# facebookresearch/mbrl-lib

Measured on AMD Instinct MI355X. Metric: candidate-steps/sec (pop×particles×horizon / plan) per CEM iter; plans/sec, higher is better.
Workload: dtype f32

## Files before the change

__graft_entry__.py:

```python
import os
import subprocess
import sys

ROOT = os.path.dirname(os.path.abspath(__file__))
PKG = os.path.join(ROOT, "mbrl-lib_amd")
CSRC = os.path.join(PKG, "csrc")
LIB = os.path.join(PKG, "hipets", "libhipets.so")
BUILDINFO = os.path.join(PKG, "hipets", "libhipets.buildinfo.json")
OBJDIR = os.path.join(PKG, "build")
HIPCC = os.environ.get("HIPCC", "/opt/rocm/bin/hipcc")
HOST_UNITS = ["train.hip", "plan.hip", "rollout.hip", "model.hip", "comm.hip", "engine.hip"]
UNITS = ["rollout_r3.hip", "rollout_r4_gen.hip", "rollout_r4_gens.hip", "rollout_r3_gen.hip", "rollout_r3_gens.hip", "rollout_r2.hip", "rollout_r2_gen.hip",
         "rollout_r2_gens.hip", "rollout_r1_gen.hip", "rollout_r1_gens.hip", "rollout_r1.hip", "rollout_r4.hip", "rollout_r2_fast.hip", "rollout_r3_fast.hip",
         "rollout_r1_fast.hip", "planet.hip"] + HOST_UNITS + ["rollout_r4_fast.hip"]
FLAGS = ["--offload-arch=gfx950", "-O3", "-std=c++17", "-ffp-contract=off", "-fPIC", "-Wno-pass-failed"]


def _sources():
    return sorted(os.path.join(CSRC, f) for f in os.listdir(CSRC)) + [os.path.join(ROOT, "include", "hipets.h")]


def source_digest(extra_flags=()):
    import hashlib

    h = hashlib.sha256()
    h.update(" ".join(FLAGS + list(extra_flags)).encode())
    for path in _sources():
        h.update(os.path.basename(path).encode())
        with open(path, "rb") as f:
            h.update(f.read())
    return h.hexdigest()[:16]


def built_digest(lib=LIB):
    import json

    info = os.path.splitext(lib)[0] + ".buildinfo.json"
    if not (os.path.exists(lib) and os.path.exists(info)):
        return None
    try:
        return json.load(open(info)).get("source_digest")
    except Exception:
        return None


def scan_isa_hazards(asm_path):
    import re

    def regs(tok):
        tok = tok.strip().rstrip(",")
        m = re.fullmatch(r"([va])\[(\d+):(\d+)\]", tok)
        if m:
            return {(m.group(1), x) for x in range(int(m.group(2)), int(m.group(3)) + 1)}
        m = re.fullmatch(r"([va])(\d+)", tok)
        return {(m.group(1), int(m.group(2)))} if m else set()

    prog, labels, in_asm = [], {}, False
    for raw in open(asm_path, errors="replace"):
        line = raw.split(";")[0].strip() if not raw.lstrip().startswith(";;#") else raw.strip()
        if line.startswith(";;#ASMSTART"):
            in_asm = True
            continue
        if line.startswith(";;#ASMEND"):
            in_asm = False
            continue
        if not line or line.startswith("."):
            if line.startswith(".L") and line.endswith(":"):
                labels[line[:-1]] = len(prog)
                prog.append(("label", line[:-1], False))
            continue
        if line.endswith(":"):
            if line[0].isdigit():
                continue
            prog.append(("kernel", line[:-1], False))
            continue
        prog.append(("ins", line, in_asm))

    findings, seen = [], 0

    def step(kernel, line, asm, inflight, recent, count, via):
        nonlocal seen
        parts = line.replace(",", " ").split()
        op, ops = parts[0], parts[1:]
        touched = set()
        for o in ops:
            touched |= regs(o)
        if op.startswith("v_mfma"):
            if asm:
                if count:
                    seen += 1
                src = set()
                for o in ops[1:]:
                    src |= regs(o)
                ws = 0
                for nop, written, text, _ in reversed(recent[-3:]):
                    if ws >= 2:
                        break
                    if nop is not None:
                        ws += nop
                        continue
                    if written & src:
                        findings.append(f"{kernel}: '{text}' writes a source of '{line}' {ws} wait state(s) ahead{via}")
                    ws += 1
            inflight = [(r, c - 32) for r, c in inflight if c - 32 > 0]
            if asm:
                inflight.append((regs(ops[0]), 40))
            recent.append((None, set(), line, set()))
        else:
            cost, nop = 4, None
            if op == "s_nop":
                nop = int(ops[0]) + 1
                cost = 4 * nop
            elif op.startswith("s_waitcnt") or op.startswith("s_barrier"):
                cost = 64
            if any(r & touched for r, _ in inflight) and op.split("_")[0] in ("v", "ds", "global", "buffer", "scratch", "flat"):
                findings.append(f"{kernel}: '{line}' touches the destination of an MFMA still in flight{via}")
            inflight = [(r, c - cost) for r, c in inflight if c - cost > 0]
            writes = set()
            if ops and (op.startswith("v_") or op.startswith("ds_read") or (op.split("_")[0] in ("global", "buffer", "flat", "scratch") and "_load" in op)):
                writes = regs(ops[0])
            if writes:
                ws = 0
                for pnop, _, ptext, pstore in reversed(recent[-3:]):
                    if ws >= 2:
                        break
                    if pnop is not None:
                        ws += pnop
                        continue
                    if pstore & writes:
                        findings.append(f"{kernel}: '{line}' overwrites the data of '{ptext}' {ws} wait state(s) behind it{via}")
                    ws += 1
            store_data = set()
            if asm and op.split("_")[0] in ("global", "buffer", "flat", "scratch") and re.search(r"_store_dwordx[34]", op):
                store_data = regs(ops[1]) if op.startswith(("global", "flat", "scratch")) else regs(ops[0])
            recent.append((nop, regs(ops[0]) if (op.startswith("v_") and ops) else set(), line, store_data))
        if len(recent) > 8:
            del recent[0]
        return inflight

    def undrained(inflight, recent):
        ws = 0
        for nop, written, _, store in reversed(recent[-3:]):
            if ws >= 2:
                break
            if nop is not None:
                ws += nop
                continue
            if written or store:
                return True
            ws += 1
        return bool(inflight)

    edges = []
    kernel, inflight, recent = "?", [], []
    for kind, text, asm in prog:
        if kind == "kernel":
            kernel, inflight, recent = text, [], []
        elif kind == "ins":
            inflight = step(kernel, text, asm, inflight, recent, True, "")
            op = text.split()[0]
            if op.startswith("s_cbranch") or op == "s_branch":
                target = text.split()[-1]
                if target in labels and undrained(inflight, recent):
                    edges.append((kernel, target, list(inflight), list(recent)))
            if op in ("s_branch", "s_endpgm", "s_setpc_b64"):
                inflight, recent = [], []
    done = set()
# ... 247 lines not shown
```

include/hipets.h:

```cpp
#ifndef HIPETS_H
#define HIPETS_H

#include <stdint.h>

#ifdef __cplusplus
extern "C" {
#endif

#define HIPETS_ABI_VERSION 9
#define HIPETS_MAX_LAYERS 8
#define HIPETS_MAX_REWARD_TERMS 64
#define HIPETS_MAX_TERM_INTERVALS 64
#define HIPETS_MAX_OBS_COLUMNS 512

typedef struct hipets_engine hipets_engine;

enum { HIPETS_ACT_RELU = 0, HIPETS_ACT_SILU = 1, HIPETS_ACT_LEAKY_RELU = 2, HIPETS_ACT_TANH = 3, HIPETS_ACT_SIGMOID = 4 };
enum { HIPETS_PROP_RANDOM_MODEL = 0, HIPETS_PROP_FIXED_MODEL = 1, HIPETS_PROP_EXPECTATION = 2 };
enum { HIPETS_OBS_NONE = 0, HIPETS_OBS_HALFCHEETAH = 1, HIPETS_OBS_CARTPOLE_PETS = 2,
       HIPETS_OBS_COLUMNS = 3  };
enum { HIPETS_REW_LEARNED = 0, HIPETS_REW_CARTPOLE = 1, HIPETS_REW_CARTPOLE_PETS = 2, HIPETS_REW_INVERTED_PENDULUM = 3,
       HIPETS_REW_HALFCHEETAH = 4, HIPETS_REW_PUSHER = 5,
       HIPETS_REW_NONE = 6,
       HIPETS_REW_TERMS = 7  };
enum { HIPETS_TERM_NONE = 0, HIPETS_TERM_CARTPOLE = 1, HIPETS_TERM_INVERTED_PENDULUM = 2, HIPETS_TERM_HOPPER = 3,
       HIPETS_TERM_WALKER2D = 4, HIPETS_TERM_ANT = 5, HIPETS_TERM_HUMANOID = 6,
       HIPETS_TERM_BOX = 7  };
enum { HIPETS_NORM_NONE = 0, HIPETS_NORM_F32 = 1, HIPETS_NORM_F64 = 2 };
enum { HIPETS_ENSEMBLE_GAUSSIAN_MLP = 0, HIPETS_ENSEMBLE_BASIC = 1 };
enum { HIPETS_PREC_F32 = 0,
       HIPETS_PREC_BF16X3 = 1,
       HIPETS_PREC_BF16 = 2
                                };
enum { HIPETS_MODE_EXACT = 0,
       HIPETS_MODE_FAST = 1,
       HIPETS_MODE_DEVICE = 2
                                };

enum { HIPETS_TERM_FN_LINEAR = 0, HIPETS_TERM_FN_SQUARE = 1, HIPETS_TERM_FN_ABS = 2,
       HIPETS_TERM_FN_SIN = 3, HIPETS_TERM_FN_COS = 4, HIPETS_TERM_FN_EXP = 5, HIPETS_TERM_FN_SQRT = 6 };
enum { HIPETS_TERM_SRC_OBS = 0, HIPETS_TERM_SRC_ACT = 1, HIPETS_TERM_SRC_GROUP = 2, HIPETS_TERM_SRC_CONST = 3 };
enum { HIPETS_TERM_OP_ADD = 0, HIPETS_TERM_OP_MUL = 1, HIPETS_TERM_OP_DIV = 2 };
#define HIPETS_TERM_MAX_LEVEL 2
#define HIPETS_TERM_WORD(fn, op, level) ((int32_t)((fn) | ((op) << 8) | ((level) << 16)))
#define HIPETS_TERM_WORD_FN(word) ((int32_t)((word) & 0xff))
#define HIPETS_TERM_WORD_OP(word) ((int32_t)(((word) >> 8) & 0xff))
#define HIPETS_TERM_WORD_LEVEL(word) ((int32_t)(((uint32_t)(word)) >> 16))
enum { HIPETS_BOX_LO_OPEN = 1, HIPETS_BOX_HI_OPEN = 2 };
typedef struct {
    int32_t fn;
    int32_t source;
    int32_t i;
    int32_t j;
    float c;
    float w;
} hipets_reward_term;
typedef struct {
    int32_t dim;
    int32_t flags;
    float lo;
    float hi;
} hipets_term_interval;

enum { HIPETS_COL_ID = 0, HIPETS_COL_SIN = 1, HIPETS_COL_COS = 2 };
typedef struct {
    int32_t dim;
    int32_t fn;
} hipets_obs_column;

typedef struct {
    int32_t obs_dim;
    int32_t act_dim;
    int32_t in_dim;
    int32_t out_dim;
    int32_t hid;
    int32_t n_layers;
    int32_t ensemble_size;
    int32_t n_members;
    const int32_t* members;
    int32_t activation;
    float leaky_slope;
    int32_t propagation;
    int32_t deterministic;
    int32_t obs_process;
    int32_t reward_fn;
    int32_t termination_fn;
    int32_t target_is_delta;
    int32_t learned_rewards;
    int32_t n_no_delta;
    const int32_t* no_delta;
    int32_t normalizer;
    const double* norm_mean;
    const double* norm_std;
    const float* min_logvar;
    const float* max_logvar;
    const void* const* weights;
    const void* const* biases;
    int32_t ensemble_kind;
    int32_t precision;
    const hipets_reward_term* reward_terms;
    const hipets_term_interval* term_intervals;
    int32_t n_reward_terms;
    int32_t n_term_intervals;
    float reward_bias;
    float alive_bonus;
    int32_t term_require_finite;
} hipets_model_desc;

typedef struct {
    int32_t mode;
    const int64_t* perms;
    const float* eps;
    uint64_t seed;
    uint64_t stream_id;
    const int32_t* member_schedule;
    const float* fast_eps;
    float* trace_next_obs;
    float* trace_rewards;
    int32_t rows_per_group;
    int64_t* phase_cycles;
    int32_t no_sample;
    int32_t rows_per_member;
    int32_t n_env;
    int32_t generic_kernel;
    int32_t member_schedule_len;
    uint64_t perm_stream_id;
} hipets_rollout_opts;

int hipets_abi_version(void);
const char* hipets_last_error(void);
#define HIPETS_ERR_NONE 0
#define HIPETS_ERR_INVALID_ARGUMENT 1
#define HIPETS_ERR_RUNTIME 2
#define HIPETS_ERR_TIMEOUT 3
int hipets_last_error_kind(void);
int hipets_create(int device, hipets_engine** out);
void hipets_destroy(hipets_engine* e);

int hipets_set_model(hipets_engine* e, const hipets_model_desc* desc, void* stream);
int hipets_set_model_columns(hipets_engine* e, const hipets_model_desc* desc, const hipets_obs_column* cols, int32_t n_cols, void* stream);

int hipets_rollout(hipets_engine* e, const float* actions, const float* s0, int32_t pop, int32_t horizon,
                   int32_t num_particles, const hipets_rollout_opts* opts, float* returns, void* stream);
int hipets_step(hipets_engine* e, const float* obs, const float* actions, int32_t batch, const hipets_rollout_opts* opts,
                float* next_obs, float* rewards, uint8_t* dones, void* stream);

int hipets_fast_geometry(hipets_engine* e, int32_t pop, int32_t num_particles, int32_t horizon, int32_t rows_per_group,
                         int32_t* n_workgroups, int32_t* row_tiles);

enum { HIPETS_KERNEL_GENERIC = 0, HIPETS_KERNEL_HIDDEN_STATIC = 1, HIPETS_KERNEL_FUSED = 2, HIPETS_KERNEL_WIDE = 3,
       HIPETS_KERNEL_BF16 = 4  };
int hipets_kernel_class(hipets_engine* e, int32_t pop, int32_t num_particles, int32_t horizon, int32_t mode, int32_t rows_per_group,
                        int32_t* kernel_class, int32_t* row_tiles);

int hipets_fast_schedule(hipets_engine* e, int32_t horizon, int32_t n_workgroups, uint64_t seed, uint64_t stream_id,
                         int32_t* schedule, void* stream);
int hipets_fast_normals(hipets_engine* e, int32_t horizon, int32_t batch, uint64_t seed, uint64_t stream_id,
                        float* normals, void* stream);

int hipets_device_perms(hipets_engine* e, int32_t horizon, int32_t batch, uint64_t seed, uint64_t stream_id, int64_t* perms,
                        void* stream);

int hipets_set_persistent(hipets_engine* e, int32_t on);
int hipets_set_handover_timeout(hipets_engine* e, double seconds);
int hipets_check_async_error(hipets_engine* e, int32_t* timed_out);

typedef struct {
    int32_t population_size;
    int32_t horizon;
    int32_t act_dim;
    int32_t num_iterations;
    int32_t elite_num;
    double alpha;
    int32_t return_mean_elites;
    int32_t clipped_normal;
    int32_t unbiased_var;
} hipets_cem_params;

int hipets_cem_sample(hipets_engine* e, const hipets_cem_params* p, const float* mu, const float* dispersion,
                      const float* lower, const float* upper, const float* z, uint64_t seed, uint64_t stream_id,
                      float* population, void* stream);
int hipets_cem_refit(hipets_engine* e, const hipets_cem_params* p, float* values, const float* population,
                     float* mu, float* dispersion, float* best_value, float* best_solution, int32_t* elite_idx,
                     void* stream);

int hipets_cem_refit_elites(hipets_engine* e, const hipets_cem_params* p, float* values, const float* population,
                            const int32_t* elites, float* mu, float* dispersion, float* best_value, float* best_solution,
                            void* stream);

int hipets_gather_rows(hipets_engine* e, int32_t rows, int32_t dim, const float* src, const int32_t* index, float* dst,
                       void* stream);

int hipets_mppi_sample(hipets_engine* e, int32_t pop, int32_t horizon, int32_t act_dim, double beta, const float* mean,
                       const float* past_action, const float* lower, const float* upper, const float* z, uint64_t seed,
                       uint64_t stream_id, float* population, void* stream);
int hipets_mppi_update(hipets_engine* e, int32_t pop, int32_t horizon, int32_t act_dim, double gamma, float* values,
                       const float* population, float* mean, void* stream);

int hipets_icem_sample(hipets_engine* e, int32_t n, int32_t horizon, int32_t act_dim, double exponent, const float* mu,
                       const float* var, const float* lower, const float* upper, const float* normals, uint64_t seed,
                       uint64_t stream_id, float* population, void* stream);
int hipets_icem_shift(hipets_engine* e, int32_t keep, int32_t horizon, int32_t act_dim, const float* kept, const float* mu,
                      const float* var, const float* end_noise, uint64_t seed, uint64_t stream_id, float* out, void* stream);

int hipets_set_plan_mode(hipets_engine* e, int32_t mode);

typedef struct {
    float* populations;
    float* values;
    float* mus;
    float* dispersions;
    int32_t* elite_idx;
    int32_t max_rows;
} hipets_plan_trace;
int hipets_set_plan_trace(hipets_engine* e, const hipets_plan_trace* trace);

int hipets_plan_cem(hipets_engine* e, const hipets_cem_params* p, const float* x0, const float* lower,
                    const float* upper, const float* s0, int32_t num_particles, uint64_t seed, uint64_t plan_id,
                    float* out, void* stream);
int hipets_plan_cem_batched(hipets_engine* e, const hipets_cem_params* p, int32_t n_env, const float* x0, const float* lower,
                            const float* upper, const float* s0, int32_t num_particles, uint64_t seed, uint64_t plan_id,
                            float* out, void* stream);

int hipets_plan_mppi(hipets_engine* e, int32_t population_size, int32_t horizon, int32_t act_dim, int32_t num_iterations,
                     double gamma, double beta, float* mean, const float* lower, const float* upper, const float* s0,
                     int32_t num_particles, uint64_t seed, uint64_t plan_id, void* stream);

int hipets_plan_mppi_batched(hipets_engine* e, int32_t population_size, int32_t horizon, int32_t act_dim, int32_t num_iterations,
                             double gamma, double beta, int32_t n_env, float* mean, const float* lower, const float* upper,
                             const float* s0, int32_t num_particles, uint64_t seed, uint64_t plan_id, void* stream);

typedef struct {
    int32_t population_size;
    int32_t horizon;
    int32_t act_dim;
    int32_t num_iterations;
    int32_t elite_num;
    int32_t keep_elite_size;
    int32_t population_size_module;
    int32_t return_mean_elites;
    double alpha;
    double population_decay_factor;
    double colored_noise_exponent;
} hipets_icem_params;

int hipets_plan_icem(hipets_engine* e, const hipets_icem_params* p, const float* x0, const float* lower, const float* upper,
                     float* elite, int32_t has_elite, const int32_t* keep_idx, const float* s0, int32_t num_particles,
                     uint64_t seed, uint64_t plan_id, float* out, void* stream);

int hipets_plan_icem_batched(hipets_engine* e, const hipets_icem_params* p, int32_t n_env, const float* x0, const float* lower,
                             const float* upper, float* elite, int32_t has_elite, const int32_t* keep_idx, const float* s0,
                             int32_t num_particles, uint64_t seed, uint64_t plan_id, float* out, void* stream);

#define HIPETS_COMM_ID_BYTES 128
int hipets_comm_unique_id(void* id_out);
int hipets_comm_init(hipets_engine* e, const void* unique_id, int32_t rank, int32_t world_size);
int hipets_comm_destroy(hipets_engine* e);
int hipets_comm_info(hipets_engine* e, int32_t* rank, int32_t* world_size);
int hipets_plan_cem_sharded(hipets_engine* e, const hipets_cem_params* p, const float* x0, const float* lower, const float* upper,
                            const float* s0, int32_t num_particles, uint64_t seed, uint64_t plan_id, float* out, void* stream);

int hipets_plan_mppi_sharded(hipets_engine* e, int32_t population_size, int32_t horizon, int32_t act_dim, int32_t num_iterations,
                             double gamma, double beta, float* mean, const float* lower, const float* upper, const float* s0,
                             int32_t num_particles, uint64_t seed, uint64_t plan_id, void* stream);
int hipets_plan_icem_sharded(hipets_engine* e, const hipets_icem_params* p, const float* x0, const float* lower, const float* upper,
                             float* elite, int32_t has_elite, const int32_t* keep_idx, const float* s0, int32_t num_particles,
                             uint64_t seed, uint64_t plan_id, float* out, void* stream);

typedef struct {
    int32_t latent_size;
    int32_t action_size;
    int32_t belief_size;
    int32_t hidden_size;
    float min_std;
    const void* w_embed;
    const void* b_embed;
    const void* w_ih;
    const void* b_ih;
    const void* w_hh;
    const void* b_hh;
    const void* w_prior1;
    const void* b_prior1;
    const void* w_prior2;
    const void* b_prior2;
    const void* w_rew1;
    const void* b_rew1;
    const void* w_rew2;
    const void* b_rew2;
    const void* w_rew3;
    const void* b_rew3;
} hipets_planet_desc;
int hipets_planet_set_model(hipets_engine* e, const hipets_planet_desc* d, void* stream);

typedef struct {
    const float* eps;
    uint64_t seed;
    uint64_t stream_id;
    int32_t no_sample;
    float* trace_latent;
    float* trace_belief;
    float* trace_rewards;
    int64_t* phase_cycles;
    int32_t n_env;
} hipets_planet_opts;
int hipets_planet_rollout(hipets_engine* e, const float* actions, const float* latent0, const float* belief0, int32_t pop,
                          int32_t horizon, int32_t num_particles, const hipets_planet_opts* opts, float* returns, void* stream);

int hipets_plan_planet_cem(hipets_engine* e, const hipets_cem_params* p, const float* x0, const float* lower, const float* upper,
                           const float* latent0, const float* belief0, int32_t num_particles, uint64_t seed, uint64_t plan_id,
                           float* out, void* stream);

int hipets_plan_planet_cem_batched(hipets_engine* e, const hipets_cem_params* p, int32_t n_env, const float* x0, const float* lower,
                                   const float* upper, const float* latent0, const float* belief0, int32_t num_particles, uint64_t seed,
                                   uint64_t plan_id, float* out, void* stream);
int hipets_plan_planet_mppi_batched(hipets_engine* e, int32_t population_size, int32_t horizon, int32_t act_dim, int32_t num_iterations,
                                    double gamma, double beta, int32_t n_env, float* mean, const float* lower, const float* upper,
// ... 41 lines not shown
```

mbrl-lib_amd/csrc/engine.hip:

```cpp
#include <cstdarg>
#include <cstdio>
#include <cstring>

#include "engine.hpp"

namespace hipets {

thread_local std::string g_err;
thread_local int g_err_kind = HIPETS_ERR_NONE;

int fail(const char* fmt, ...) {
    char buf[1024];
    va_list ap;
    va_start(ap, fmt);
    vsnprintf(buf, sizeof(buf), fmt, ap);
    va_end(ap);
    g_err = buf;
    g_err_kind = HIPETS_ERR_INVALID_ARGUMENT;
    return 1;
}

int fail_kind(const int kind, const char* fmt, ...) {
    char buf[1024];
    va_list ap;
    va_start(ap, fmt);
    vsnprintf(buf, sizeof(buf), fmt, ap);
    va_end(ap);
    g_err = buf;
    g_err_kind = kind;
    return 1;
}

int stage_h2d(hipets_engine* e, void* dst, const void* src, size_t bytes, hipStream_t st) {
    hipets_engine::HostStage& sl = e->stage[e->stage_next];
    e->stage_next = (e->stage_next + 1) % 4;
    if (sl.used) HCHECK(hipEventSynchronize(sl.done));
    if (bytes > sl.cap) {
        if (sl.p) (void)hipHostFree(sl.p);
        sl.p = nullptr;
        sl.cap = 0;
        HCHECK(hipHostMalloc(&sl.p, bytes < 4096 ? 4096 : bytes, hipHostMallocDefault));
        sl.cap = bytes < 4096 ? 4096 : bytes;
    }
    if (!sl.done) HCHECK(hipEventCreateWithFlags(&sl.done, hipEventDisableTiming));
    std::memcpy(sl.p, src, bytes);
    HCHECK(hipMemcpyAsync(dst, sl.p, bytes, hipMemcpyHostToDevice, st));
    HCHECK(hipEventRecord(sl.done, st));
    sl.used = true;
    return 0;
}

int enter_stream(hipets_engine* e, hipStream_t st) {
    if (!e->last_done) HCHECK(hipEventCreateWithFlags(&e->last_done, hipEventDisableTiming));
    if (e->last_stream_set && e->last_stream != st) HCHECK(hipStreamWaitEvent(st, e->last_done, 0));
    e->last_stream = st;
    e->last_stream_set = true;
    return 0;
}

StreamScope::~StreamScope() {
    static const bool off = std::getenv("HIPETS_NO_STREAM_SCOPE") != nullptr;
    if (e && e->last_done && !off) (void)hipEventRecord(e->last_done, st);
}

}

using namespace hipets;

extern "C" {

int hipets_abi_version(void) { return HIPETS_ABI_VERSION; }

const char* hipets_last_error(void) { return g_err.c_str(); }

int hipets_last_error_kind(void) { return g_err_kind; }

int hipets_create(int device, hipets_engine** out) {
    if (!out) return fail("null out pointer");
    *out = nullptr;
    int n = 0;
    hipError_t err = hipGetDeviceCount(&n);
    if (err != hipSuccess || n <= 0)
        return fail("no HIP device visible (%s) -- libhipets has no CPU fallback", hipGetErrorString(err));
    if (device < 0 || device >= n) return fail("device %d out of range (%d visible)", device, n);
    HCHECK(hipSetDevice(device));
    hipDeviceProp_t prop;
    HCHECK(hipGetDeviceProperties(&prop, device));
    if (std::string(prop.gcnArchName).rfind("gfx950", 0) != 0)
        return fail("device %d is %s; libhipets is built for gfx950 (MI355X) only", device, prop.gcnArchName);
    auto* e = new hipets_engine();
    e->device = device;
    e->num_cu = prop.multiProcessorCount > 0 ? prop.multiProcessorCount : 256;
    e->lds_max = prop.sharedMemPerBlockOptin > 0 ? (size_t)prop.sharedMemPerBlockOptin : (size_t)prop.sharedMemPerBlock;
    if (e->lds_max > 160 * 1024) e->lds_max = 160 * 1024;
    if (hipHostMalloc(reinterpret_cast<void**>(&e->error_flag), sizeof(int), hipHostMallocMapped) != hipSuccess) e->error_flag = nullptr;
    if (e->error_flag) *e->error_flag = 0;
    const char* np = std::getenv("HIPETS_NO_PERSISTENT");
    e->persistent_ok = e->error_flag != nullptr && !(np && np[0] == '1');
    if (e->census.ensure(2 * sizeof(int))) e->persistent_ok = false;
    *out = e;
    return 0;
}

void hipets_destroy(hipets_engine* e) {
    if (!e) return;
    (void)hipSetDevice(e->device);
    comm_release(e);
    for (DevBuf* b : {&e->w3pack, &e->wpack, &e->bpack, &e->layer_meta, &e->norm_mean, &e->norm_std, &e->min_lv, &e->max_lv, &e->no_delta, &e->members,
                      &e->s0, &e->state, &e->totals, &e->term, &e->exchange, &e->step_keys, &e->plan_keys, &e->mu, &e->disp, &e->population, &e->values,
                      &e->best_value, &e->best_solution, &e->past_action, &e->kept, &e->elite_idx, &e->keep_idx, &e->planet_w, &e->planet_b, &e->planet_member, &e->planet_ops, &e->shard_values, &e->gathered, &e->census, &e->train_slab, &e->train_partial})
        b->release();
    for (auto& ev : e->events) { (void)hipEventDestroy(ev.first); (void)hipEventDestroy(ev.second); }
    for (auto& ev : e->event_pool) { (void)hipEventDestroy(ev.first); (void)hipEventDestroy(ev.second); }
    if (e->error_flag) (void)hipHostFree(e->error_flag);
    if (e->last_done) (void)hipEventDestroy(e->last_done);
    for (auto& sl : e->stage) {
        if (sl.p) (void)hipHostFree(sl.p);
        if (sl.done) (void)hipEventDestroy(sl.done);
    }
    delete e;
}

int hipets_set_plan_mode(hipets_engine* e, int32_t mode) {
    if (!e) return fail("null engine");
    if (mode != HIPETS_MODE_FAST && mode != HIPETS_MODE_DEVICE) return fail("plan mode must be HIPETS_MODE_FAST or HIPETS_MODE_DEVICE");
    e->plan_mode = mode;
    return 0;
}

int hipets_set_persistent(hipets_engine* e, int32_t on) {
    if (!e) return fail("null engine");
    if (on && !e->error_flag) return fail("persistent DEVICE-mode launches need the host-mapped timeout flag, which could not be allocated");
    e->persistent_ok = on != 0;
    return 0;
}

int hipets_set_handover_timeout(hipets_engine* e, double seconds) {
    if (!e) return fail("null engine");
    if (!(seconds >= 0.0) || seconds > 60.0) return fail("hand-over timeout %g s outside [0, 60]", seconds);
    e->poll_ticks = (long long)(seconds * 1.0e8);
    return 0;
}

int hipets_check_async_error(hipets_engine* e, int32_t* timed_out) {
    if (!e || !timed_out) return fail("null argument");
    *timed_out = 0;
    if (e->error_flag && *e->error_flag) {
        *e->error_flag = 0;
        e->persistent_ok = false;
        *timed_out = 1;
        g_err_kind = HIPETS_ERR_TIMEOUT;
        g_err = "a persistent DEVICE-mode rollout gave up waiting for rows of another workgroup (its workgroups were not all resident: "
                "another process or stream held CUs); everything computed from that launch on is invalid -- re-run the call.  "
                "Persistent launches are now disabled for this engine.";
    }
    return 0;
}

int hipets_set_plan_trace(hipets_engine* e, const hipets_plan_trace* t) {
    if (!e) return fail("null engine");
    e->has_trace = t != nullptr;
    if (t) e->trace = *t;
    return 0;
}

int hipets_timing_enable(hipets_engine* e, int32_t on) {
    if (!e) return fail("null engine");
    e->timing = on != 0;
    e->timing_stride = on > 1 ? on : 1;
    e->launch_counter = 0;
    return 0;
}

int hipets_timing_read(hipets_engine* e, int64_t* launches, double* total_ms, int32_t reset) {
    if (!e) return fail("null engine");
    HCHECK(hipSetDevice(e->device));
    double tot = 0.0;
    for (auto& ev : e->events) {
        HCHECK(hipEventSynchronize(ev.second));
        float ms = 0.f;
        HCHECK(hipEventElapsedTime(&ms, ev.first, ev.second));
        tot += ms;
    }
    if (launches) *launches = (int64_t)e->events.size();
    if (total_ms) *total_ms = tot;
    if (reset) {
        for (auto& ev : e->events) e->event_pool.push_back(ev);
        e->events.clear();
    }
    return 0;
}

}
```

mbrl-lib_amd/csrc/engine.hpp:

```cpp
#pragma once
#include <hip/hip_runtime.h>

#include <cstdlib>
#include <string>
#include <utility>
#include <vector>

#include "../../include/hipets.h"
#include "planet_types.hpp"
#include "rollout_types.hpp"

namespace hipets {

extern thread_local std::string g_err;
extern thread_local int g_err_kind;

}

#pragma GCC visibility push(hidden)

namespace hipets {

int fail(const char* fmt, ...);
int fail_kind(int kind, const char* fmt, ...);

#define HCHECK(expr)                                                                              \
    do {                                                                                          \
        hipError_t _e = (expr);                                                                   \
        if (_e != hipSuccess) return fail_kind(HIPETS_ERR_RUNTIME, "%s failed: %s (%s:%d)", #expr, hipGetErrorString(_e), __FILE__, __LINE__); \
    } while (0)

struct DevBuf {
    void* p = nullptr;
    size_t cap = 0;
    int ensure(size_t bytes) {
        if (bytes <= cap) return 0;
        if (p) (void)hipFree(p);
        p = nullptr;
        cap = 0;
        hipError_t e = hipMalloc(&p, bytes);
        if (e != hipSuccess) return fail_kind(HIPETS_ERR_RUNTIME, "hipMalloc(%zu) failed: %s", bytes, hipGetErrorString(e));
        cap = bytes;
        return 0;
    }
    void release() {
        if (p) (void)hipFree(p);
        p = nullptr;
        cap = 0;
    }
    template <typename T>
    T* as() const { return reinterpret_cast<T*>(p); }
};

}

#pragma GCC visibility pop

struct hipets_engine {
    using DevBuf = hipets::DevBuf;
    int device = 0;
    int num_cu = 256;
    size_t lds_max = 160 * 1024;
    bool has_model = false;
    hipets::ModelDev md{};
    int ensemble_size = 0;
    DevBuf w3pack;
    DevBuf wpack, bpack, layer_meta, norm_mean, norm_std, min_lv, max_lv, no_delta, members;
    DevBuf s0, state, totals, term;
    DevBuf exchange, step_keys, plan_keys;
    struct HostStage { void* p = nullptr; size_t cap = 0; hipEvent_t done = nullptr; bool used = false; };
    HostStage stage[4];
    int stage_next = 0;
    uint32_t tag_base = 0;
    uint64_t plan_keys_seed = 0, plan_keys_first = 0;
    int plan_keys_count = 0, plan_keys_H = 0;
    int* error_flag = nullptr;
    bool persistent_ok = true;
    long long poll_ticks = 20000000ll;
    DevBuf census;
    hipStream_t last_stream = nullptr;
    bool last_stream_set = false;
    hipEvent_t last_done = nullptr;
    DevBuf mu, disp, population, values, best_value, best_solution, past_action, kept, elite_idx, keep_idx;
    void* comm = nullptr;
    int comm_rank = 0, comm_world = 1;
    DevBuf shard_values, gathered;
    bool has_planet = false;
    bool planet_static = false;
    hipets::PlanetDev pd{};
    DevBuf planet_w, planet_b, planet_member, planet_ops;
    int plan_mode = HIPETS_MODE_FAST;
    bool has_trace = false;
    hipets_plan_trace trace{};
    bool timing = false;
    int timing_stride = 1;
    unsigned long long launch_counter = 0;
    std::vector<std::pair<hipEvent_t, hipEvent_t>> events;
    std::vector<std::pair<hipEvent_t, hipEvent_t>> event_pool;
    DevBuf train_slab, train_partial;
};

#pragma GCC visibility push(hidden)

namespace hipets {


int stage_h2d(hipets_engine* e, void* dst, const void* src, size_t bytes, hipStream_t st);

int enter_stream(hipets_engine* e, hipStream_t st);
struct StreamScope {
    hipets_engine* e;
    hipStream_t st;
    ~StreamScope();
};
#define ENTER_STREAM(e, st)                \
    if (enter_stream((e), (st))) return 1; \
    StreamScope stream_scope_ { (e), (st) }

struct LocalErr {
    std::string msg;
    int kind = HIPETS_ERR_NONE;
    bool ok() const { return kind == HIPETS_ERR_NONE; }
    void note(const int rc) {
        if (rc && ok()) { msg = g_err; kind = g_err_kind == HIPETS_ERR_NONE ? HIPETS_ERR_RUNTIME : g_err_kind; }
    }
    int report() const {
        if (ok()) return 0;
        g_err = msg;
        g_err_kind = kind;
        return 1;
    }
};


int rollout_impl(hipets_engine* e, const float* actions, const float* s0, int32_t pop, int32_t H, int32_t P, const hipets_rollout_opts* o,
                 float* returns, void* stream);
int planet_rollout_impl(hipets_engine* e, const float* actions, const float* latent0, const float* belief0, int32_t pop, int32_t H, int32_t P,
                        const hipets_planet_opts* o, float* returns, hipStream_t st);
int plan_step_keys(hipets_engine* e, int H, int iters, uint64_t seed, uint64_t first_stream, hipStream_t st);
int pack_weights(hipStream_t st, float* dst, const float* src, const int* members, int M, int K, int N, int Kp, int Np, long long member_stride,
                 long long layer_off, int permute_cols, int src_nk, int head_dim = 0);
int pack_weights_b3(hipStream_t st, uint4* dst, const float* src, const int* members, int M, int K, int N, int Kp32, int Np, long long member_stride,
                    long long layer_off, int src_nk, int pieces);
int pack_bias(hipStream_t st, float* dst, const float* src, const int* members, int M, int N, int Np, int member_stride, int layer_off,
              int permute_cols, int head_dim = 0);


int comm_all_gather(hipets_engine* e, size_t width, hipStream_t st);
int comm_unpad_shards(hipets_engine* e, int rows, int width, hipStream_t st);
void comm_release(hipets_engine* e);

}

#pragma GCC visibility pop
```

mbrl-lib_amd/csrc/kspec.hpp:

```cpp
#pragma once
#include "gemm_bf16.hpp"
#include "gemm_f32.hpp"
#include "rollout_types.hpp"

namespace hipets {

constexpr int kSplMaxTiles = 8;

constexpr int lean_ld(int hidc, int outc) {
    int m = (hidc > outc ? hidc : outc) * 16;
    while (m % 64 != 8) m += 4;
    return m;
}

template <int ACT_, int HIDC_ = -1, int OUTC_ = -1, int NORM_ = -1, int OBSP_ = -1, int REW_ = -1, int TERM_ = -1, int KMODE_ = -1, int PREC_ = 0,
          int FUSE_ = 0>
struct KSpec {
    static constexpr bool WIDE = FUSE_ != 0 && HIDC_ >= 0 && PREC_ == HIPETS_PREC_F32 && OUTC_ > kSplMaxTiles;
    static constexpr int LD = (HIDC_ >= 0 && PREC_ == HIPETS_PREC_F32) ? lean_ld(HIDC_, WIDE ? HIDC_ : OUTC_) : -1;
    static constexpr int ACT = ACT_, HIDC = HIDC_, OUTC = OUTC_, NORM = NORM_, OBSP = OBSP_, REW = REW_, TERM = TERM_, KMODE = KMODE_;
    static constexpr int PREC = PREC_;
    static constexpr int PIECES = PREC_ == HIPETS_PREC_BF16X3 ? 3 : (PREC_ == HIPETS_PREC_BF16 ? 1 : 0);
    static constexpr bool LEAN = HIDC_ >= 0 && OUTC_ >= 0;
    static constexpr bool HID_STATIC = HIDC_ >= 0 && OUTC_ < 0;
    static constexpr bool FUSE = FUSE_ != 0 && LEAN && PREC_ == HIPETS_PREC_F32 && (OUTC_ <= kSplMaxTiles || WIDE);
    static constexpr bool SPL_OUT = OUTC_ >= 0 && OUTC_ <= kSplMaxTiles;
    static constexpr bool KSPLIT = FUSE && !WIDE && kWaves == 4 && HIDC_ == 13;
    static_assert(!FUSE || ((REW_ == HIPETS_REW_HALFCHEETAH || REW_ == HIPETS_REW_CARTPOLE || REW_ == HIPETS_REW_CARTPOLE_PETS || REW_ == HIPETS_REW_LEARNED) &&
                            (TERM_ == HIPETS_TERM_NONE || TERM_ == HIPETS_TERM_CARTPOLE || TERM_ == HIPETS_TERM_HUMANOID || TERM_ == HIPETS_TERM_INVERTED_PENDULUM ||
                             TERM_ == HIPETS_TERM_HOPPER)),
                  "fused tail: the reward / termination lane sees dims 0..3 of its row");
    static_assert(!FUSE || TERM_ != HIPETS_TERM_HOPPER || (REW_ == HIPETS_REW_LEARNED && !WIDE),
                  "fused tail with an all-dims termination function: instances with a learned reward");
    static_assert(!FUSE || REW_ != HIPETS_REW_LEARNED || !WIDE, "fused tail with learned rewards: no WIDE instance");
    static_assert(!FUSE || (NORM_ == HIPETS_NORM_F64 && (OBSP_ == HIPETS_OBS_NONE || !WIDE)), "fused tail: f64 normaliser; WIDE instances: no obs preprocessing");
    static_assert(!FUSE || OBSP_ == HIPETS_OBS_NONE || OBSP_ == HIPETS_OBS_HALFCHEETAH || OBSP_ == HIPETS_OBS_CARTPOLE_PETS, "unknown obs preprocessing");
};

template <int R, class S>
__device__ __forceinline__ void mlp_layer_b3(const ModelDev& md, const LayerMeta* lmeta, const int l, const int member, const float* in, float* out,
                                             const int wave, const int lane) {
    const LayerMeta lm = lmeta[l];
    const uint4* W3 = md.w3 + (size_t)member * md.w3member + lm.woff3;
    const float* bias = md.b + (size_t)member * md.bmember + lm.boff;
    const char* inb = reinterpret_cast<const char*>(in);
    char* outb = reinterpret_cast<char*>(out);
    if (l < md.n_layers - 1) linear_op_b3<R, S::ACT, S::HIDC, S::PIECES>(W3, bias, lm.Kp32 / 32, md.ld * 4, false, inb, outb, wave, lane);
    else linear_op_b3<R, S::ACT, S::OUTC, S::PIECES>(W3, bias, lm.Kp32 / 32, md.ld * 4, true, inb, outb, wave, lane);
}

template <int R, class S>
__device__ __forceinline__ void mlp_layer(const ModelDev& md, const LayerMeta* lmeta, const int l, const int member,
                                          const float* in, float* out, const int wave, const int lane, Prof& prof, float* part = nullptr) {
    const LayerMeta lm = lmeta[l];
    const float* W = md.w + (size_t)member * md.wmember + lm.woff;
    const float* bias = md.b + (size_t)member * md.bmember + lm.boff;
    if constexpr (S::KSPLIT && R == 1) {
        float* const po = part + (l & 1) * (kWaves * 64 * 4);
        const float* const pi = part + ((l & 1) ^ 1) * (kWaves * 64 * 4);
        if (l == 0) linear_op<R, S::ACT, S::HIDC, NoTail, S::LD, false, -1, 2>(W, bias, lm, md.ld, true, md.activation, md.slope, in, out, wave, lane, prof, nullptr, 0, nullptr, po);
        else linear_op<R, S::ACT, S::HIDC, NoTail, S::LD, false, S::HIDC, 3>(W, bias, lm, md.ld, true, md.activation, md.slope, in, out, wave, lane, prof, nullptr, 0, pi, po);
    } else if constexpr (S::LEAN) {
        constexpr int kHidChunks = MinWavesOf<R>::value == 1 ? S::HIDC : -1;
        if (l == 0) linear_op<R, S::ACT, S::HIDC, NoTail, S::LD>(W, bias, lm, md.ld, true, md.activation, md.slope, in, out, wave, lane, prof, nullptr, S::WIDE ? md.ld_in : 0);
        else if (l < md.n_layers - 1) linear_op<R, S::ACT, S::HIDC, NoTail, S::LD, false, kHidChunks>(W, bias, lm, md.ld, true, md.activation, md.slope, in, out, wave, lane, prof);
        else linear_op<R, S::ACT, S::OUTC, NoTail, S::LD, (S::OUTC <= kSplMaxTiles), kHidChunks>(W, bias, lm, md.ld, false, md.activation, md.slope, in, out, wave, lane, prof);
    } else if constexpr (S::HID_STATIC) {
        constexpr int kHidChunks = (MinWavesOf<R>::value == 1 && ((S::HIDC + kWaves - 1) / kWaves) * R <= 13) ? S::HIDC : -1;
        if (l == 0) linear_op<R, S::ACT, S::HIDC, NoTail, S::LD>(W, bias, lm, md.ld, true, md.activation, md.slope, in, out, wave, lane, prof);
        else if (l < md.n_layers - 1) linear_op<R, S::ACT, S::HIDC, NoTail, S::LD, false, kHidChunks>(W, bias, lm, md.ld, true, md.activation, md.slope, in, out, wave, lane, prof);
        else if (lm.Np / kTile <= kSplMaxTiles)
            linear_op<R, S::ACT, -1, NoTail, -1, true>(W, bias, lm, md.ld, false, md.activation, md.slope, in, out, wave, lane, prof);
        else linear_op<R, S::ACT>(W, bias, lm, md.ld, false, md.activation, md.slope, in, out, wave, lane, prof);
    } else {
        if (l == md.n_layers - 1 && lm.Np / kTile <= kSplMaxTiles)
            linear_op<R, S::ACT, -1, NoTail, -1, true>(W, bias, lm, md.ld, false, md.activation, md.slope, in, out, wave, lane, prof);
        else linear_op<R, S::ACT>(W, bias, lm, md.ld, l < md.n_layers - 1, md.activation, md.slope, in, out, wave, lane, prof);
    }
}

template <int R, class S, class TL>
__device__ __forceinline__ void mlp_output_layer_fused(const ModelDev& md, const LayerMeta* lmeta, const int member, const float* in,
                                                       const int wave, const int lane, Prof& prof, const TL& tl, const float* part = nullptr) {
    const LayerMeta lm = lmeta[md.n_layers - 1];
    const float* W = md.w + (size_t)member * md.wmember + lm.woff_pairs;
    const float* bias = md.b + (size_t)member * md.bmember + lm.boff_pairs;
    if constexpr (S::KSPLIT && R == 1) {
        const float* const pi = part + ((md.n_layers - 2) & 1) * (kWaves * 64 * 4);
        linear_op<R, S::ACT, S::OUTC, TL, S::LD, S::SPL_OUT, S::HIDC, 1>(W, bias, lm, md.ld, false, md.activation, md.slope, in, nullptr, wave, lane, prof, &tl, 0, pi);
    } else {
        linear_op<R, S::ACT, S::OUTC, TL, S::LD, S::SPL_OUT, MinWavesOf<R>::value == 1 ? S::HIDC : -1>(W, bias, lm, md.ld, false, md.activation, md.slope, in, nullptr, wave, lane, prof, &tl);
    }
}

}
```

mbrl-lib_amd/csrc/residency.hpp:

```cpp
#pragma once
#include <hip/hip_ext.h>

#include <cstdio>
#include <cstdlib>
#include <iterator>
#include <map>
#include <mutex>
#include <utility>

#include "launch.hpp"
#include "residency_rule.hpp"

namespace hipets {

inline hipError_t enqueue_rollout(const KernelRec& k, int grid, unsigned lds, const ModelDev& md, const RolloutArgs& ra, hipStream_t st, hipEvent_t start, hipEvent_t stop) {
    void* args[2] = {const_cast<ModelDev*>(&md), const_cast<RolloutArgs*>(&ra)};
    if (start) (void)hipExtLaunchKernel(k.fn, dim3(grid), dim3(kThreads), args, lds, st, start, stop, 0);
    else (void)hipLaunchKernel(k.fn, dim3(grid), dim3(kThreads), args, lds, st);
    return hipGetLastError();
}

inline int max_workgroups() {
    static const int wg_cap = [] { const char* v = std::getenv("HIPETS_MAX_WORKGROUPS"); const int n = v ? std::atoi(v) : 0; return n > 0 ? n : 0; }();
    return wg_cap;
}

struct DeviceResidency {
    std::mutex mu;
    std::map<std::pair<const void*, unsigned>, Occ> table;
};
constexpr int kDevSlots = 64, kMaxEntries = 32;
inline DeviceResidency& device_residency(const int dev) {
    static DeviceResidency devices[kDevSlots];
    return devices[dev >= 0 && dev < kDevSlots ? dev : kDevSlots - 1];
}
template <class F>
hipError_t with_residency(const KernelRec& k, const unsigned lds, const int lds_max, F&& f) {
    int dev = 0;
    hipError_t e = hipGetDevice(&dev);
    if (e != hipSuccess) return e;
    DeviceResidency& d = device_residency(dev);
    std::lock_guard<std::mutex> lock(d.mu);
    auto& table = d.table;
    if (dev >= kDevSlots) table.clear();
    const auto first = table.lower_bound({k.fn, 0u}), last = table.upper_bound({k.fn, ~0u});
    if (std::distance(first, last) >= kMaxEntries && !table.count({k.fn, lds})) table.erase(first, last);
    Occ& oc = table[{k.fn, lds}];
    if (oc.blocks == 0) {
        int nb = 0;
        hipFuncAttributes fa{};
        if ((e = hipOccupancyMaxActiveBlocksPerMultiprocessor(&nb, k.fn, kThreads, lds)) != hipSuccess) return e;
        if ((e = hipDeviceGetAttribute(&oc.n_cu, hipDeviceAttributeMultiprocessorCount, dev)) != hipSuccess) return e;
        if ((e = hipFuncGetAttributes(&fa, k.fn)) != hipSuccess) return e;
        const int regs = std::max(fa.numRegs, 1);
        const int by_regs = 512 / (((regs + 7) / 8) * 8);
        const int by_lds = (int)((size_t)lds_max / ((size_t)lds + (size_t)fa.sharedSizeBytes + 2048));
        if (std::getenv("HIPETS_DEBUG_OCC")) std::fprintf(stderr, "[hipets] occupancy query %d, regs %d -> %d, lds %u -> %d\n", nb, regs, by_regs, lds, by_lds);
        oc.api = std::clamp(nb, 1, 2);
        oc.blocks = std::clamp(std::max(nb, std::min(by_regs, by_lds)), 1, 2);
        oc.validated = 0;
    }
    return f(oc);
}

inline hipError_t resident_capacity(KernelRec& k, const int want, const unsigned lds, const int lds_max, const ModelDev& md, const RolloutArgs& q, hipStream_t st, int* capacity) {
    const hipError_t e = full_lds_once(k.lds, k.fn, lds_max);
    if (e != hipSuccess) return e;
    auto census_ok = [&](const int g) {
        int seen[2] = {0, 0};
        if (!q.census || hipMemsetAsync(q.census, 0, sizeof(seen), st) != hipSuccess || enqueue_rollout(k, g, lds, md, q, st, nullptr, nullptr) != hipSuccess ||
            hipMemcpyAsync(seen, q.census, sizeof(seen), hipMemcpyDeviceToHost, st) != hipSuccess || hipStreamSynchronize(st) != hipSuccess)
            return false;
        if (std::getenv("HIPETS_DEBUG_OCC")) std::fprintf(stderr, "[hipets] co-residency self-test: grid %d, arrived %d, saw all %d\n", g, seen[0], seen[1]);
        return seen[1] == g;
    };
    return with_residency(k, lds, lds_max, [&](Occ& oc) { return *capacity = resident_capacity_rule(oc, want, max_workgroups(), census_ok), hipSuccess; });
}

inline hipError_t decide_launch_form(KernelRec& k, const int logical, const unsigned lds, const int lds_max, const int n_cu, const ModelDev& md, const RolloutArgs& ra,
                                     int* census, const long long poll_ticks, hipStream_t st, bool* persistent_ok, bool* persistent) {
    int capacity = 0;
    RolloutArgs q = ra;
    q.census = census;
    q.poll_ticks = std::max(poll_ticks, 20000000ll);
    const hipError_t e = resident_capacity(k, logical, lds, lds_max, md, q, st, &capacity);
    if (e == hipSuccess && capacity <= 0) *persistent_ok = false;
    *persistent = capacity > 0 && persistent_pays(logical, capacity, n_cu);
    return e;
}

inline hipError_t launch_rollout_kernel(KernelRec& k, int grid, const unsigned lds, const int lds_max, const ModelDev& md, const RolloutArgs& ra, hipStream_t st,
                                        hipEvent_t start, hipEvent_t stop) {
    const hipError_t e = full_lds_once(k.lds, k.fn, lds_max);
    if (e != hipSuccess) return e;
    if (!ra.exchange) return enqueue_rollout(k, grid, lds, md, ra, st, start, stop);
    return with_residency(k, lds, lds_max, [&](Occ& oc) {
        grid = std::min(grid, oc.blocks * oc.n_cu);
        if (max_workgroups()) grid = std::min(grid, max_workgroups());
        if (grid > oc.validated) return hipErrorLaunchFailure;
        return enqueue_rollout(k, grid, lds, md, ra, st, start, stop);
    });
}

}
```

mbrl-lib_amd/csrc/rollout.hip:

```cpp
#include <hip/hip_ext.h>

#include <algorithm>

#include "engine.hpp"
#include "launch.hpp"
#include "residency.hpp"
#include "rollout_helpers.hpp"
#include "rollout_smem.hpp"

using namespace hipets;

namespace {

KernelRec* rollout_instance(const hipets_engine* e, int R, const RolloutArgs& ra) {
    static constexpr decltype(&rollout_instance_r1) resolvers[kMaxR] = {rollout_instance_r1, rollout_instance_r2, rollout_instance_r3, rollout_instance_r4};
    if (R < 1 || R > kMaxR) return fail("unsupported rows_per_group %d (1..%d)", R, kMaxR), nullptr;
    hipError_t why = hipSuccess;
    KernelRec* k = resolvers[R - 1](e->md, ra, &why);
    const bool b3 = e->md.precision == HIPETS_PREC_BF16X3;
    if (!k && why == hipErrorNotSupported && (b3 || e->md.precision == HIPETS_PREC_BF16))
        fail("precision %s: no shape-specialised kernel instance for this model / call (SiLU, f64 normaliser, no obs preprocessing, in-kernel "
             "sampling, one of the %s layer shapes, R = %d); use precision f32", b3 ? "bf16x3" : "bf16", b3 ? "BASELINE" : "two bf16", R);
    else if (!k) fail_kind(HIPETS_ERR_RUNTIME, "rollout kernel launch failed: %s", hipGetErrorString(why));
    return k;
}

int launch_rollout(hipets_engine* e, int R, int grid, size_t lds, const RolloutArgs& ra, hipStream_t st) {
    RolloutArgs rl = ra;
    rl.lds_bytes = (unsigned)lds;
    KernelRec* k = rollout_instance(e, R, rl);
    if (!k) return 1;
    hipEvent_t a = nullptr, b = nullptr;
    const bool timed = e->timing && (e->launch_counter++ % (unsigned long long)e->timing_stride) == 0;
    if (timed) {
        if (!e->event_pool.empty()) {
            a = e->event_pool.back().first;
            b = e->event_pool.back().second;
            e->event_pool.pop_back();
        } else {
            HCHECK(hipEventCreate(&a));
            HCHECK(hipEventCreate(&b));
        }
    }
    const hipError_t err = launch_rollout_kernel(*k, grid, (unsigned)lds, (int)e->lds_max, e->md, rl, st, a, b);
    if (timed) e->events.emplace_back(a, b);
    if (err != hipSuccess) return fail_kind(HIPETS_ERR_RUNTIME, "rollout kernel launch failed: %s", hipGetErrorString(err));
    return 0;
}

int launch_form(hipets_engine* e, int R, int logical, size_t lds, RolloutArgs ra, hipStream_t st, bool* persistent) {
    ra.lds_bytes = (unsigned)lds;
    KernelRec* k = rollout_instance(e, R, ra);
    if (!k) return 1;
    HCHECK(decide_launch_form(*k, logical, (unsigned)lds, (int)e->lds_max, e->num_cu, e->md, ra, e->census.as<int>(), e->poll_ticks, st, &e->persistent_ok, persistent));
    return 0;
}

size_t lds_for(const hipets_engine* e, int R, int horizon, bool wide = false) {
    const ModelDev& md = e->md;
    if (wide)
        return rollout_smem_bytes(kTile * R, lean_ld(md.hidC, md.hidC), md.obs_dim, md.act_dim, md.in_dim, md.out_dim, md.out_total, horizon, false,
                                  md.lv_rows, md.ld_in);
    return rollout_smem_bytes(kTile * R, md.ld, md.obs_dim, md.act_dim, md.in_dim, md.out_dim, md.out_total, horizon,
                              md.propagation == HIPETS_PROP_EXPECTATION, md.lv_rows);
}


int wave_units(int C, int R) {
    const int full = C / kWaves, rem = C % kWaves, nu = rem * R;
    int simd[4] = {0, 0, 0, 0};
    for (int w = 0; w < kWaves; ++w) simd[w % 4] += full * R + (w < nu ? (nu - w + kWaves - 1) / kWaves : 0);
    return std::max(std::max(simd[0], simd[1]), std::max(simd[2], simd[3]));
}

int choose_R(const hipets_engine* e, long long tiles_total_per_slice, int slices, int forced, int horizon, bool wide, bool drift) {
    if (forced > 0) return forced;
    const int C = e->md.hidC;
    const double a = (wide ? (drift ? 6.45 : 2.67) : 1.77) * (double)C / 13.0;
    int best = 1;
    double best_cost = 1e300;
    bool b3_only = false;
    if (e->md.precision != HIPETS_PREC_F32)
        for (int R = 1; R <= kMaxR; ++R) b3_only = b3_only || b3_shape_exists(e->md, R);
    for (int R = 1; R <= kMaxR; ++R) {
        if (lds_for(e, R, horizon, wide) > e->lds_max) break;
        if (wide && R > 2) break;
        if (b3_only && !b3_shape_exists(e->md, R)) continue;
        const long long groups = (tiles_total_per_slice + R - 1) / R;
        const long long nwg = groups * slices;
        const long long n = (nwg + e->num_cu - 1) / e->num_cu;
        const int co = (R <= 2 && !wide) ? 2 : 1;
        const double u = wave_units(C, R);
        const double u_pair = (co == 2 && drift) ? (double)C * R / 4.0 : u;
        const long long full = n / co, rem = n % co;
        double cost = (double)full * (a + co * u_pair) + (rem ? a + (double)rem * u : 0.0);
        if (!lean_shape_exists(e->md, R)) cost *= 1.08;
        if (cost < best_cost - 1e-9) {
            best_cost = cost;
            best = R;
        }
    }
    return best;
}

enum class GeoCall { rollout, step, query };
struct Geometry {
    int domains;
    long long rpd;
    long long tiles;
    bool wide;
    bool whole_horizon;
    int R;
    int groups;
    size_t lds;
};

int rollout_geometry(const hipets_engine* e, int mode, long long B, int rows_per_member, int H, int rows_per_group, GeoCall call,
                     const RolloutArgs& probe, Geometry* g) {
    const ModelDev& md = e->md;
    const bool fast = mode == HIPETS_MODE_FAST;
    const bool expectation = md.propagation == HIPETS_PROP_EXPECTATION;
    g->domains = (fast || expectation) ? 1 : md.M;
    const bool slots = mode == HIPETS_MODE_EXACT && !expectation && rows_per_member > 0;
    g->rpd = slots ? rows_per_member : B / g->domains;
    g->tiles = (g->rpd + kTile - 1) / kTile;
    g->whole_horizon = fast && call != GeoCall::step;
    g->wide = call != GeoCall::step && rows_per_group <= 2 && wide_model(md) && lean_call(md, probe);
    if (g->whole_horizon && !g->wide && wide_model(md) && probe.schedule && rows_per_group == 0)
        return fail("this call runs the general kernel layout (injected eps / traces / generic_kernel) on a model whose default geometry is "
                    "the wide-output instance's: size member_schedule with hipets_fast_geometry(rows_per_group = -1) and pass its row-tile "
                    "count as opts->rows_per_group");
    const bool drift = g->whole_horizon && H > 1;
    g->R = choose_R(e, g->tiles, g->domains, rows_per_group, H, g->wide, drift);
    g->lds = lds_for(e, g->R, H, g->wide);
    if (g->lds > e->lds_max) return fail("rows_per_group %d does not fit LDS", g->R);
    g->groups = (int)((g->tiles + g->R - 1) / g->R);
    if (fast && call != GeoCall::query && g->groups > 8000)
        return fail("FAST mode supports at most 8000 workgroups per launch (got %d)%s", g->groups, call == GeoCall::rollout ? "; shard the population" : "");
    return 0;
}

int check_member_maps(const hipets_engine* e, const hipets_rollout_opts* o, long long B, bool one_step) {
    const ModelDev& md = e->md;
    const bool device = o->mode == HIPETS_MODE_DEVICE;
    const bool expectation = md.propagation == HIPETS_PROP_EXPECTATION;
    const bool slots = o->mode == HIPETS_MODE_EXACT && !expectation && o->rows_per_member > 0;
    const bool exempt = one_step ? o->mode == HIPETS_MODE_EXACT && o->rows_per_member > 0 : slots;
    if (!md.iid_members && !exempt && B % md.M != 0)
        return fail("GaussianMLP ensemble requires batch size to be a multiple of the number of models. "
                    "Current batch size is %lld for %d models.", B, md.M);
    if ((o->mode != HIPETS_MODE_EXACT && !device) || expectation) return 0;
    if (device && md.iid_members) return fail("DEVICE mode has no BasicEnsemble (iid member map) variant: use FAST, or EXACT with injected maps");
    if (!device && !o->perms) return fail("EXACT mode with random_model/fixed_model propagation needs opts.perms");
    if ((md.iid_members && !device && !slots) || (slots && o->rows_per_member > B))
        return fail("EXACT mode with per-row member maps needs opts.rows_per_member in [1, B] (padded member slots)");
    return 0;
}

int bind_mode(const hipets_engine* e, const hipets_rollout_opts* o, long long B, int H, GeoCall call, uint64_t perm_stream, uint32_t perm_step,
              RolloutArgs* ra, Geometry* g) {
    const bool expectation = e->md.propagation == HIPETS_PROP_EXPECTATION;
    const bool fast = o->mode == HIPETS_MODE_FAST;
    if (o->mode == HIPETS_MODE_DEVICE) {
        ra->use_philox = o->no_sample ? 0 : 1;
        if (!expectation) {
            ra->perm_n = (unsigned)B;
            perm_radices((uint32_t)B, &ra->perm_a, &ra->perm_b);
            ra->perm_keys = perm_round_keys(perm_key(o->seed, perm_stream, perm_step));
        }
    } else if (o->mode == HIPETS_MODE_EXACT) {
        ra->perm = expectation ? nullptr : reinterpret_cast<const long long*>(o->perms);
        ra->eps = o->eps;
    } else if (fast) {
        ra->eps = o->fast_eps;
        ra->use_philox = (o->fast_eps || o->no_sample) ? 0 : 1;
        ra->schedule = expectation ? nullptr : o->member_schedule;
        ra->fast_members = call == GeoCall::step ? 1 : 0;
    } else {
        return fail("unknown rollout mode %d", o->mode);
    }
    if (rollout_geometry(e, o->mode, B, o->rows_per_member, H, o->rows_per_group, call, *ra, g)) return 1;
    ra->whole_horizon = g->whole_horizon ? 1 : 0;
    ra->wide_lds = g->wide ? 1 : 0;
    ra->groups = g->groups;
    if (!g->whole_horizon) ra->rows_per_domain = (int)g->rpd;
    if (fast) perm_radices((uint32_t)g->groups, &ra->fm_a, &ra->fm_b);
    return 0;
}

}

namespace hipets {

int pack_weights(hipStream_t st, float* dst, const float* src, const int* members, int M, int K, int N, int Kp, int Np, long long member_stride,
                 long long layer_off, int permute_cols, int src_nk, int head_dim) {
    const long long n = (long long)Kp * Np * M;
    hipLaunchKernelGGL(pack_weights_kernel, dim3((unsigned)((n + 255) / 256)), dim3(256), 0, st, dst, src, members, M, K, N, Kp, Np, member_stride, layer_off,
                       permute_cols, src_nk, head_dim);
    HCHECK(hipGetLastError());
    return 0;
}

int pack_weights_b3(hipStream_t st, uint4* dst, const float* src, const int* members, int M, int K, int N, int Kp32, int Np, long long member_stride,
                    long long layer_off, int src_nk, int pieces) {
    const long long n3 = (long long)(Np / 16) * (Kp32 / 32) * pieces * 64 * M;
    hipLaunchKernelGGL(pack_weights_b3_kernel, dim3((unsigned)((n3 + 255) / 256)), dim3(256), 0, st, dst, src, members, M, K, N, Kp32, Np, member_stride,
                       layer_off, src_nk, pieces);
    HCHECK(hipGetLastError());
    return 0;
}

int pack_bias(hipStream_t st, float* dst, const float* src, const int* members, int M, int N, int Np, int member_stride, int layer_off, int permute_cols,
              int head_dim) {
    const int nb = M * Np;
    hipLaunchKernelGGL(pack_bias_kernel, dim3((nb + 255) / 256), dim3(256), 0, st, dst, src, members, M, N, Np, member_stride, layer_off, permute_cols, head_dim);
    HCHECK(hipGetLastError());
    return 0;
}

int plan_step_keys(hipets_engine* e, int H, int iters, uint64_t seed, uint64_t first_stream, hipStream_t st) {
    if (e->md.propagation != HIPETS_PROP_RANDOM_MODEL || iters < 1 || e->plan_mode != HIPETS_MODE_DEVICE || !e->persistent_ok) return 0;
    if (e->plan_keys.ensure((size_t)iters * H * sizeof(PermKeys))) return 1;
    hipLaunchKernelGGL(step_keys_kernel, dim3((H + 63) / 64, iters), dim3(64), 0, st, e->plan_keys.as<PermKeys>(), H, (unsigned long long)seed,
                       (unsigned long long)first_stream);
    HCHECK(hipGetLastError());
    e->plan_keys_seed = seed; e->plan_keys_first = first_stream; e->plan_keys_count = iters; e->plan_keys_H = H;
    return 0;
}

int rollout_impl(hipets_engine* e, const float* actions, const float* s0, int32_t pop, int32_t H, int32_t P,
                 const hipets_rollout_opts* o, float* returns, void* stream) {
    if (!e || !e->has_model) return fail("engine has no model (call hipets_set_model)");
    if (!actions || !o) return fail("null argument");
    if (pop < 1 || H < 1 || P < 1) return fail("bad pop/horizon/particles");
    if (e->error_flag && *e->error_flag) {
        *e->error_flag = 0;
        e->persistent_ok = false;
        return fail_kind(HIPETS_ERR_TIMEOUT, "a persistent DEVICE-mode rollout timed out waiting for rows of another workgroup (its workgroups were not all "
                    "resident) and nobody asked (hipets_check_async_error after the results were read): the results of that earlier "
                    "call are invalid.  Persistent launches are now disabled for this engine.");
    }
    hipStream_t st = reinterpret_cast<hipStream_t>(stream);
    HCHECK(hipSetDevice(e->device));
    const ModelDev& md = e->md;
    const long long B = (long long)pop * P;
    if (B > 0x7FFFFFFF / std::max(md.obs_dim, md.out_dim)) return fail("batch too large");
    if (o->rows_per_group < 0 || o->rows_per_group > kMaxR) return fail("rows_per_group outside [0, %d]", kMaxR);

    const int n_env = o->n_env > 1 ? o->n_env : 1;
    if (n_env > 1 && ((o->mode != HIPETS_MODE_FAST && o->mode != HIPETS_MODE_DEVICE) || pop % n_env != 0))
        return fail("n_env %d needs FAST or DEVICE mode and a population (%d) divisible by it", n_env, pop);
    if (e->s0.ensure((size_t)n_env * md.obs_dim * 4)) return 1;
    if (e->totals.ensure((size_t)B * 4)) return 1;
    if (s0 && stage_h2d(e, e->s0.p, s0, (size_t)n_env * md.obs_dim * 4, st)) return 1;

    RolloutArgs ra{};
    ra.pop = pop; ra.P = P; ra.H = H; ra.B = (int)B;
    ra.actions = actions;
    ra.s0 = e->s0.as<float>();
    ra.totals = e->totals.as<float>();
    ra.seed = o->seed;
    ra.stream_id = o->stream_id;
    ra.trace_next_obs = o->trace_next_obs;
    ra.trace_rewards = o->trace_rewards;
    ra.phase_cycles = reinterpret_cast<long long*>(o->phase_cycles);
    ra.pop_env = n_env > 1 ? pop / n_env : 0;
    ra.generic_only = o->generic_kernel;

    const bool device = o->mode == HIPETS_MODE_DEVICE;
    if ((device || o->mode == HIPETS_MODE_EXACT) && check_member_maps(e, o, B, false)) return 1;
    Geometry g;
    if (bind_mode(e, o, B, H, GeoCall::rollout, o->stream_id, 0xFFFFFFFFu, &ra, &g)) return 1;
    if (o->mode != HIPETS_MODE_FAST) {
        const int R = g.R, domains = g.domains, groups = g.groups;
        const size_t lds = g.lds;
        if (!device && md.propagation == HIPETS_PROP_RANDOM_MODEL) ra.perm_step = (long long)domains * g.rpd;
        const bool per_step = !device || md.propagation == HIPETS_PROP_RANDOM_MODEL;
        if (e->state.ensure((size_t)B * md.obs_dim * 4) || e->term.ensure((size_t)B)) return 1;
        ra.state = e->state.as<float>();
        ra.term = e->term.as<unsigned char>();
        bool persistent = device && per_step && e->persistent_ok && H > 1;
        if (persistent && launch_form(e, R, domains * groups, lds, ra, st, &persistent)) return 1;
        if (!persistent) {
            hipLaunchKernelGGL(init_state_kernel, dim3((unsigned)((B * md.obs_dim + 255) / 256)), dim3(256), 0, st,
                               e->state.as<float>(), e->totals.as<float>(), e->term.as<unsigned char>(), e->s0.as<float>(), (int)B,
                               md.obs_dim, P, ra.pop_env);
            HCHECK(hipGetLastError());
        }
        if (persistent) {
            const size_t nv = 2 * ((size_t)(md.obs_dim + 1) / 2 + 1);
            const size_t cap_before = e->exchange.cap;
            if (e->exchange.ensure((size_t)B * nv * 8)) return 1;
            if (e->exchange.cap != cap_before || e->tag_base > 0xFFFFFFFFu - 2u * (uint32_t)H - 2u) {
                HCHECK(hipMemsetAsync(e->exchange.p, 0, e->exchange.cap, st));
                e->tag_base = 0;
            }
            ra.tag_base = e->tag_base;
            e->tag_base += (uint32_t)H;
            ra.exchange = e->exchange.as<unsigned long long>();
            const uint64_t sid = o->stream_id;
            if (e->plan_keys.p && o->seed == e->plan_keys_seed && H == e->plan_keys_H && sid >= e->plan_keys_first &&
                sid - e->plan_keys_first < (uint64_t)e->plan_keys_count) {
                ra.step_keys = e->plan_keys.as<PermKeys>() + (size_t)(sid - e->plan_keys_first) * H;
            } else {
                if (e->step_keys.ensure((size_t)H * sizeof(PermKeys))) return 1;
                hipLaunchKernelGGL(step_keys_kernel, dim3((H + 63) / 64), dim3(64), 0, st, e->step_keys.as<PermKeys>(), H, (unsigned long long)o->seed,
                                   (unsigned long long)o->stream_id);
                HCHECK(hipGetLastError());
                ra.step_keys = e->step_keys.as<PermKeys>();
            }
            ra.error_flag = e->error_flag;
            ra.poll_ticks = e->poll_ticks;
            ra.t_begin = 0;
            ra.t_end = H;
            ra.n_logical = domains * groups;
            static const bool ragged_ok = [] { const char* v = std::getenv("HIPETS_RAGGED_LAST_TURN"); return !(v && v[0] == '0'); }();
            ra.ragged_last_turn = (g.wide && R == 2 && ragged_ok) ? 1 : 0;

            if (launch_rollout(e, R, domains * groups, lds, ra, st)) return 1;
        } else if (per_step) {
            for (int t = 0; t < H; ++t) {
                ra.t_begin = t;
                ra.t_end = t + 1;
                if (ra.perm_n) ra.perm_keys = perm_round_keys(perm_key(o->seed, o->stream_id, (uint32_t)t));
                if (launch_rollout(e, R, domains * groups, lds, ra, st)) return 1;
            }
        } else {
            ra.t_begin = 0;
            ra.t_end = H;
            if (launch_rollout(e, R, domains * groups, lds, ra, st)) return 1;
        }
    } else {
        const int nwg = g.groups;
        if (o->member_schedule && o->member_schedule_len != 0 && (long long)o->member_schedule_len != (long long)H * nwg)
            return fail("member_schedule holds %d entries, this call's geometry is horizon %d x %d workgroups (hipets_fast_geometry)",
                        o->member_schedule_len, H, nwg);
        ra.t_begin = 0;
        ra.t_end = H;
        if (launch_rollout(e, g.R, nwg, g.lds, ra, st)) return 1;
    }
    if (!returns) return 0;
    hipLaunchKernelGGL(particle_mean_kernel, dim3((pop + 255) / 256), dim3(256), 0, st, e->totals.as<float>(), returns, pop, P);
    HCHECK(hipGetLastError());
    return 0;
}

int planet_rollout_impl(hipets_engine* e, const float* actions, const float* latent0, const float* belief0, int32_t pop, int32_t H,
                        int32_t P, const hipets_planet_opts* o, float* returns, hipStream_t st) {
    const int n_env = std::max(o->n_env, 1);
    if (o->n_env < 0 || n_env > 4096) return fail("n_env %d outside [0, 4096]", o->n_env);
    if (pop % n_env) return fail("PlaNet rollout: population %d is not divisible by n_env %d", pop, n_env);
    const long long B = (long long)pop * P;
    if (B > 0x7FFFFFFF / std::max(e->pd.belief, 16)) return fail("batch too large");
    if (e->totals.ensure((size_t)B * 4)) return 1;
    PlanetArgs ra{};
    ra.pop = pop; ra.P = P; ra.H = H; ra.B = (int)B;
    ra.n_env = n_env;
    ra.rows_env = pop / n_env * P;
    ra.actions = actions;
    ra.latent0 = latent0;
    ra.belief0 = belief0;
    ra.totals = e->totals.as<float>();
    ra.eps = o->eps;
    ra.use_philox = (o->eps || o->no_sample) ? 0 : 1;
    ra.seed = o->seed;
    ra.stream_id = o->stream_id;
    ra.trace_latent = o->trace_latent;
    ra.trace_belief = o->trace_belief;
    ra.trace_rewards = o->trace_rewards;
    ra.phase_cycles = reinterpret_cast<long long*>(o->phase_cycles);
    const size_t lds = planet_smem_bytes(e->pd.ld);
    const int nwg = (int)((B + kTile - 1) / kTile);
    const char* pg = std::getenv("HIPETS_PLANET_GENERIC");
    HCHECK(launch_planet_rollout(nwg, (unsigned)lds, (int)e->lds_max, e->pd, ra, st, e->planet_static && !(pg && pg[0] == '1')));
    if (!returns) return 0;
    hipLaunchKernelGGL(particle_mean_kernel, dim3((pop + 255) / 256), dim3(256), 0, st, e->totals.as<float>(), returns, pop, P);
    HCHECK(hipGetLastError());
    return 0;
}

}

extern "C" {

int hipets_fast_geometry(hipets_engine* e, int32_t pop, int32_t P, int32_t horizon, int32_t rows_per_group,
                         int32_t* n_workgroups, int32_t* row_tiles) {
    if (!e || !e->has_model) return fail("engine has no model");
    if (pop < 1 || P < 1) return fail("bad pop/P");
    if (rows_per_group < -1 || rows_per_group > kMaxR) return fail("rows_per_group outside [-1, %d]", kMaxR);
    RolloutArgs probe{};
    probe.use_philox = 1;
    probe.generic_only = rows_per_group < 0 ? 1 : 0;
    Geometry g;
    if (rollout_geometry(e, HIPETS_MODE_FAST, (long long)pop * P, 0, horizon, std::max(rows_per_group, 0), GeoCall::query, probe, &g)) return 1;
    if (n_workgroups) *n_workgroups = g.groups;
    if (row_tiles) *row_tiles = g.R;
    return 0;
}

int hipets_kernel_class(hipets_engine* e, int32_t pop, int32_t P, int32_t horizon, int32_t mode, int32_t rows_per_group, int32_t* kernel_class,
                        int32_t* row_tiles) {
    if (!e || !e->has_model) return fail("engine has no model");
    if (pop < 1 || P < 1 || horizon < 1) return fail("bad pop/horizon/particles");
    if (rows_per_group < 0 || rows_per_group > kMaxR) return fail("rows_per_group outside [0, %d]", kMaxR);
    if (mode != HIPETS_MODE_FAST && mode != HIPETS_MODE_DEVICE) return fail("hipets_kernel_class: mode must be HIPETS_MODE_FAST or HIPETS_MODE_DEVICE");
    const ModelDev& md = e->md;
    const long long B = (long long)pop * P;
    if (mode == HIPETS_MODE_DEVICE && md.propagation != HIPETS_PROP_EXPECTATION) {
        if (md.iid_members && md.M > 1) return fail("DEVICE mode has no BasicEnsemble (iid member map) variant");
        if (B % md.M != 0) return fail("GaussianMLP ensemble requires batch size to be a multiple of the number of models. "
                                       "Current batch size is %lld for %d models.", B, md.M);
    }
    RolloutArgs probe{};
    probe.use_philox = 1;
    Geometry g;
    if (rollout_geometry(e, mode, B, 0, horizon, rows_per_group, GeoCall::query, probe, &g)) return fail("the model does not fit LDS");
    probe.whole_horizon = g.whole_horizon ? 1 : 0;
    probe.wide_lds = g.wide ? 1 : 0;
    int cls = HIPETS_KERNEL_GENERIC;
    switch (pick_rollout_instance(md, probe, g.R)) {
        case RolloutInstance::lean: case RolloutInstance::b3: cls = HIPETS_KERNEL_FUSED; break;
        case RolloutInstance::bf16: cls = HIPETS_KERNEL_BF16; break;
        case RolloutInstance::lean_wide: cls = HIPETS_KERNEL_WIDE; break;
        case RolloutInstance::hidden_static: cls = HIPETS_KERNEL_HIDDEN_STATIC; break;
        case RolloutInstance::generic_silu: case RolloutInstance::generic: break;
        case RolloutInstance::no_b3: return fail("bf16x3 arithmetic exists for the shape-specialised instances only");
        case RolloutInstance::no_bf16: return fail("bf16 arithmetic exists for the shape-specialised instances only");
        case RolloutInstance::no_wide: return fail("no WIDE instance of this model's shape for R = %d", g.R);
    }
    if (kernel_class) *kernel_class = cls;
    if (row_tiles) *row_tiles = g.R;
    return 0;
}

int hipets_rollout(hipets_engine* e, const float* actions, const float* s0, int32_t pop, int32_t H, int32_t P,
                   const hipets_rollout_opts* o, float* returns, void* stream) {
    if (!e || !s0) return fail("null argument");
    hipStream_t st = reinterpret_cast<hipStream_t>(stream);
    HCHECK(hipSetDevice(e->device));
    ENTER_STREAM(e, st);
    return rollout_impl(e, actions, s0, pop, H, P, o, returns, stream);
}

int hipets_step(hipets_engine* e, const float* obs, const float* actions, int32_t B, const hipets_rollout_opts* o, float* next_obs,
                float* rewards, uint8_t* dones, void* stream) {
    if (!e || !e->has_model) return fail("engine has no model (call hipets_set_model)");
    if (!obs || !actions || !o || !next_obs || !rewards || !dones) return fail("null argument");
    if (B < 1) return fail("bad batch");
    hipStream_t st = reinterpret_cast<hipStream_t>(stream);
    HCHECK(hipSetDevice(e->device));
    ENTER_STREAM(e, st);
    const ModelDev& md = e->md;
    if (o->rows_per_group < 0 || o->rows_per_group > kMaxR) return fail("rows_per_group outside [0, %d]", kMaxR);
    if (check_member_maps(e, o, B, true)) return 1;
    RolloutArgs ra{};
    ra.pop = B; ra.P = 1; ra.H = 1; ra.B = B;
    ra.actions = actions;
    ra.state = next_obs;
    ra.totals = rewards;
    ra.term = dones;
    ra.seed = o->seed;
    ra.stream_id = o->stream_id;
    ra.generic_only = o->generic_kernel;
    ra.t_begin = 0;
    ra.t_end = 1;
    const bool fixed = md.propagation == HIPETS_PROP_FIXED_MODEL;
    const uint64_t pstream = (fixed && o->perm_stream_id) ? o->perm_stream_id : o->stream_id;
    Geometry g;
    if (bind_mode(e, o, B, 1, GeoCall::step, pstream, fixed ? 0xFFFFFFFFu : 0u, &ra, &g)) return 1;
    if (o->mode == HIPETS_MODE_FAST && o->member_schedule && o->member_schedule_len != 0 && o->member_schedule_len != g.groups)
// ... 62 lines not shown
```

mbrl-lib_amd/csrc/rollout.hpp:

```cpp
#pragma once
#include "closed_forms.hpp"
#include "common.hpp"
#include "gemm_f32.hpp"
#include "kspec.hpp"
#include "rollout_smem.hpp"
#include "rollout_types.hpp"

namespace hipets {

__device__ __forceinline__ void pair_store(unsigned long long* p, const unsigned v0, const unsigned v1, const unsigned tag) {
    const u32x4g d = {v0, tag, v1, tag};
    asm volatile("global_store_dwordx4 %0, %1, off sc1\n\ts_nop 1" ::"v"(p), "v"(d) : "memory");
}
__device__ __forceinline__ void pair_load_issue(u32x4g& d, const unsigned long long* p) {
    asm volatile("global_load_dwordx4 %0, %1, off sc1" : "=&v"(d) : "v"(p) : "memory");
}
__device__ __forceinline__ void lds_barrier() { asm volatile("s_waitcnt lgkmcnt(0)\n\ts_barrier" ::: "memory"); }
__device__ __forceinline__ void pair_dma_issue(const unsigned long long* gsrc, const unsigned lds_dst) {
    unsigned keep;
    asm volatile("s_mov_b32 %0, m0\n\ts_mov_b32 m0, %2\n\ts_nop 0\n\tglobal_load_lds_dwordx4 %1, off sc1\n\ts_mov_b32 m0, %0"
                 : "=&s"(keep) : "v"(gsrc), "s"(lds_dst) : "memory");
}
__device__ __forceinline__ void vmem_drain() { asm volatile("s_waitcnt vmcnt(0)" ::: "memory"); }

template <int R, class S> struct MinWaves { static constexpr int value = S::WIDE ? 1 : MinWavesOf<R>::value; };

#ifdef HIPETS_STEP_TRACE
#define HIPETS_STAMP(k, step)                                                                                                     \
    do {       \
        (void)(step);                                                                                                             \
        if (persist && ra.phase_cycles && tid == 0 && n_serve <= 4)                                                                \
            ra.phase_cycles[128 + ((size_t)blockIdx.x * (ra.H * 4) + stamp_seq) * 4 + (k)] = wall_clock64();   \
    } while (0)
#else
#define HIPETS_STAMP(k, step) do {} while (0)
#endif

template <int R, class S>
__global__ __launch_bounds__(kThreads, (MinWaves<R, S>::value)) void rollout_kernel(const ModelDev md, const RolloutArgs ra) {
    constexpr int ROWS = kTile * R;
    constexpr bool kLean = S::LEAN;
    constexpr bool kB3 = S::PIECES > 0;
    constexpr int kNP = kB3 ? S::PIECES : 1;
    static_assert(!kB3 || kLean, "bf16x3 / bf16 arithmetic exists for the shape-specialised instances");
    const int normalizer = S::NORM >= 0 ? S::NORM : md.normalizer;
    const int obs_process = S::OBSP >= 0 ? S::OBSP : md.obs_process;
    const int reward_fn = S::REW >= 0 ? S::REW : md.reward_fn;
    const int term_fn = S::TERM >= 0 ? S::TERM : md.term_fn;
    const int lv_rows = kLean ? 1 : md.lv_rows;
    const bool deterministic = kLean ? false : md.deterministic != 0;
    float* const trace_next_obs = kLean ? nullptr : ra.trace_next_obs;
    float* const trace_rewards = kLean ? nullptr : ra.trace_rewards;
    const int ld_k = S::LD > 0 ? S::LD : md.ld;
    constexpr bool kWide = S::WIDE;
    const int ld_in = kWide ? md.ld_in : ld_k;
    extern __shared__ __attribute__((aligned(16))) char smem[];
    RolloutSmem sm;
    {
        char* p = smem;
#define HIPETS_CARVE(T, name, bytes)   \
    sm.name = reinterpret_cast<T*>(p); \
    p += (bytes);
        HIPETS_ROLLOUT_SECTIONS(HIPETS_CARVE, ROWS, ld_in, ld_k, md.obs_dim, md.act_dim, md.in_dim, md.lv_rows, md.out_dim, md.out_total, ra.H, false, false)
#undef HIPETS_CARVE
#if HIPETS_DEBUG_BOUNDS
        {
#define HIPETS_SECTION_START(T, name, bytes) (char*)sm.name,
            const char* const secs[] = {HIPETS_ROLLOUT_SECTION_NAMES(HIPETS_SECTION_START)};
#undef HIPETS_SECTION_START
            for (int i = 0; i < kRolloutSections; ++i) {
                HIPETS_BOUND(secs[i] >= smem && secs[i] <= smem + ra.lds_bytes);
                HIPETS_BOUND(((size_t)(secs[i] - smem) & 15) == 0);
                HIPETS_BOUND(i == 0 || secs[i] >= secs[i - 1]);
            }
            const bool expect = !S::LEAN && md.propagation == HIPETS_PROP_EXPECTATION;
            HIPETS_BOUND(rollout_smem_bytes(ROWS, ld_k, md.obs_dim, md.act_dim, md.in_dim, md.out_dim, md.out_total, ra.H, expect, md.lv_rows, kWide ? ld_in : 0) <= ra.lds_bytes);
            HIPETS_BOUND(md.Kp0 <= (kWide ? md.ld_in : ld_k) && md.obs_in + md.act_dim == md.in_dim && md.in_dim <= md.Kp0);
        }
#endif
    }
    const int tid = threadIdx.x;
    if (ra.census) {
        if (tid == 0) {
            __hip_atomic_fetch_add(ra.census, 1, __ATOMIC_RELAXED, __HIP_MEMORY_SCOPE_AGENT);
            const long long t0 = wall_clock64();
            bool all = true;
            while (__hip_atomic_load(ra.census, __ATOMIC_RELAXED, __HIP_MEMORY_SCOPE_AGENT) < (int)gridDim.x) {
                if (wall_clock64() - t0 > ra.poll_ticks) { all = false; break; }
                __builtin_amdgcn_s_sleep(8);
            }
            if (all) __hip_atomic_fetch_add(ra.census + 1, 1, __ATOMIC_RELAXED, __HIP_MEMORY_SCOPE_AGENT);
        }
        return;
    }
    const int lane = tid & 63;
    const int wave = __builtin_amdgcn_readfirstlane(tid >> 6);
    const bool fast = S::KMODE >= 0 ? S::KMODE == HIPETS_MODE_FAST : ra.whole_horizon != 0;
    const bool expectation = kLean ? false : md.propagation == HIPETS_PROP_EXPECTATION;
    int wg = blockIdx.x;
    if (!fast) {
        const int nwg = gridDim.x, x = wg & 7, slot = wg >> 3;
        wg = x * (nwg >> 3) + min(x, nwg & 7) + slot;
    }

    int domain = 0;
    if (fast) {
        for (int s = tid; s < ROWS; s += kThreads) {
            const int g = wg * ROWS + s;
            const int p = g / ra.pop, c = g - p * ra.pop;
            sm.rowid[s] = g < ra.B ? c * ra.P + p : -1;
        }
        if (!expectation) {
            if (ra.schedule) {
                for (int t = tid; t < ra.H; t += kThreads) sm.sched[t] = ra.schedule[(size_t)t * gridDim.x + wg];
            } else {
                const bool fixed = md.propagation == HIPETS_PROP_FIXED_MODEL;
                for (int t = tid; t < ra.H; t += kThreads)
                    sm.sched[t] = fast_member((unsigned)wg, gridDim.x, ra.fm_a, ra.fm_b, md.M, md.iid_members, ra.seed, ra.stream_id, fixed ? 0xFFFFFFFFu : (unsigned)t);
            }
        }
    } else {
        domain = wg / ra.groups;
        const int j0 = (wg % ra.groups) * ROWS;
        const long long* perm = ra.perm ? ra.perm + (long long)ra.t_begin * ra.perm_step : nullptr;
        if (perm && perm[(long long)domain * ra.rows_per_domain + j0] < 0) return;
        const PermKeys keys0 = ra.exchange ? ra.step_keys[ra.t_begin] : ra.perm_keys;
        for (int s = tid; s < ROWS; s += kThreads) {
            const int j = j0 + s;
            int rid = -1;
            if (j < ra.rows_per_domain) {
                const int jj = domain * ra.rows_per_domain + j;
                rid = perm ? (int)perm[jj] : (ra.perm_n ? (int)perm_apply((unsigned)jj, ra.perm_n, ra.perm_a, ra.perm_b, keys0) : jj);
            }
            sm.rowid[s] = rid;
        }
    }
    int member_dom = domain;
    if (!fast && ra.fast_members && !expectation)
        member_dom = __builtin_amdgcn_readfirstlane(
            ra.schedule ? ra.schedule[(size_t)ra.t_begin * gridDim.x + wg]
                        : fast_member((unsigned)wg, gridDim.x, ra.fm_a, ra.fm_b, md.M, md.iid_members, ra.seed, ra.stream_id,
                                      md.propagation == HIPETS_PROP_FIXED_MODEL ? 0xFFFFFFFFu : (unsigned)ra.t_begin));
    const bool persist = !fast && ra.exchange != nullptr;
    constexpr bool kRagged = S::WIDE && R == 2;
    int half_from = 0x7FFFFFFF;
    int n_logical = ra.n_logical;
    int hf_dom = 0, hf_tile = 0, hf_tpd = 1;
    if constexpr (kRagged) {
        if (persist && ra.ragged_last_turn) {
            const int G = (int)gridDim.x, n2 = ra.n_logical;
            const int turns2 = (n2 + G - 1) / G, full = (turns2 - 1) * G;
            if (turns2 >= 2) {
                hf_tpd = (ra.rows_per_domain + kTile - 1) / kTile;
                hf_dom = full / ra.groups;
                hf_tile = 2 * (full - hf_dom * ra.groups);
                const int rem = (hf_tpd - hf_tile) + (n2 / ra.groups - 1 - hf_dom) * hf_tpd;
                if (rem <= G) {
                    half_from = full;
                    n_logical = full + rem;
                }
            }
        }
    }
    auto logical_rows = [&](const int v, int& dom, int& j0, int& live) __attribute__((always_inline)) {
        if (!kRagged || v < half_from) {
            dom = v / ra.groups;
            j0 = (v - dom * ra.groups) * ROWS;
            live = ROWS;
        } else {
            int w = v - half_from + hf_tile;
            const int dd = w / hf_tpd;
            dom = hf_dom + dd;
            j0 = (w - dd * hf_tpd) * kTile;
            live = kTile;
        }
    };
    const bool poll_every = ra.poll_ticks < 1000;
    constexpr int kG = 2;
    const int NVP = (md.obs_dim + 1) / 2 + 1;
    const int NV = 2 * NVP;
    const unsigned nvp_magic = (unsigned)(0x100000000ull / (unsigned)NVP) + 1u;
    auto poll_gave_up = [&](const int spins, const long long t_poll) __attribute__((always_inline)) {
        if ((poll_every || (spins & 63) == 63) && (wall_clock64() - t_poll > ra.poll_ticks || *(volatile int*)ra.error_flag)) {
            *ra.error_flag = 1;
            return true;
        }
        return false;
    };
    auto fetch_late_total = [&](const int rid, const int t, float& tot, int& trm) __attribute__((always_inline)) {
        const unsigned long long* const src = ra.exchange + (size_t)rid * NV + (NV - 2);
        const unsigned want = ra.tag_base + (unsigned)t;
        const long long t_poll = wall_clock64();
        u32x4g g = {0u, 0u, 0u, 0u};
        for (int spins = 0;; ++spins) {
            pair_load_issue(g, src);
            asm volatile("s_waitcnt vmcnt(0)" : "+v"(g)::"memory");
            if (g[1] == want && g[3] == want) break;
            if (poll_gave_up(spins, t_poll)) break;
            __builtin_amdgcn_s_sleep(8);
        }
        tot = __uint_as_float(g[0]);
        trm = (int)g[2];
    };
    auto end_step_for_row = [&](const int s, const int rid, float tot, int trm, float r, const bool done, unsigned long long* const handover,
                                const unsigned tag) __attribute__((always_inline)) {
        if (trm) r = 0.f;
        trm = trm | (done ? 1 : 0);
        tot += r;
        sm.term[s] = trm;
        sm.tot[s] = tot;
        if (handover) pair_store(handover + (size_t)rid * NV + (NV - 2), __float_as_uint(tot), (unsigned)trm, tag);
        else if (persist) ra.totals[rid] = tot;
    };
    constexpr int kGT = (kLean && S::OUTC >= 4) ? 4 : kG;
    int xs[kG], xv[kG];
#pragma unroll
    for (int q = 0; q < kG; ++q) {
        const int i = tid + q * kThreads;
        xs[q] = i < ROWS * NVP ? i / NVP : -1;
        xv[q] = i < ROWS * NVP ? i - (i / NVP) * NVP : 0;
    }
    if constexpr (kB3) {
        f32x4* z = reinterpret_cast<f32x4*>(sm.buf0);
        const int n16 = (int)(2 * act_buf_bytes(ROWS, ld_k) / 16);
        for (int i = tid; i < n16; i += kThreads) z[i] = f32x4{0.f, 0.f, 0.f, 0.f};
    }
    const int nlv = deterministic ? 0 : lv_rows * md.out_dim;
    const bool norm = normalizer != HIPETS_NORM_NONE;
    double c_nm = 0.0, c_ns = 1.0;
    float c_lo = 0.f, c_hi = 0.f;
    int c_nd = 0, c_lm = 0;
    constexpr int kMetaWords = (int)(sizeof(LayerMeta) / sizeof(int));
    const int n_meta = md.n_layers * kMetaWords;
    if (norm && tid < md.in_dim) { c_nm = md.norm_mean[tid]; c_ns = md.norm_std[tid]; }
    if (tid < nlv) { c_lo = md.min_lv[tid]; c_hi = md.max_lv[tid]; }
    if (tid < md.obs_dim) c_nd = md.no_delta[tid];
    if (tid < n_meta) c_lm = reinterpret_cast<const int*>(md.layers)[tid];
    auto commit_constants = [&]() __attribute__((always_inline)) {
        if (norm && tid < md.in_dim) { sm.nmean[tid] = c_nm; sm.nstd[tid] = normalizer == HIPETS_NORM_F64 ? 1.0 / c_ns : c_ns; }
        if (tid < nlv) { sm.minlv[tid] = c_lo; sm.maxlv[tid] = c_hi; }
        if (tid < md.obs_dim) sm.nodelta[tid] = c_nd;
        if (tid < n_meta) reinterpret_cast<int*>(sm.lmeta)[tid] = c_lm;
        if (norm)
            for (int i = tid + kThreads; i < md.in_dim; i += kThreads) { sm.nmean[i] = md.norm_mean[i]; sm.nstd[i] = normalizer == HIPETS_NORM_F64 ? 1.0 / md.norm_std[i] : md.norm_std[i]; }
        for (int i = tid + kThreads; i < nlv; i += kThreads) { sm.minlv[i] = md.min_lv[i]; sm.maxlv[i] = md.max_lv[i]; }
        for (int i = tid + kThreads; i < md.obs_dim; i += kThreads) sm.nodelta[i] = md.no_delta[i];
    };
    lds_barrier();

    auto load_initial_state = [&]() __attribute__((always_inline)) {
        constexpr int kStage = 4;
        constexpr int kRowStage = (ROWS + kThreads - 1) / kThreads;
        const int n_st = ROWS * md.obs_dim;
        float tot0[kRowStage];
        int term0[kRowStage];
#pragma unroll
        for (int q = 0; q < kRowStage; ++q) {
            const int s = tid + q * kThreads;
            const int rid = s < ROWS ? sm.rowid[s] : -1;
            tot0[q] = (!fast && !persist && rid >= 0) ? ra.totals[rid] : 0.f;
            term0[q] = (!fast && !persist && rid >= 0) ? (int)ra.term[rid] : 0;
        }
        bool first = true;
        for (int base = tid; base < n_st || first; base += kStage * kThreads) {
            float v[kStage];
#pragma unroll
            for (int q = 0; q < kStage; ++q) {
                const int i = base + q * kThreads;
                v[q] = 0.f;
                if (i < n_st) {
                    const int s = i / md.obs_dim, d = i - s * md.obs_dim;
                    const int rid = sm.rowid[s];
                    if (fast) {
                        if (!kLean && ra.pop_env > 0) v[q] = rid >= 0 ? ra.s0[(size_t)((rid / ra.P) / ra.pop_env) * md.obs_dim + d] : 0.f;
                        else v[q] = ra.s0[d];
                    } else if (rid >= 0) {
                        if (!persist) v[q] = ra.state[(size_t)rid * md.obs_dim + d];
                        else if (!kLean && ra.pop_env > 0) v[q] = ra.s0[(size_t)((rid / ra.P) / ra.pop_env) * md.obs_dim + d];
                        else v[q] = ra.s0[d];
                    }
                }
            }
            if (first) {
                commit_constants();
#pragma unroll
                for (int q = 0; q < kRowStage; ++q) {
                    const int s = tid + q * kThreads;
                    if (s < ROWS) {
                        sm.tot[s] = tot0[q];
                        sm.term[s] = term0[q];
                        sm.lrew[s] = 0.f;
                        sm.pend[s] = 0;
                        sm.pend[ROWS + s] = 0;
                    }
                }
                first = false;
            }
#pragma unroll
            for (int q = 0; q < kStage; ++q) {
                const int i = base + q * kThreads;
                if (i < n_st) sm.state[i] = v[q];
            }
        }
    };

    const int nblk = (md.out_dim + 3) / 4;
    const int Kp0 = md.Kp0;
    Prof prof;
    prof.on = (!kLean || HIPETS_LEAN_PROF) && ra.phase_cycles != nullptr && wg == 0 && lane == 0;
    prof.slot = sm.prof + wave * 16;
    if (prof.on) {
#pragma unroll
        for (int i = 0; i < 15; ++i) prof.slot[i] = 0;
        prof.slot[15] = __builtin_amdgcn_s_getreg((4) | (0 << 6) | (15 << 11));
    }
    prof.t = prof.on ? clock64() : 0;

    constexpr int kPrefetch = 4;
    const int n_act = ROWS * md.act_dim;
    long long act_base[kPrefetch];
    int act_s[kPrefetch], act_a[kPrefetch];
#pragma unroll
    for (int q = 0; q < kPrefetch; ++q) {
        const int i = tid + q * kThreads;
        act_s[q] = i < n_act ? i / md.act_dim : -1;
        act_a[q] = i < n_act ? i - (i / md.act_dim) * md.act_dim : 0;
    }
    const bool magic_ok = ra.P > 1 && (unsigned long long)ra.B * (unsigned)ra.P < 0x100000000ull;
    const unsigned magic_p = (unsigned)(0x100000000ull / (unsigned)max(ra.P, 2)) + 1u;
    const int act_stride = ra.H * md.act_dim;
    const int* act_rows = sm.rowid;
    auto compute_act_base = [&]() __attribute__((always_inline)) {
#pragma unroll
        for (int q = 0; q < kPrefetch; ++q) {
            act_base[q] = -1;
            if (act_s[q] >= 0) {
                const int rid = act_rows[act_s[q]];
                const int cand = magic_ok ? (int)__umulhi((unsigned)rid, magic_p) : rid / ra.P;
                if (rid >= 0) act_base[q] = (long long)cand * act_stride + act_a[q];
            }
        }
    };
    compute_act_base();
    auto fetch_actions_rest = [&](const int t) __attribute__((always_inline)) {
        float* actn_t = sm.actn + (t & 1) * n_act;
        for (int i = tid + kPrefetch * kThreads; i < n_act; i += kThreads) {
            const int s = i / md.act_dim, a = i % md.act_dim;
            const int rid = act_rows[s];
            actn_t[i] = rid >= 0 ? ra.actions[((size_t)(rid / ra.P) * ra.H + t) * md.act_dim + a] : 0.f;
        }
    };
    auto fetch_actions_issue = [&](const int t, float (&av)[kPrefetch]) {
#pragma unroll
        for (int q = 0; q < kPrefetch; ++q) av[q] = act_base[q] >= 0 ? ra.actions[act_base[q] + (long long)t * md.act_dim] : 0.f;
    };
    auto fetch_actions_commit = [&](const int t, const float (&av)[kPrefetch]) {
        float* actn_t = sm.actn + (t & 1) * n_act;
#pragma unroll
        for (int q = 0; q < kPrefetch; ++q) {
            const int i = tid + q * kThreads;
            if (i < n_act) actn_t[i] = av[q];
        }
        fetch_actions_rest(t);
    };

    int kq = Kp0 >> 2;
    auto build_input_impl = [&](const int t, float* const dst, auto norm_tag, auto plain_tag) __attribute__((always_inline)) {
        constexpr int NORM = decltype(norm_tag)::value;
        constexpr bool PLAIN = decltype(plain_tag)::value;
        constexpr bool kByGroup = !kB3 && (PLAIN || !kLean);
        const float* actn_t = sm.actn + (t & 1) * n_act;
        if constexpr (kByGroup && PLAIN && NORM != HIPETS_NORM_F32) {
            const int d_s = kThreads / kq, d_c = kThreads - d_s * kq;
            int s = tid / kq, cq = tid - s * kq;
            for (int i = tid; i < ROWS * kq; i += kThreads) {
                const bool valid = sm.rowid[s] >= 0;
                float xv[4];
                double nm[4], ns[4];
                bool inb[4];
#pragma unroll
                for (int q = 0; q < 4; ++q) {
                    const int c = ((cq >> 2) << 4) + 4 * q + (cq & 3);
                    const int cc = min(c, md.in_dim - 1);
                    const float* src = cc < md.obs_in ? sm.state + s * md.obs_dim + cc : actn_t + s * md.act_dim + (cc - md.obs_in);
                    xv[q] = *src;
                    inb[q] = c < md.in_dim;
                    if constexpr (NORM == HIPETS_NORM_F64) { nm[q] = sm.nmean[cc]; ns[q] = sm.nstd[cc]; }
                }
                f32x4 v;
#pragma unroll
                for (int q = 0; q < 4; ++q) {
                    float x = xv[q];
                    if constexpr (NORM == HIPETS_NORM_F64) x = (float)(((double)x - nm[q]) * ns[q]);
                    v[q] = (inb[q] && valid) ? x : 0.f;
                }
                HIPETS_BOUND(s >= 0 && s < ROWS && 4 * cq + 3 < ld_in);
                *reinterpret_cast<f32x4*>(dst + s * ld_in + 4 * cq) = v;
                s += d_s;
                cq += d_c;
                if (cq >= kq) { cq -= kq; ++s; }
            }
            return;
        }
        for (int i = tid; i < ROWS * kq; i += kThreads) {
            const int s = i / kq, cq = i % kq;
            const bool valid = sm.rowid[s] >= 0;
            float v[4];
#pragma unroll
            for (int q = 0; q < 4; ++q) {
                const int c = kByGroup ? ((cq >> 2) << 4) + 4 * q + (cq & 3) : 4 * cq + q;
                const int cc = min(c, md.in_dim - 1);
                float x;
                if (cc < md.obs_in) {
                    if constexpr (PLAIN) x = sm.state[s * md.obs_dim + cc];
                    else x = processed_obs(sm.state + s * md.obs_dim, cc, obs_process, kLean ? nullptr : obs_columns(md));
                } else {
                    x = actn_t[s * md.act_dim + (cc - md.obs_in)];
                }
                if constexpr (NORM == HIPETS_NORM_F64) x = (float)(((double)x - sm.nmean[cc]) * sm.nstd[cc]);
                else if constexpr (NORM == HIPETS_NORM_F32) x = (x - (float)sm.nmean[cc]) / (float)sm.nstd[cc];
                v[q] = (c < md.in_dim && valid) ? x : 0.f;
            }
            HIPETS_BOUND(s >= 0 && s < ROWS && 4 * cq + 3 < ld_in);
            if constexpr (kB3) {
                u32x2 pc[kNP];
                split_x4<kNP>(f32x4{v[0], v[1], v[2], v[3]}, pc);
                char* row = reinterpret_cast<char*>(dst) + (size_t)s * ld_in * 4;
#pragma unroll
                for (int p = 0; p < kNP; ++p) *reinterpret_cast<u32x2*>(row + b3_offset<kNP>(4 * cq, p)) = pc[p];
            } else if constexpr (kByGroup) {
                *reinterpret_cast<f32x4*>(dst + s * ld_in + 4 * cq) = f32x4{v[0], v[1], v[2], v[3]};
            } else {
#pragma unroll
                for (int q = 0; q < 4; ++q) dst[s * ld_in + lds_col(4 * cq + q)] = v[q];
            }
        }
    };
    int in_rows = ROWS;
    auto build_input_cols = [&](const int t, float* const dst) __attribute__((always_inline)) {
        const float* actn_t = sm.actn + (t & 1) * n_act;
        constexpr int kU = 8;
        static_assert(ROWS % kU == 0, "row batches");
        for (int c = tid; c < Kp0; c += kThreads) {
            const bool inb = c < md.in_dim;
            const int cc = min(c, md.in_dim - 1);
            const double nm = sm.nmean[cc], ns = sm.nstd[cc];
            const bool from_state = cc < md.obs_in;
            const float* const src = from_state ? sm.state + cc : actn_t + (cc - md.obs_in);
            const int stride = from_state ? md.obs_dim : md.act_dim;
            float* const out = dst + lds_col(c);
            for (int s0_ = 0; s0_ < in_rows; s0_ += kU) {
                float x[kU];
                int rid[kU];
#pragma unroll
                for (int u = 0; u < kU; ++u) {
                    x[u] = src[(s0_ + u) * stride];
                    rid[u] = sm.rowid[s0_ + u];
                }
#pragma unroll
                for (int u = 0; u < kU; ++u) out[(s0_ + u) * ld_in] = (inb && rid[u] >= 0) ? (float)(((double)x[u] - nm) * ns) : 0.f;
            }
        }
    };
    auto build_input = [&](const int t, float* const dst) __attribute__((always_inline)) {
        using T = std::true_type;
        using F = std::false_type;
        if constexpr (kWide) {
            build_input_cols(t, dst);
            return;
        }
        const bool plain = obs_process == HIPETS_OBS_NONE;
        switch (normalizer) {
            case HIPETS_NORM_F64:
                if (plain) build_input_impl(t, dst, std::integral_constant<int, HIPETS_NORM_F64>{}, T{});
                else build_input_impl(t, dst, std::integral_constant<int, HIPETS_NORM_F64>{}, F{});
                break;
            case HIPETS_NORM_F32:
                if (plain) build_input_impl(t, dst, std::integral_constant<int, HIPETS_NORM_F32>{}, T{});
                else build_input_impl(t, dst, std::integral_constant<int, HIPETS_NORM_F32>{}, F{});
                break;
            default:
                if (plain) build_input_impl(t, dst, std::integral_constant<int, HIPETS_NORM_NONE>{}, T{});
                else build_input_impl(t, dst, std::integral_constant<int, HIPETS_NORM_NONE>{}, F{});
                break;
        }
    };
    const int bac_c = md.obs_in + (tid & 15);
    const bool bac_fast = S::FUSE && !kWide && Kp0 - md.obs_in <= 16;
    const bool bac_live = bac_fast && bac_c < md.in_dim;
    double bac_nm = 0.0, bac_ns = 0.0;
    const int bac_pos = lds_col(min(bac_c, Kp0 - 1));
    auto build_action_columns = [&](const int t, float* const dst) __attribute__((always_inline)) {
        const float* actn_t = sm.actn + (t & 1) * n_act;
        if (bac_fast) {
            if (wave != 0 && bac_c < Kp0) {
                constexpr int kRowsPerPass = (kThreads - 64) / 16;
                constexpr int kPasses = (ROWS + kRowsPerPass - 1) / kRowsPerPass;
                const int r0 = (tid - 64) >> 4;
                float x[kPasses];
                int rid[kPasses];
#pragma unroll
                for (int q = 0; q < kPasses; ++q) {
                    const int s = r0 + kRowsPerPass * q;
                    rid[q] = s < ROWS ? act_rows[s] : -1;
                    x[q] = (bac_live && s < ROWS) ? actn_t[s * md.act_dim + (bac_c - md.obs_in)] : 0.f;
                }
#pragma unroll
                for (int q = 0; q < kPasses; ++q) {
                    const int s = r0 + kRowsPerPass * q;
                    if (s < ROWS) dst[s * ld_in + bac_pos] = (bac_live && rid[q] >= 0) ? (float)(((double)x[q] - bac_nm) * bac_ns) : 0.f;
                }
            }
            return;
        }
        const int ntc = Kp0 - md.obs_in;
        for (int i = tid; i < ROWS * ntc; i += kThreads) {
            const int s = i / ntc, c = md.obs_in + (i - s * ntc);
            float v = 0.f;
            if (c < md.in_dim && act_rows[s] >= 0) {
                const float x = actn_t[s * md.act_dim + (c - md.obs_in)];
                v = (float)(((double)x - sm.nmean[c]) * sm.nstd[c]);
            }
            dst[s * ld_in + lds_col(c)] = v;
        }
    };

    {
        float av[kPrefetch];
        fetch_actions_issue(ra.t_begin, av);
        load_initial_state();
        fetch_actions_commit(ra.t_begin, av);
    }
    __syncthreads();
    if (bac_live) { bac_nm = sm.nmean[bac_c]; bac_ns = sm.nstd[bac_c]; }
    if constexpr (kB3) kq = sm.lmeta[0].Kp32 >> 2;
    build_input(ra.t_begin, sm.buf0);
    __syncthreads();
    prof.mark(0);
    float* step_in = sm.buf0;

    const int n_serve = persist ? (n_logical - wg + (int)gridDim.x - 1) / (int)gridDim.x : 1;
    const int n_seq = (ra.t_end - ra.t_begin) * n_serve;
    int stamp_seq = 0;
    (void)stamp_seq;
    const bool straight = S::FUSE && !kWide && persist && ra.n_logical == (int)gridDim.x && md.n_layers >= 4;
    int* const rows_a = sm.rowid;
    int* const rows_b = sm.pend + ROWS;
    int* const hop_flags = reinterpret_cast<int*>(sm.lrew);
    auto collect_straight = [&](const int t_next, const int* const rows, float* const dst) __attribute__((always_inline)) {
        const unsigned want = ra.tag_base + (unsigned)t_next;
        for (int base = 0; base < ROWS * NVP; base += kG * kThreads) {
            const unsigned long long* src[kG];
            u32x4g g[kG];
            int gs[kG], gv[kG];
            bool soft[kG], live[kG];
            double nm[kG][2], ns[kG][2];
#pragma unroll
            for (int q = 0; q < kG; ++q) {
                const int i = base + tid + q * kThreads;
                gs[q] = base == 0 ? xs[q] : (i < ROWS * NVP ? i / NVP : -1);
                gv[q] = base == 0 ? xv[q] : (i < ROWS * NVP ? i - (i / NVP) * NVP : 0);
                soft[q] = gv[q] == NVP - 1;
                src[q] = nullptr;
                live[q] = false;
                g[q] = u32x4g{0u, want, 0u, want};
                if (gs[q] >= 0) {
                    const int rid = rows[gs[q]];
                    if (rid >= 0) { src[q] = ra.exchange + (size_t)rid * NV + 2 * gv[q]; live[q] = true; }
                }
                const int d = soft[q] ? 0 : 2 * gv[q];
                const int i0 = max(0, min(ObsMap<S::OBSP>::col(d), md.obs_in - 1)), i1 = max(0, min(ObsMap<S::OBSP>::col(d + 1), md.obs_in - 1));
                nm[q][0] = sm.nmean[i0]; nm[q][1] = sm.nmean[i1];
                ns[q][0] = sm.nstd[i0]; ns[q][1] = sm.nstd[i1];
            }
            const long long t_poll = wall_clock64();
            for (int spins = 0;; ++spins) {
                static_assert(kG == 2, "the wait below names the two destinations");
                u32x4g got[kG];
                pair_load_issue(got[0], src[0] ? src[0] : ra.exchange);
                pair_load_issue(got[1], src[1] ? src[1] : ra.exchange);
                asm volatile("s_waitcnt vmcnt(0)" : "+v"(got[0]), "+v"(got[1])::"memory");
                bool ready = true;
#pragma unroll
                for (int q = 0; q < kG; ++q)
                    if (src[q]) {
                        g[q] = got[q];
                        if (got[q][1] == want && got[q][3] == want) src[q] = nullptr;
                        else if (!soft[q]) ready = false;
                    }
                if (ready) break;
                if (poll_gave_up(spins, t_poll)) break;
                __builtin_amdgcn_s_sleep(8);
            }
#pragma unroll
            for (int q = 0; q < kG; ++q)
                if (gs[q] >= 0) {
                    HIPETS_BOUND(gs[q] < ROWS && gv[q] >= 0 && gv[q] < NVP);
                    if (!soft[q]) {
                        using OM = ObsMap<S::OBSP>;
                        const int d = 2 * gv[q];
                        const float v0 = __uint_as_float(g[q][0]), v1 = __uint_as_float(g[q][2]);
                        float x0 = v0, x1 = v1;
                        if constexpr (OM::kTrigDim >= 0) {
                            if (d == OM::kTrigDim || d + 1 == OM::kTrigDim) {
                                const float tv = d == OM::kTrigDim ? v0 : v1;
                                const float sv = sinf(tv), cv = cosf(tv);
                                if (d == OM::kTrigDim) x0 = sv; else x1 = sv;
                                dst[gs[q] * ld_in + lds_col(OM::kCosCol)] = live[q] ? (float)(((double)cv - sm.nmean[OM::kCosCol]) * sm.nstd[OM::kCosCol]) : 0.f;
                            }
                        }
                        if constexpr (S::TERM == HIPETS_TERM_HOPPER) {
                            if (live[q] && hopper_pair_bad(d, v0, v1, true, d + 1 < md.obs_dim)) hop_flags[gs[q]] = 1;
                        }
                        const int c0 = OM::col(d), c1 = OM::col(d + 1);
                        sm.state[gs[q] * md.obs_dim + d] = v0;
                        if (c0 >= 0) dst[gs[q] * ld_in + lds_col(c0)] = live[q] ? (float)(((double)x0 - nm[q][0]) * ns[q][0]) : 0.f;
                        if (d + 1 < md.obs_dim) {
                            sm.state[gs[q] * md.obs_dim + d + 1] = v1;
                            if (c1 >= 0) dst[gs[q] * ld_in + lds_col(c1)] = live[q] ? (float)(((double)x1 - nm[q][1]) * ns[q][1]) : 0.f;
                        }
                    } else if (src[q]) {
                        sm.pend[gs[q]] = 1;
                    } else {
                        sm.tot[gs[q]] = __uint_as_float(g[q][0]);
                        sm.term[gs[q]] = (int)g[q][2];
                    }
                }
        }
        HIPETS_STAMP(2, t_next - 1);
    };
    auto dma_collect = [&](const unsigned want) __attribute__((always_inline)) {
        constexpr int CPR = kWide ? (((S::OUTC > 0 ? S::OUTC : 1) * 8 + 1) / 2 + 1 + 63) / 64 : 1;
        constexpr int kRowsPerWave = ROWS / kWaves;
        static_assert(ROWS % kWaves == 0 && kRowsPerWave * CPR <= 32, "row slots are dealt to the waves; one pending bit per (row, chunk)");
        const int n_main = (int)(act_bytes(ROWS, ld_in, ld_k) >> 10);
        char* const stage0 = reinterpret_cast<char*>(sm.buf0);
        HIPETS_BOUND(CPR == (NVP + 63) / 64 && (size_t)max(ROWS * CPR - n_main, 0) * 1024 <= stage_extra_bytes(ROWS, ld_in, ld_k, md.obs_dim));
        auto chunk_ptr = [&](const int c) __attribute__((always_inline)) { return c < n_main ? stage0 + ((size_t)c << 10) : sm.stage_x + ((size_t)(c - n_main) << 10); };
        auto lds_of = [&](const int c) __attribute__((always_inline)) { return (unsigned)__builtin_amdgcn_readfirstlane((int)(unsigned)(size_t)chunk_ptr(c)); };
        unsigned pending = 0;
        int rids[kRowsPerWave];
#pragma unroll
        for (int j = 0; j < kRowsPerWave; ++j) rids[j] = sm.rowid[wave + kWaves * j];
#pragma unroll
        for (int j = 0; j < kRowsPerWave; ++j) {
            const int s = wave + kWaves * j;
            const int rid = __builtin_amdgcn_readfirstlane(rids[j]);
            rids[j] = rid;
            if (rid >= 0) {
                const unsigned long long* const row = ra.exchange + (size_t)rid * NV;
#pragma unroll
                for (int k = 0; k < CPR; ++k) {
                    const int v = min(64 * k + lane, NVP - 1);
                    pair_dma_issue(row + 2 * v, lds_of(s * CPR + k));
                }
                pending |= ((1u << CPR) - 1u) << (j * CPR);
            } else {
                for (int d = lane; d < md.obs_dim; d += 64) sm.state[s * md.obs_dim + d] = 0.f;
                if (lane == 0) { sm.tot[s] = 0.f; sm.term[s] = 0; sm.pend[s] = 0; }
            }
        }
        const long long t_poll = wall_clock64();
        for (int spins = 0; pending; ++spins) {
            vmem_drain();
            unsigned still = 0;
#pragma unroll
            for (int j = 0; j < kRowsPerWave; ++j) {
                if (!((pending >> (j * CPR)) & ((1u << CPR) - 1u))) continue;
                const int s = wave + kWaves * j;
                u32x4g g[CPR];
#pragma unroll
                for (int k = 0; k < CPR; ++k) g[k] = *reinterpret_cast<const u32x4g*>(chunk_ptr(s * CPR + k) + lane * 16);
#pragma unroll
                for (int k = 0; k < CPR; ++k) {
                    if (!((pending >> (j * CPR + k)) & 1u)) continue;
                    const int v = 64 * k + lane;
                    const bool mine = v < NVP, soft = v == NVP - 1;
                    const bool ok = g[k][1] == want && g[k][3] == want;
                    HIPETS_BOUND(s < ROWS);
                    if (mine && !soft) {
                        if (ok) {
                            const int d = 2 * v;
                            sm.state[s * md.obs_dim + d] = __uint_as_float(g[k][0]);
                            if (d + 1 < md.obs_dim) sm.state[s * md.obs_dim + d + 1] = __uint_as_float(g[k][2]);
                        }
                    } else if (soft) {
                        if (ok) {
                            sm.tot[s] = __uint_as_float(g[k][0]);
                            sm.term[s] = (int)g[k][2];
                        }
                        sm.pend[s] = ok ? 0 : 1;
                    }
                    if (__builtin_amdgcn_ballot_w64(mine && !soft && !ok) != 0) {
                        still |= 1u << (j * CPR + k);
                        pair_dma_issue(ra.exchange + (size_t)rids[j] * NV + 2 * min(v, NVP - 1), lds_of(s * CPR + k));
                    }
                }
            }
            pending = still;
            if (!pending) break;
            if (poll_gave_up(spins, t_poll)) {
                vmem_drain();
                break;
            }
            __builtin_amdgcn_s_sleep(8);
        }
    };
    (void)dma_collect;

    bool one_tile = false;
    for (int q_seq = 0; q_seq < n_seq; ++q_seq) {
        stamp_seq = q_seq;
        const int t = ra.t_begin + q_seq / n_serve;
        const bool more = t + 1 < ra.t_end;
        const bool has_next = q_seq + 1 < n_seq;
        const int t_next = ra.t_begin + (q_seq + 1) / n_serve;
        const int v_next = wg + ((q_seq + 1) - ((q_seq + 1) / n_serve) * n_serve) * (int)gridDim.x;
        float av[kPrefetch];
        if (more && !persist) fetch_actions_issue(t + 1, av);
        unsigned long long* const handover = (more && persist) ? ra.exchange : nullptr;
        const unsigned long long handover_tag = (unsigned long long)(ra.tag_base + (unsigned)t + 1u) << 32;
        if constexpr (S::FUSE) {
            const int member = fast ? __builtin_amdgcn_readfirstlane(sm.sched[t]) : member_dom;
            float* cur = step_in;
            float* nxt = step_in == sm.buf0 ? sm.buf1 : sm.buf0;
            const int L = md.n_layers;
            const bool write_input = more && !persist && !kWide;
            const bool wide_fast_next = kWide && more && !persist;
            const bool prep_next = straight && more;
            int* const rows_nxt = sm.rowid == rows_a ? rows_b : rows_a;
            for (int l = 0; l + 1 < L; ++l) {
                prof.mark(12);
                if (l == 1 && prep_next && wave == kWaves - 1) {
                    for (int s = lane; s < ROWS; s += 64) {
                        const int j = (wg % ra.groups) * ROWS + s;
                        rows_nxt[s] = j < ra.rows_per_domain
                                          ? (int)perm_apply((unsigned)(domain * ra.rows_per_domain + j), ra.perm_n, ra.perm_a, ra.perm_b, ra.step_keys[t + 1]) : -1;
                    }
                }
                if (l == 2 && prep_next) {
                    act_rows = rows_nxt;
                    compute_act_base();
                    fetch_actions_issue(t + 1, av);
                }
                if (l == L - 2 && (write_input || prep_next || wide_fast_next)) fetch_actions_commit(t + 1, av);
                if constexpr (kRagged) {
                    if (one_tile) mlp_layer<1, S>(md, sm.lmeta, l, member, cur, nxt, wave, lane, prof, sm.part);
                    else mlp_layer<R, S>(md, sm.lmeta, l, member, cur, nxt, wave, lane, prof, sm.part);
                } else {
                    mlp_layer<R, S>(md, sm.lmeta, l, member, cur, nxt, wave, lane, prof, sm.part);
                }
                __syncthreads();
                prof.mark(8);
                float* tmp = cur; cur = nxt; nxt = tmp;
            }
            if (write_input || (prep_next && !kWide)) build_action_columns(t + 1, nxt);
            const float* const actn_t = sm.actn + (t & 1) * n_act;
            const unsigned handover_tg = (unsigned)(handover_tag >> 32);
            auto tail_prep = [&](FusedSlot& q, const int c, const int r) __attribute__((always_inline)) {
                const int s = r * kTile + (lane & 15);
                const int d0 = 8 * c + 2 * (lane >> 4);
                const int dA = min(d0, md.out_dim - 1), dB = min(d0 + 1, md.out_dim - 1);
                const int oA = min(d0, md.obs_dim - 1), oB = min(d0 + 1, md.obs_dim - 1);
                q.rid = sm.rowid[s];
                q.mxA = sm.maxlv[dA]; q.mxB = sm.maxlv[dB]; q.mnA = sm.minlv[dA]; q.mnB = sm.minlv[dB];
                q.pA = sm.state[s * md.obs_dim + oA]; q.pB = sm.state[s * md.obs_dim + oB];
                q.ndA = sm.nodelta[oA]; q.ndB = sm.nodelta[oB];
                using OM = ObsMap<S::OBSP>;
                const int iA = max(0, min(OM::col(d0), md.obs_in - 1)), iB = max(0, min(OM::col(d0 + 1), md.obs_in - 1));
                q.nmA = sm.nmean[iA]; q.nmB = sm.nmean[iB]; q.nsA = sm.nstd[iA]; q.nsB = sm.nstd[iB];
            };
            constexpr bool kPairDraws = !(MinWaves<R, S>::value == 2 && R == 2 && S::KMODE != HIPETS_MODE_FAST && (S::OBSP != HIPETS_OBS_NONE || S::REW == HIPETS_REW_LEARNED));
            auto unit_draw = [&](const int rid, const int c, float& n0, float& n1) __attribute__((always_inline)) {
                const int g = lane >> 4;
                const bool odd = (g & 1) != 0;
                const Philox4 r4 = philox4x32_10((uint32_t)rid, (uint32_t)t, (uint32_t)((8 * c + 2 * g) >> 2), (uint32_t)ra.stream_id, (uint32_t)ra.seed,
                                                 (uint32_t)(ra.seed >> 32) ^ (uint32_t)(ra.stream_id >> 32));
                box_muller(odd ? r4.z : r4.x, odd ? r4.w : r4.y, n0, n1);
            };
            auto tail_draw = [&](FusedSlot& qa, FusedSlot& qb, const int ca, const int cb, const bool two) __attribute__((always_inline)) {
#ifndef HIPETS_TIMING_NO_DRAWS
#define HIPETS_TIMING_NO_DRAWS 0
#endif
                if constexpr (HIPETS_TIMING_NO_DRAWS) {
                    qa.n0 = 0.37f + 1e-3f * (float)(qa.rid & 7);
                    qa.n1 = -0.81f;
                    qb.n0 = 0.37f + 1e-3f * (float)(qb.rid & 7);
                    qb.n1 = -0.81f;
                    return;
                }
                if constexpr (!kPairDraws) return;
                const int g = lane >> 4;
                const bool odd = (g & 1) != 0;
                const uint32_t k0 = (uint32_t)ra.seed, k1 = (uint32_t)(ra.seed >> 32) ^ (uint32_t)(ra.stream_id >> 32);
                if (!two) {
                    unit_draw(qa.rid, ca, qa.n0, qa.n1);
                    return;
                }
                const Philox4 r4 = philox4x32_10((uint32_t)(odd ? qb.rid : qa.rid), (uint32_t)t, (uint32_t)((8 * (odd ? cb : ca) + 2 * g) >> 2),
                                                 (uint32_t)ra.stream_id, k0, k1);
                const int partner = ((lane ^ 16) & 63) << 2;
                const uint32_t t0 = (uint32_t)__builtin_amdgcn_ds_bpermute(partner, (int)(odd ? r4.x : r4.z));
                const uint32_t t1 = (uint32_t)__builtin_amdgcn_ds_bpermute(partner, (int)(odd ? r4.y : r4.w));
                box_muller(odd ? t0 : r4.x, odd ? t1 : r4.y, qa.n0, qa.n1);
                box_muller(odd ? r4.z : t0, odd ? r4.w : t1, qb.n0, qb.n1);
            };
            auto tail_unit = [&](const FusedSlot& q, const f32x4 a, const int c, const int r) __attribute__((always_inline)) {
                const int g = lane >> 4, j = lane & 15;
                const int s = r * kTile + j;
                const int d0 = 8 * c + 2 * g;
                const int rid = q.rid;
                HIPETS_BOUND(s >= 0 && s < ROWS && r >= 0 && r < R && c >= 0 && 16 * c < 2 * md.out_dim + 16 && rid < ra.B);
                const bool okA = rid >= 0 && d0 < md.obs_dim, okB = rid >= 0 && d0 + 1 < md.obs_dim;
                const float mxA = q.mxA, mxB = q.mxB, mnA = q.mnA, mnB = q.mnB, pA = q.pA, pB = q.pB;
                const bool addA = md.target_is_delta && !q.ndA, addB = md.target_is_delta && !q.ndB;
                const double nmA = q.nmA, nmB = q.nmB, nsA = q.nsA, nsB = q.nsB;
                float n0 = q.n0, n1 = q.n1;
                if constexpr (!kPairDraws && !HIPETS_TIMING_NO_DRAWS) unit_draw(rid, c, n0, n1);
                float lvA = a[2], lvB = a[3];
                lvA = mxA - softplus_fast(mxA - lvA);
                lvB = mxB - softplus_fast(mxB - lvB);
                lvA = mnA + softplus_fast(lvA - mnA);
                lvB = mnB + softplus_fast(lvB - mnB);
                const float predA = a[0] + __builtin_amdgcn_sqrtf(exp_hw(lvA)) * n0;
                const float predB = a[1] + __builtin_amdgcn_sqrtf(exp_hw(lvB)) * n1;
                const float vA = predA + (addA ? pA : 0.f);
                const float vB = predB + (addB ? pB : 0.f);
                sm.state[okA ? s * md.obs_dim + d0 : (int)(sm.dump - sm.state)] = vA;
                sm.state[okB ? s * md.obs_dim + d0 + 1 : (int)(sm.dump - sm.state) + 1] = vB;
                if (write_input) {
                    using OM = ObsMap<S::OBSP>;
                    const int cA = OM::col(d0), cB = OM::col(d0 + 1);
                    float xA = vA, xB = vB;
                    if constexpr (OM::kTrigDim >= 0) {
                        if (c == 0) {
                            const bool trigA = d0 == OM::kTrigDim, trigB = d0 + 1 == OM::kTrigDim;
                            const float tv = trigA ? vA : vB;
                            const float sv = sinf(tv), cv = cosf(tv);
                            xA = trigA ? sv : xA;
                            xB = trigB ? sv : xB;
                            const bool okT = (trigA && okA) || (trigB && okB);
                            nxt[okT ? s * ld_k + lds_col(OM::kCosCol) : (int)(sm.dump - nxt) + 1] = (float)(((double)cv - sm.nmean[OM::kCosCol]) * sm.nstd[OM::kCosCol]);
                        }
                    }
                    nxt[(okA && cA >= 0) ? s * ld_k + lds_col(max(cA, 0)) : (int)(sm.dump - nxt) + 2] = (float)(((double)xA - nmA) * nsA);
                    nxt[(okB && cB >= 0) ? s * ld_k + lds_col(max(cB, 0)) : (int)(sm.dump - nxt) + 3] = (float)(((double)xB - nmB) * nsB);
                }
                const unsigned pubA = okA ? __float_as_uint(vA) : 0u, pubB = okB ? __float_as_uint(vB) : 0u;
                if (handover && okA) pair_store(handover + (size_t)rid * NV + d0, pubA, pubB, handover_tg);
                constexpr bool kLearnedRew = S::REW == HIPETS_REW_LEARNED;
                constexpr bool kAllDims = S::TERM == HIPETS_TERM_HOPPER;
                constexpr bool kRewLane = kLearnedRew && (S::TERM == HIPETS_TERM_NONE || kAllDims);
                if constexpr (kAllDims) {
                    if (!persist && hopper_pair_bad(d0, vA, vB, okA, okB)) sm.pend[(t & 1) * ROWS + s] = 1;
                }
                const int c_rew = kRewLane ? (md.obs_dim >> 3) : 0, g_rew = kRewLane ? ((md.obs_dim & 7) >> 1) : 0;
                if (c == c_rew) {
                    float st[4] = {0.f, 0.f, 0.f, 0.f};
                    float lrew = (md.obs_dim & 1) ? predB : predA;
                    if constexpr (!kRewLane) {
                        st[0] = okA ? vA : 0.f;
                        st[1] = okB ? vB : 0.f;
                        st[2] = __uint_as_float((unsigned)__builtin_amdgcn_ds_bpermute(((lane + 16) & 63) << 2, (int)pubA));
                        st[3] = __uint_as_float((unsigned)__builtin_amdgcn_ds_bpermute(((lane + 16) & 63) << 2, (int)pubB));
                        if constexpr (kLearnedRew)
                            lrew = __uint_as_float((unsigned)__builtin_amdgcn_ds_bpermute(((lane + 16 * ((md.obs_dim & 7) >> 1)) & 63) << 2, (int)__float_as_uint(lrew)));
                    }
                    if (g == g_rew && rid >= 0) {
                        float tot = sm.tot[s];
                        int trm = sm.term[s];
                        if (persist && sm.pend[s]) {
                            sm.pend[s] = 0;
                            fetch_late_total(rid, t, tot, trm);
                        }
                        float rwd;
                        if constexpr (kLearnedRew) rwd = lrew;
                        else rwd = reward_eval(st, actn_t + s * md.act_dim, 4, md.act_dim, S::REW, 0.f);
                        bool done = false;
                        if constexpr (kAllDims) {
                            if (persist) {
                                trm = trm | hop_flags[s];
                                hop_flags[s] = 0;
                            } else {
                                int* const flag = sm.pend + ((t & 1) ^ 1) * ROWS + s;
                                trm = trm | (t > ra.t_begin ? *flag : 0);
                                *flag = 0;
                            }
                        } else {
                            done = term_eval(st, 4, S::TERM);
                        }
                        end_step_for_row(s, rid, tot, trm, rwd, done, handover, handover_tg);
                    }
                }
            };
            auto tail_finish = [&]() __attribute__((always_inline)) {};
            const auto tail = make_tail(tail_prep, tail_draw, tail_unit, tail_finish);
            prof.mark(12);
            if constexpr (kRagged) {
                if (one_tile) mlp_output_layer_fused<1, S>(md, sm.lmeta, member, cur, wave, lane, prof, tail, sm.part);
                else mlp_output_layer_fused<R, S>(md, sm.lmeta, member, cur, wave, lane, prof, tail, sm.part);
            } else {
                mlp_output_layer_fused<R, S>(md, sm.lmeta, member, cur, wave, lane, prof, tail, sm.part);
            }
            if (prep_next) lds_barrier();
            else __syncthreads();
            prof.mark(8);
            HIPETS_STAMP(0, t);
            step_in = kWide ? sm.buf0 : nxt;
            if (wide_fast_next) {
                build_input(t + 1, step_in);
                __syncthreads();
            }
            if (prep_next) {
                HIPETS_STAMP(1, t);
                if (kWide) build_action_columns(t + 1, step_in);
                collect_straight(t + 1, rows_nxt, step_in);
                sm.rowid = rows_nxt;
                __syncthreads();
                HIPETS_STAMP(3, t);
                continue;
            }
            if (persist && has_next) {
                int nd, nj0, nlive;
                logical_rows(v_next, nd, nj0, nlive);
                if constexpr (kRagged) {
                    one_tile = nlive < ROWS;
                    in_rows = nlive;
                }
                for (int s = tid; s < ROWS; s += kThreads) {
                    const int j = nj0 + s;
                    sm.rowid[s] = (s < nlive && j < ra.rows_per_domain)
                                      ? (int)perm_apply((unsigned)(nd * ra.rows_per_domain + j), ra.perm_n, ra.perm_a, ra.perm_b, ra.step_keys[t_next]) : -1;
                    sm.lrew[s] = 0.f;
                }
                __syncthreads();
            }
        } else {
            const int n_run = expectation ? md.M : 1;
            float* result = nullptr;
            int member = 0;
            for (int mi = 0; mi < n_run; ++mi) {
                if (expectation) member = mi;
                else if (fast) member = __builtin_amdgcn_readfirstlane(sm.sched[t]);
                else member = member_dom;
                if (mi > 0) {
                    build_input(t, sm.buf0);
                    __syncthreads();
                }
                float* cur = sm.buf0;
                float* nxt = sm.buf1;
                for (int l = 0; l < md.n_layers; ++l) {
                    prof.mark(12);
                    if constexpr (kB3) {
                        mlp_layer_b3<R, S>(md, sm.lmeta, l, member, cur, nxt, wave, lane);
                        __syncthreads();
                    } else {
                        mlp_layer<R, S>(md, sm.lmeta, l, member, cur, nxt, wave, lane, prof);
                        __syncthreads();
                    }
                    prof.mark(8);
                    float* tmp = cur; cur = nxt; nxt = tmp;
                }
                result = cur;

                if (expectation) {
                    for (int i = tid; i < ROWS * md.out_total; i += kThreads) {
                        const int s = i / md.out_total, c = i % md.out_total;
                        float v = result[s * ld_k + c];
                        if (!deterministic && c >= md.out_dim) {
                            const int d = c - md.out_dim;
                            const int bd = (lv_rows > 1 ? member * md.out_dim : 0) + d;
                            const float mx = sm.maxlv[bd], mn = sm.minlv[bd];
                            v = clamp_logvar(v, mn, mx);
                        }
                        sm.expacc[i] = mi == 0 ? v : sm.expacc[i] + v;
                    }
                    __syncthreads();
                }
            }

            HIPETS_STAMP(0, t);
            auto sample_impl = [&](auto expect_tag, auto mode_tag) __attribute__((always_inline)) {
                constexpr bool EXPECT = decltype(expect_tag)::value;
                constexpr int MODE = decltype(mode_tag)::value;
                const float inv_m = 1.0f / (float)md.M;
                const float* lvmin = sm.minlv + (lv_rows > 1 ? member * md.out_dim : 0);
                const float* lvmax = sm.maxlv + (lv_rows > 1 ? member * md.out_dim : 0);
                for (int item = tid; item < ROWS * nblk; item += kThreads) {
                    const int s = item / nblk, blk = item % nblk;
                    const int rid = sm.rowid[s];
                    HIPETS_BOUND(s < ROWS && rid < ra.B && 4 * blk < md.out_dim + 4 && md.out_total <= ld_k);
                    if (rid < 0) continue;
                    float nrm[4] = {0.f, 0.f, 0.f, 0.f};
                    if constexpr (MODE == 1) {
    #pragma unroll
                        for (int q = 0; q < 4; ++q) {
                            const int d = min(blk * 4 + q, md.out_dim - 1);
                            nrm[q] = ra.eps[((size_t)t * ra.B + rid) * md.out_dim + d];
                        }
                    } else if constexpr (MODE == 2) {
                        rollout_normals4(rid, t, blk, ra.seed, ra.stream_id, nrm);
                    }
                    float pred[4], prev[4];
    #pragma unroll
                    for (int q = 0; q < 4; ++q) {
                        const int d = min(blk * 4 + q, md.out_dim - 1);
                        float mean, lv = 0.f;
                        if constexpr (EXPECT) {
                            mean = sm.expacc[s * md.out_total + d] / (float)md.M;
                            if constexpr (MODE != 0) lv = sm.expacc[s * md.out_total + md.out_dim + d] / (float)md.M;
                        } else {
                            mean = result[s * ld_k + d];
                            if constexpr (MODE != 0) {
                                lv = result[s * ld_k + md.out_dim + d];
                                const float mx = lvmax[d], mn = lvmin[d];
                                lv = clamp_logvar(lv, mn, mx);
                            }
                        }
                        if constexpr (MODE != 0) pred[q] = mean + __builtin_amdgcn_sqrtf(exp_hw(lv)) * nrm[q];
                        else pred[q] = mean;
                        const int do_ = min(d, md.obs_dim - 1);
                        prev[q] = (md.target_is_delta && !sm.nodelta[do_]) ? sm.state[s * md.obs_dim + do_] : 0.f;
                    }
                    (void)inv_m;
                    unsigned pub[4] = {0u, 0u, 0u, 0u};
    #pragma unroll
                    for (int q = 0; q < 4; ++q) {
                        const int d = blk * 4 + q;
                        if (d < md.obs_dim) {
                            const float nobs = pred[q] + prev[q];
                            sm.state[s * md.obs_dim + d] = nobs;
                            pub[q] = __float_as_uint(nobs);
                            if (trace_next_obs) trace_next_obs[((size_t)t * ra.B + rid) * md.obs_dim + d] = nobs;
                        } else if (d < md.out_dim) {
                            sm.lrew[s] = pred[q];
                        }
                    }
                    if (handover) {
                        const unsigned tg = (unsigned)(handover_tag >> 32);
                        if (blk * 4 < md.obs_dim) pair_store(handover + (size_t)rid * NV + blk * 4, pub[0], pub[1], tg);
                        if (blk * 4 + 2 < md.obs_dim) pair_store(handover + (size_t)rid * NV + blk * 4 + 2, pub[2], pub[3], tg);
                    }
                }
            };
            {
                using T = std::true_type;
                using F = std::false_type;
                const int mode = kLean ? 2 : (deterministic ? 0 : (ra.eps != nullptr ? 1 : (ra.use_philox ? 2 : 0)));
                if (expectation) {
                    if (mode == 0) sample_impl(T{}, std::integral_constant<int, 0>{});
                    else if (mode == 1) sample_impl(T{}, std::integral_constant<int, 1>{});
                    else sample_impl(T{}, std::integral_constant<int, 2>{});
                } else {
                    if (mode == 0) sample_impl(F{}, std::integral_constant<int, 0>{});
                    else if (mode == 1) sample_impl(F{}, std::integral_constant<int, 1>{});
                    else sample_impl(F{}, std::integral_constant<int, 2>{});
                }
            }
            if (more && !persist) fetch_actions_commit(t + 1, av);
            __syncthreads();
            prof.mark(9);

            for (int s = tid; s < ROWS; s += kThreads) {
                const int rid = sm.rowid[s];
                if (rid >= 0) {
                    int so = s;
                    if constexpr (!kLean) asm volatile("" : "+v"(so));
                    const float* st = sm.state + so * md.obs_dim;
                    const float* ac = sm.actn + (t & 1) * ROWS * md.act_dim + so * md.act_dim;
                    float tot = sm.tot[s];
                    int trm = sm.term[s];
                    if (persist && sm.pend[s]) {
                        sm.pend[s] = 0;
                        fetch_late_total(rid, t, tot, trm);
                    }
                    const FormTables* forms = kLean ? nullptr : form_tables(md);
                    if constexpr (!kLean) asm volatile("" : "+s"(forms));
                    float r = reward_eval(st, ac, md.obs_dim, md.act_dim, reward_fn, sm.lrew[s], forms);
                    const bool done = term_eval(st, md.obs_dim, term_fn, forms);
                    if (reward_fn == HIPETS_REW_TERMS) r = reward_alive_bonus(r, done, forms);
                    if (trace_rewards) trace_rewards[(size_t)t * ra.B + rid] = r;
                    end_step_for_row(s, rid, tot, trm, r, done, handover, (unsigned)(handover_tag >> 32));
                }
                if (persist && has_next) {
                    const int j = (v_next % ra.groups) * ROWS + s;
                    sm.rowid[s] = j < ra.rows_per_domain
                                      ? (int)perm_apply((unsigned)((v_next / ra.groups) * ra.rows_per_domain + j), ra.perm_n, ra.perm_a, ra.perm_b, ra.step_keys[t_next]) : -1;
                    sm.lrew[s] = 0.f;
                }
            }
            if (more && !persist) build_input(t + 1, sm.buf0);
            __syncthreads();
            prof.mark(10);

        }
        HIPETS_STAMP(1, t);
        if (persist && has_next) {
            {
                int nj0, nlive;
                logical_rows(v_next, domain, nj0, nlive);
            }
            member_dom = domain;
            compute_act_base();
            float av2[kPrefetch];
            fetch_actions_issue(t_next, av2);
            const unsigned long long tag = (unsigned long long)(ra.tag_base + (unsigned)t_next) << 32;
            if (t_next == ra.t_begin) {
                for (int i = tid; i < ROWS * md.obs_dim; i += kThreads) {
                    const int s_ = i / md.obs_dim;
                    const int rid_ = sm.rowid[s_];
                    const size_t env_off = (!kLean && ra.pop_env > 0 && rid_ >= 0) ? (size_t)((rid_ / ra.P) / ra.pop_env) * md.obs_dim : 0;
                    sm.state[i] = rid_ >= 0 ? ra.s0[env_off + (i - s_ * md.obs_dim)] : 0.f;
                }
                for (int s_ = tid; s_ < ROWS; s_ += kThreads) {
                    sm.tot[s_] = 0.f;
                    sm.term[s_] = 0;
                }
            } else if constexpr (kWide) {
                dma_collect((unsigned)(tag >> 32));
            } else
            for (int base = 0; base < ROWS * NVP; base += kGT * kThreads) {
                const unsigned long long* src[kGT];
                u32x4g g[kGT];
                int gs[kGT], gv[kGT];
                bool soft[kGT];
                const unsigned want = (unsigned)(tag >> 32);
#pragma unroll
                for (int q = 0; q < kGT; ++q) {
                    const int i = base + tid + q * kThreads;
                    const int i_row = (int)__umulhi((unsigned)i, nvp_magic);
                    gs[q] = (base == 0 && q < kG) ? xs[q < kG ? q : 0] : (i < ROWS * NVP ? i_row : -1);
                    gv[q] = (base == 0 && q < kG) ? xv[q < kG ? q : 0] : (i < ROWS * NVP ? i - i_row * NVP : 0);
                    soft[q] = gv[q] == NVP - 1;
                    src[q] = nullptr;
                    g[q] = u32x4g{0u, want, 0u, want};
                    if (gs[q] >= 0) {
                        const int rid = sm.rowid[gs[q]];
                        if (rid >= 0) src[q] = ra.exchange + (size_t)rid * NV + 2 * gv[q];
                    }
                }
                const long long t_poll = wall_clock64();
                for (int spins = 0;; ++spins) {
                    static_assert(kGT == 2 || kGT == 4, "the wait below names its destinations");
                    u32x4g got[kGT];
#pragma unroll
                    for (int q = 0; q < kGT; ++q) pair_load_issue(got[q], src[q] ? src[q] : ra.exchange);
                    if constexpr (kGT == 2) asm volatile("s_waitcnt vmcnt(0)" : "+v"(got[0]), "+v"(got[1])::"memory");
                    else asm volatile("s_waitcnt vmcnt(0)" : "+v"(got[0]), "+v"(got[1]), "+v"(got[2]), "+v"(got[3])::"memory");
                    bool ready = true;
#pragma unroll
                    for (int q = 0; q < kGT; ++q)
                        if (src[q]) {
                            g[q] = got[q];
                            if (got[q][1] == want && got[q][3] == want) src[q] = nullptr;
                            else if (!soft[q]) ready = false;
                        }
                    if (ready) break;
                    if (poll_gave_up(spins, t_poll)) break;
                    __builtin_amdgcn_s_sleep(8);
                }
#pragma unroll
                for (int q = 0; q < kGT; ++q)
                    if (gs[q] >= 0) {
                        HIPETS_BOUND(gs[q] < ROWS && gv[q] >= 0 && gv[q] < NVP);
                        if (!soft[q]) {
                            const int d = 2 * gv[q];
                            const float v0 = __uint_as_float(g[q][0]), v1 = __uint_as_float(g[q][2]);
                            if constexpr (S::FUSE && S::TERM == HIPETS_TERM_HOPPER) {
                                if (sm.rowid[gs[q]] >= 0 && hopper_pair_bad(d, v0, v1, true, d + 1 < md.obs_dim)) hop_flags[gs[q]] = 1;
                            }
                            sm.state[gs[q] * md.obs_dim + d] = v0;
                            if (d + 1 < md.obs_dim) sm.state[gs[q] * md.obs_dim + d + 1] = v1;
                        } else if (src[q]) {
                            sm.pend[gs[q]] = 1;
                        } else {
                            sm.tot[gs[q]] = __uint_as_float(g[q][0]);
                            sm.term[gs[q]] = (int)g[q][2];
                        }
                    }
            }
            HIPETS_STAMP(2, t);
            fetch_actions_commit(t_next, av2);
            __syncthreads();
            build_input(t_next, step_in);
            __syncthreads();
            HIPETS_STAMP(3, t);
        }
    }

    if constexpr (S::FUSE && S::TERM == HIPETS_TERM_HOPPER) {
        if (ra.t_end > ra.t_begin && !persist)
            for (int s = tid; s < ROWS; s += kThreads) sm.term[s] |= sm.pend[((ra.t_end - 1) & 1) * ROWS + s];
    }
    for (int s = tid; s < ROWS; s += kThreads) {
        const int rid = sm.rowid[s];
        if (rid < 0 || persist) continue;
        ra.totals[rid] = sm.tot[s];
        if (!fast && !persist) ra.term[rid] = (unsigned char)sm.term[s];
    }
    if (prof.on) {
#pragma unroll
        for (int i = 0; i < 16; ++i) ra.phase_cycles[wave * 16 + i] += prof.slot[i];
    }
    if (!fast && !persist) {
        for (int i = tid; i < ROWS * md.obs_dim; i += kThreads) {
            const int s = i / md.obs_dim, d = i % md.obs_dim;
            const int rid = sm.rowid[s];
            if (rid >= 0) ra.state[(size_t)rid * md.obs_dim + d] = sm.state[i];
        }
    }
}

}
```

mbrl-lib_amd/csrc/rollout_inst.inc:

```
#ifndef HIPETS_PART
#error "define HIPETS_PART (1..4) and HIPETS_R before including rollout_inst.inc"
#endif
#define HIPETS_CAT2_(a, b) a##b
#define HIPETS_CAT2(a, b) HIPETS_CAT2_(a, b)
#define HIPETS_FN(suffix) HIPETS_CAT2(HIPETS_CAT2(rollout_instance_r, HIPETS_R), suffix)
#include <hip/hip_runtime.h>

#include "launch.hpp"
#include "rollout.hpp"

#define HIPETS_LEAN_SHAPES(X) HIPETS_CAT2(HIPETS_LEAN_SHAPES_R, HIPETS_R)(X)
#define HIPETS_B3_SHAPES(X) HIPETS_CAT2(HIPETS_B3_SHAPES_R, HIPETS_R)(X)
#define HIPETS_BF16_SHAPES(X) HIPETS_CAT2(HIPETS_BF16_SHAPES_R, HIPETS_R)(X)

#if HIPETS_PART == 2
#define HIPETS_LEAN_MODE HIPETS_MODE_FAST
#define HIPETS_SPEC_FN HIPETS_FN(_fast)
#else
#define HIPETS_LEAN_MODE HIPETS_MODE_EXACT
#define HIPETS_SPEC_FN HIPETS_FN(_exact)
#endif
#define HIPETS_TRY_SHAPE(HC, OC, RW, TM, OB) \
    if (lean_shape_is(md, HC, OC, RW, TM, OB)) return &rec<LeanSpec<HC, OC, RW, TM, OB, HIPETS_LEAN_MODE>>();
#define HIPETS_TRY_PREC(PREC, HC, OC, RW, TM) \
    if (b3_shape_is(md, HC, OC, RW, TM)) return &rec<KSpec<HIPETS_ACT_SILU, HC, OC, HIPETS_NORM_F64, HIPETS_OBS_NONE, RW, TM, HIPETS_LEAN_MODE, PREC>>();
#define HIPETS_TRY_B3(HC, OC, RW, TM) HIPETS_TRY_PREC(HIPETS_PREC_BF16X3, HC, OC, RW, TM)
#define HIPETS_TRY_BF16(HC, OC, RW, TM) HIPETS_TRY_PREC(HIPETS_PREC_BF16, HC, OC, RW, TM)
#define HIPETS_TRY_HID(HC) \
    if (hid_static_is(md, HC)) return &rec<KSpec<HIPETS_ACT_SILU, HC>>();

namespace hipets {

namespace {
template <class S>
KernelRec& rec() {
    static KernelRec r{reinterpret_cast<const void*>(&rollout_kernel<HIPETS_R, S>)};
    return r;
}
}

KernelRec* HIPETS_FN(_fast)(RolloutInstance pick, const ModelDev& md);
KernelRec* HIPETS_FN(_gen)();
KernelRec* HIPETS_FN(_gens)();

#if HIPETS_PART == 3
KernelRec* HIPETS_FN(_gen)() { return &rec<KSpec<-1>>(); }
#endif
#if HIPETS_PART == 4
KernelRec* HIPETS_FN(_gens)() { return &rec<KSpec<HIPETS_ACT_SILU>>(); }
#endif

#if HIPETS_PART <= 2
KernelRec* HIPETS_SPEC_FN(const RolloutInstance pick, const ModelDev& md) {
    if (pick == RolloutInstance::b3) {
        HIPETS_B3_SHAPES(HIPETS_TRY_B3)
    } else if (pick == RolloutInstance::bf16) {
        HIPETS_BF16_SHAPES(HIPETS_TRY_BF16)
    } else {
        HIPETS_LEAN_SHAPES(HIPETS_TRY_SHAPE)
    }
    return nullptr;
}
#endif

#if HIPETS_PART == 1
KernelRec* HIPETS_FN()(const ModelDev& md, const RolloutArgs& ra, hipError_t* why) {
    const RolloutInstance pick = pick_rollout_instance(md, ra, HIPETS_R);
    *why = hipErrorNotSupported;
    switch (pick) {
        case RolloutInstance::lean:
        case RolloutInstance::lean_wide:
        case RolloutInstance::b3:
        case RolloutInstance::bf16: return (ra.whole_horizon ? HIPETS_FN(_fast) : HIPETS_FN(_exact))(pick, md);
        case RolloutInstance::hidden_static: HIPETS_HID_STATIC_SHAPES(HIPETS_TRY_HID) break;
        case RolloutInstance::generic_silu: return HIPETS_FN(_gens)();
        case RolloutInstance::generic: return HIPETS_FN(_gen)();
        case RolloutInstance::no_b3:
        case RolloutInstance::no_bf16: break;
        case RolloutInstance::no_wide: *why = hipErrorInvalidConfiguration; break;
    }
    return nullptr;
}
#endif

}
```

mbrl-lib_amd/hipets/_lib.py:

```python
from __future__ import annotations

import ctypes as C
import os

_HERE = os.path.dirname(os.path.abspath(__file__))
LIB_PATH = os.environ.get("HIPETS_LIB") or os.path.join(_HERE, "libhipets.so")

ABI_VERSION = 9
MAX_LAYERS = 8

ACT = {"relu": 0, "silu": 1, "leaky_relu": 2, "tanh": 3, "sigmoid": 4}
PROP = {"random_model": 0, "fixed_model": 1, "expectation": 2}
OBS = {"none": 0, "halfcheetah": 1, "cartpole_pets": 2, "columns": 3}
REW = {None: 0, "learned": 0, "cartpole": 1, "cartpole_pets": 2, "inverted_pendulum": 3, "halfcheetah": 4, "pusher": 5, "none": 6,
       "terms": 7}
TERM = {"no_termination": 0, "cartpole": 1, "inverted_pendulum": 2, "hopper": 3, "walker2d": 4, "ant": 5, "humanoid": 6,
        "box": 7}
NORM = {"none": 0, "f32": 1, "f64": 2}
ENSEMBLE = {"gaussian_mlp": 0, "basic_ensemble": 1}
PREC = {"f32": 0, "bf16x3": 1, "bf16": 2}
MODE_EXACT, MODE_FAST, MODE_DEVICE = 0, 1, 2
MODES = {"exact": MODE_EXACT, "fast": MODE_FAST, "device": MODE_DEVICE}
TERM_FN = {"linear": 0, "square": 1, "abs": 2, "sin": 3, "cos": 4, "exp": 5, "sqrt": 6}
TERM_SRC = {"obs": 0, "act": 1, "group": 2, "const": 3}
TERM_OP = {"add": 0, "mul": 1, "div": 2}
TERM_MAX_LEVEL = 2


def term_word(fn: int, op: int = 0, level: int = 0) -> int:
    return int(fn) | (int(op) << 8) | (int(level) << 16)


def term_word_fields(word: int):
    return word & 0xFF, (word >> 8) & 0xFF, (word & 0xFFFFFFFF) >> 16
BOX_LO_OPEN, BOX_HI_OPEN = 1, 2
MAX_REWARD_TERMS, MAX_TERM_INTERVALS = 64, 64
COL_FN = {"id": 0, "sin": 1, "cos": 2}
MAX_OBS_COLUMNS = 512
KERNEL_CLASSES = ("generic", "hidden_static", "fused", "wide", "bf16")


class RewardTermC(C.Structure):
    _fields_ = [("fn", C.c_int32), ("source", C.c_int32), ("i", C.c_int32), ("j", C.c_int32), ("c", C.c_float), ("w", C.c_float)]


class TermIntervalC(C.Structure):
    _fields_ = [("dim", C.c_int32), ("flags", C.c_int32), ("lo", C.c_float), ("hi", C.c_float)]


class ObsColumnC(C.Structure):
    _fields_ = [("dim", C.c_int32), ("fn", C.c_int32)]


class ModelDesc(C.Structure):
    _fields_ = [
        ("obs_dim", C.c_int32), ("act_dim", C.c_int32), ("in_dim", C.c_int32), ("out_dim", C.c_int32),
        ("hid", C.c_int32), ("n_layers", C.c_int32), ("ensemble_size", C.c_int32), ("n_members", C.c_int32),
        ("members", C.POINTER(C.c_int32)),
        ("activation", C.c_int32), ("leaky_slope", C.c_float), ("propagation", C.c_int32),
        ("deterministic", C.c_int32), ("obs_process", C.c_int32), ("reward_fn", C.c_int32),
        ("termination_fn", C.c_int32), ("target_is_delta", C.c_int32), ("learned_rewards", C.c_int32),
        ("n_no_delta", C.c_int32), ("no_delta", C.POINTER(C.c_int32)),
        ("normalizer", C.c_int32), ("norm_mean", C.POINTER(C.c_double)), ("norm_std", C.POINTER(C.c_double)),
        ("min_logvar", C.POINTER(C.c_float)), ("max_logvar", C.POINTER(C.c_float)),
        ("weights", C.POINTER(C.c_void_p)), ("biases", C.POINTER(C.c_void_p)),
        ("ensemble_kind", C.c_int32),
        ("precision", C.c_int32),
        ("reward_terms", C.POINTER(RewardTermC)), ("term_intervals", C.POINTER(TermIntervalC)),
        ("n_reward_terms", C.c_int32), ("n_term_intervals", C.c_int32),
        ("reward_bias", C.c_float), ("alive_bonus", C.c_float), ("term_require_finite", C.c_int32),
    ]


class RolloutOpts(C.Structure):
    _fields_ = [
        ("mode", C.c_int32),
        ("perms", C.c_void_p), ("eps", C.c_void_p),
        ("seed", C.c_uint64), ("stream_id", C.c_uint64),
        ("member_schedule", C.c_void_p), ("fast_eps", C.c_void_p),
        ("trace_next_obs", C.c_void_p), ("trace_rewards", C.c_void_p),
        ("rows_per_group", C.c_int32),
        ("phase_cycles", C.c_void_p),
        ("no_sample", C.c_int32),
        ("rows_per_member", C.c_int32),
        ("n_env", C.c_int32),
        ("generic_kernel", C.c_int32),
        ("member_schedule_len", C.c_int32),
        ("perm_stream_id", C.c_uint64),
    ]


class CemParams(C.Structure):
    _fields_ = [
        ("population_size", C.c_int32), ("horizon", C.c_int32), ("act_dim", C.c_int32),
        ("num_iterations", C.c_int32), ("elite_num", C.c_int32), ("alpha", C.c_double),
        ("return_mean_elites", C.c_int32), ("clipped_normal", C.c_int32), ("unbiased_var", C.c_int32),
    ]


class IcemParams(C.Structure):
    _fields_ = [
        ("population_size", C.c_int32), ("horizon", C.c_int32), ("act_dim", C.c_int32),
        ("num_iterations", C.c_int32), ("elite_num", C.c_int32), ("keep_elite_size", C.c_int32),
        ("population_size_module", C.c_int32), ("return_mean_elites", C.c_int32), ("alpha", C.c_double),
        ("population_decay_factor", C.c_double), ("colored_noise_exponent", C.c_double),
    ]


class PlanTrace(C.Structure):
    _fields_ = [("populations", C.c_void_p), ("values", C.c_void_p), ("mus", C.c_void_p), ("dispersions", C.c_void_p),
                ("elite_idx", C.c_void_p), ("max_rows", C.c_int32)]


_PLANET_TENSORS = ("w_embed", "b_embed", "w_ih", "b_ih", "w_hh", "b_hh", "w_prior1", "b_prior1", "w_prior2", "b_prior2",
                   "w_rew1", "b_rew1", "w_rew2", "b_rew2", "w_rew3", "b_rew3")


class PlanetDesc(C.Structure):
    _fields_ = [("latent_size", C.c_int32), ("action_size", C.c_int32), ("belief_size", C.c_int32), ("hidden_size", C.c_int32),
                ("min_std", C.c_float)] + [(n, C.c_void_p) for n in _PLANET_TENSORS]


class PlanetOpts(C.Structure):
    _fields_ = [("eps", C.c_void_p), ("seed", C.c_uint64), ("stream_id", C.c_uint64), ("no_sample", C.c_int32),
                ("trace_latent", C.c_void_p), ("trace_belief", C.c_void_p), ("trace_rewards", C.c_void_p), ("phase_cycles", C.c_void_p),
                ("n_env", C.c_int32)]


class TrainDesc(C.Structure):
    _fields_ = [
        ("ensemble_size", C.c_int32), ("n_layers", C.c_int32), ("in_dim", C.c_int32), ("hid", C.c_int32), ("out_dim", C.c_int32),
        ("activation", C.c_int32), ("leaky_slope", C.c_float), ("max_batch", C.c_int32),
        ("weights", C.POINTER(C.c_void_p)), ("biases", C.POINTER(C.c_void_p)),
        ("exp_avg_w", C.POINTER(C.c_void_p)), ("exp_avg_b", C.POINTER(C.c_void_p)),
        ("exp_avg_sq_w", C.POINTER(C.c_void_p)), ("exp_avg_sq_b", C.POINTER(C.c_void_p)),
        ("min_logvar", C.c_void_p), ("max_logvar", C.c_void_p),
        ("lr", C.c_double), ("beta1", C.c_double), ("beta2", C.c_double), ("eps", C.c_double), ("weight_decay", C.c_double),
        ("steps_per_launch", C.c_int32),
    ]


_P = C.c_void_p
SYMBOLS = {
    "hipets_abi_version": (C.c_int, []),
    "hipets_last_error": (C.c_char_p, []),
    "hipets_last_error_kind": (C.c_int, []),
    "hipets_create": (C.c_int, [C.c_int, C.POINTER(_P)]),
    "hipets_destroy": (None, [_P]),
    "hipets_set_model": (C.c_int, [_P, C.POINTER(ModelDesc), _P]),
    "hipets_set_model_columns": (C.c_int, [_P, C.POINTER(ModelDesc), C.POINTER(ObsColumnC), C.c_int32, _P]),
    "hipets_rollout": (C.c_int, [_P, _P, _P, C.c_int32, C.c_int32, C.c_int32, C.POINTER(RolloutOpts), _P, _P]),
    "hipets_step": (C.c_int, [_P, _P, _P, C.c_int32, C.POINTER(RolloutOpts), _P, _P, _P, _P]),
    "hipets_fast_geometry": (C.c_int, [_P, C.c_int32, C.c_int32, C.c_int32, C.c_int32, C.POINTER(C.c_int32), C.POINTER(C.c_int32)]),
    "hipets_kernel_class": (C.c_int, [_P, C.c_int32, C.c_int32, C.c_int32, C.c_int32, C.c_int32, C.POINTER(C.c_int32), C.POINTER(C.c_int32)]),
    "hipets_fast_schedule": (C.c_int, [_P, C.c_int32, C.c_int32, C.c_uint64, C.c_uint64, _P, _P]),
    "hipets_fast_normals": (C.c_int, [_P, C.c_int32, C.c_int32, C.c_uint64, C.c_uint64, _P, _P]),
    "hipets_device_perms": (C.c_int, [_P, C.c_int32, C.c_int32, C.c_uint64, C.c_uint64, _P, _P]),
    "hipets_set_plan_mode": (C.c_int, [_P, C.c_int32]),
    "hipets_set_persistent": (C.c_int, [_P, C.c_int32]),
    "hipets_set_handover_timeout": (C.c_int, [_P, C.c_double]),
    "hipets_check_async_error": (C.c_int, [_P, C.POINTER(C.c_int32)]),
    "hipets_set_plan_trace": (C.c_int, [_P, C.POINTER(PlanTrace)]),
    "hipets_cem_sample": (C.c_int, [_P, C.POINTER(CemParams), _P, _P, _P, _P, _P, C.c_uint64, C.c_uint64, _P, _P]),
    "hipets_cem_refit": (C.c_int, [_P, C.POINTER(CemParams), _P, _P, _P, _P, _P, _P, _P, _P]),
    "hipets_cem_refit_elites": (C.c_int, [_P, C.POINTER(CemParams), _P, _P, _P, _P, _P, _P, _P, _P]),
    "hipets_gather_rows": (C.c_int, [_P, C.c_int32, C.c_int32, _P, _P, _P, _P]),
    "hipets_mppi_sample": (C.c_int, [_P, C.c_int32, C.c_int32, C.c_int32, C.c_double, _P, _P, _P, _P, _P, C.c_uint64, C.c_uint64, _P, _P]),
    "hipets_mppi_update": (C.c_int, [_P, C.c_int32, C.c_int32, C.c_int32, C.c_double, _P, _P, _P, _P]),
    "hipets_icem_sample": (C.c_int, [_P, C.c_int32, C.c_int32, C.c_int32, C.c_double, _P, _P, _P, _P, _P, C.c_uint64, C.c_uint64, _P, _P]),
    "hipets_icem_shift": (C.c_int, [_P, C.c_int32, C.c_int32, C.c_int32, _P, _P, _P, _P, C.c_uint64, C.c_uint64, _P, _P]),
    "hipets_plan_cem": (C.c_int, [_P, C.POINTER(CemParams), _P, _P, _P, _P, C.c_int32, C.c_uint64, C.c_uint64, _P, _P]),
    "hipets_plan_cem_batched": (C.c_int, [_P, C.POINTER(CemParams), C.c_int32, _P, _P, _P, _P, C.c_int32, C.c_uint64, C.c_uint64, _P, _P]),
    "hipets_plan_mppi": (C.c_int, [_P, C.c_int32, C.c_int32, C.c_int32, C.c_int32, C.c_double, C.c_double, _P, _P, _P, _P, C.c_int32,
                                   C.c_uint64, C.c_uint64, _P]),
    "hipets_plan_mppi_batched": (C.c_int, [_P, C.c_int32, C.c_int32, C.c_int32, C.c_int32, C.c_double, C.c_double, C.c_int32, _P, _P, _P, _P,
                                           C.c_int32, C.c_uint64, C.c_uint64, _P]),
    "hipets_plan_icem_batched": (C.c_int, [_P, C.POINTER(IcemParams), C.c_int32, _P, _P, _P, _P, C.c_int32, _P, _P, C.c_int32, C.c_uint64,
                                           C.c_uint64, _P, _P]),
    "hipets_plan_icem": (C.c_int, [_P, C.POINTER(IcemParams), _P, _P, _P, _P, C.c_int32, _P, _P, C.c_int32, C.c_uint64, C.c_uint64,
                                   _P, _P]),
    "hipets_comm_unique_id": (C.c_int, [_P]),
    "hipets_comm_init": (C.c_int, [_P, _P, C.c_int32, C.c_int32]),
    "hipets_comm_destroy": (C.c_int, [_P]),
    "hipets_comm_info": (C.c_int, [_P, C.POINTER(C.c_int32), C.POINTER(C.c_int32)]),
    "hipets_plan_cem_sharded": (C.c_int, [_P, C.POINTER(CemParams), _P, _P, _P, _P, C.c_int32, C.c_uint64, C.c_uint64, _P, _P]),
    "hipets_plan_mppi_sharded": (C.c_int, [_P, C.c_int32, C.c_int32, C.c_int32, C.c_int32, C.c_double, C.c_double, _P, _P, _P, _P, C.c_int32,
                                           C.c_uint64, C.c_uint64, _P]),
    "hipets_plan_icem_sharded": (C.c_int, [_P, C.POINTER(IcemParams), _P, _P, _P, _P, C.c_int32, _P, _P, C.c_int32, C.c_uint64, C.c_uint64,
                                           _P, _P]),
    "hipets_planet_set_model": (C.c_int, [_P, C.POINTER(PlanetDesc), _P]),
    "hipets_planet_rollout": (C.c_int, [_P, _P, _P, _P, C.c_int32, C.c_int32, C.c_int32, C.POINTER(PlanetOpts), _P, _P]),
    "hipets_plan_planet_cem": (C.c_int, [_P, C.POINTER(CemParams), _P, _P, _P, _P, _P, C.c_int32, C.c_uint64, C.c_uint64, _P, _P]),
    "hipets_plan_planet_cem_batched": (C.c_int, [_P, C.POINTER(CemParams), C.c_int32, _P, _P, _P, _P, _P, C.c_int32, C.c_uint64, C.c_uint64,
                                                 _P, _P]),
    "hipets_plan_planet_mppi_batched": (C.c_int, [_P, C.c_int32, C.c_int32, C.c_int32, C.c_int32, C.c_double, C.c_double, C.c_int32, _P, _P,
                                                  _P, _P, _P, C.c_int32, C.c_uint64, C.c_uint64, _P]),
    "hipets_plan_planet_icem_batched": (C.c_int, [_P, C.POINTER(IcemParams), C.c_int32, _P, _P, _P, _P, C.c_int32, _P, _P, _P, C.c_int32,
                                                  C.c_uint64, C.c_uint64, _P, _P]),
    "hipets_train_steps": (C.c_int, [_P, C.POINTER(TrainDesc), _P, _P, C.c_int64, _P, _P, C.c_int32, C.c_int64, _P, _P, _P]),
    "hipets_train_eval": (C.c_int, [_P, C.POINTER(TrainDesc), _P, _P, C.c_int64, _P, _P, _P, _P]),
    "hipets_timing_enable": (C.c_int, [_P, C.c_int32]),
    "hipets_timing_read": (C.c_int, [_P, C.POINTER(C.c_int64), C.POINTER(C.c_double), C.c_int32]),
}

_lib = None


COMM_ID_BYTES = 128


ERR_NONE, ERR_INVALID_ARGUMENT, ERR_RUNTIME, ERR_TIMEOUT = 0, 1, 2, 3


class HipetsError(RuntimeError):

    def __init__(self, message="", kind: int = ERR_RUNTIME):
        super().__init__(message)
        self.kind = kind


def load():
    global _lib
    if _lib is not None:
        return _lib
    if not os.path.exists(LIB_PATH):
        raise HipetsError(
            f"{LIB_PATH} not found: build it with `python __graft_entry__.py` (hipcc --offload-arch=gfx950). "
            "hipets has no CPU fallback."
        )
    lib = C.CDLL(LIB_PATH)
    for name, (res, args) in SYMBOLS.items():
        fn = getattr(lib, name)
        fn.restype = res
        fn.argtypes = args
    if lib.hipets_abi_version() != ABI_VERSION:
        raise HipetsError(f"libhipets ABI {lib.hipets_abi_version()} != binding ABI {ABI_VERSION}")
    _lib = lib
    return lib


def check(rc: int):
    if rc != 0:
        lib = load()
        raise HipetsError(lib.hipets_last_error().decode(), lib.hipets_last_error_kind())
```

mbrl-lib_amd/hipets/engine.py:

```python
from __future__ import annotations

import ctypes as C
from typing import Dict, Optional

import numpy as np
import torch

from . import _lib
from ._lib import CemParams, HipetsError, ModelDesc, PlanTrace, RolloutOpts, TrainDesc
from .model import BoxTermination, ModelSpec, ObsColumns, RewardTerms


def _ptr(t: Optional[torch.Tensor]):
    return None if t is None else C.c_void_p(t.data_ptr())


def _stream(device) -> C.c_void_p:
    return C.c_void_p(torch.cuda.current_stream(device).cuda_stream)


def _check_dev(t: torch.Tensor, dtype, device, name: str, shape=None, numel=None):
    if not isinstance(t, torch.Tensor) or t.device != device:
        raise ValueError(f"{name} must be a tensor on {device}")
    if t.dtype != dtype:
# ... 152 lines not shown
        pop, H, A = actions.shape
        if A != self.spec.act_dim:
            raise ValueError(f"action dim {A} != model act_dim {self.spec.act_dim}")
        s0 = np.ascontiguousarray(np.asarray(s0, dtype=np.float32).reshape(-1))
        if s0.shape[0] != self.spec.obs_dim * max(1, n_env):
            raise ValueError(f"initial_state has {s0.shape[0]} values, expected n_env x obs_dim = {max(1, n_env)} x {self.spec.obs_dim}")
        if n_env > 1 and (mode not in ("fast", "device") or pop % n_env):
            raise ValueError("batched rollouts (n_env > 1) need mode='fast' or 'device' and a population divisible by n_env")
        B = pop * num_particles
        o = RolloutOpts()
        o.n_env = int(n_env)
        o.generic_kernel = int(generic_kernel)
        if mode not in _lib.MODES:
            raise ValueError("mode must be 'exact', 'fast' or 'device'")
        o.mode = _lib.MODES[mode]
        if mode == "device" and (perms is not None or eps is not None or members is not None):
            raise ValueError("mode='device' draws its permutations and eps in-kernel: perms / eps / members must be None")
        if members is not None:
            if mode != "exact" or perms is not None:
                raise ValueError("members= (explicit per-row member maps) is an EXACT-mode input, exclusive with perms=")
            want = (B,) if self.spec.propagation == "fixed_model" else (H, B)
            if tuple(members.shape) != want:
                raise ValueError(f"members must have shape {want}")
            perms, o.rows_per_member = member_slots(members.reshape(-1, B), len(self.spec.members), dev)
        elif perms is not None:
            _check_dev(perms, torch.int64, dev, "perms")
            want = (B,) if self.spec.propagation == "fixed_model" else (H, B)
            if tuple(perms.shape) != want:
                raise ValueError(f"perms must have shape {want}")
        if eps is not None:
            _check_dev(eps, torch.float32, dev, "eps", (H, B, self.spec.out_dim))
        if mode == "exact":
            o.perms, o.eps = _ptr(perms), _ptr(eps)
        elif mode == "fast":
            o.fast_eps = _ptr(eps)
            if member_schedule is not None:
                nwg, _ = self.fast_geometry(pop, num_particles, H, rows_per_group)
                _check_dev(member_schedule, torch.int32, dev, "member_schedule", (H, nwg))
                o.member_schedule, o.member_schedule_len = _ptr(member_schedule), int(member_schedule.numel())
        o.seed, o.stream_id = int(seed) & (2**64 - 1), int(stream_id) & (2**64 - 1)
        if trace_next_obs is not None:
            _check_dev(trace_next_obs, torch.float32, dev, "trace_next_obs", (H, B, self.spec.obs_dim))
            o.trace_next_obs = _ptr(trace_next_obs)
        if trace_rewards is not None:
            _check_dev(trace_rewards, torch.float32, dev, "trace_rewards", (H, B))
            o.trace_rewards = _ptr(trace_rewards)
        o.rows_per_group = int(rows_per_group)
        if phase_cycles is not None:
            _check_dev(phase_cycles, torch.int64, dev, "phase_cycles", (8, 16))
            o.phase_cycles = _ptr(phase_cycles)
        if out is None:
            out = torch.empty(pop, dtype=torch.float32, device=dev)
        else:
            _check_dev(out, torch.float32, dev, "out", (pop,))
        with torch.cuda.device(dev):
            _lib.check(self._lib.hipets_rollout(self._h, _ptr(actions), s0.ctypes.data_as(C.c_void_p), pop, H,
                                                num_particles, C.byref(o), _ptr(out), _stream(dev)))
        return out

    def step(self, obs: torch.Tensor, actions: torch.Tensor, *, mode: str = "fast", sample: bool = True,
             perm: Optional[torch.Tensor] = None, eps: Optional[torch.Tensor] = None, seed: int = 0, stream_id: int = 0,
             member_schedule: Optional[torch.Tensor] = None, rows_per_group: int = 0,
             members: Optional[torch.Tensor] = None, perm_stream_id: int = 0, generic_kernel=False):
        if self.spec is None:
            raise HipetsError("Engine.set_model() has not been called")
        dev = self.device
        B = int(obs.shape[0])
        _check_dev(obs, torch.float32, dev, "obs", (B, self.spec.obs_dim))
        _check_dev(actions, torch.float32, dev, "actions", (B, self.spec.act_dim))
        o = RolloutOpts()
        if mode not in _lib.MODES:
            raise ValueError("mode must be 'exact', 'fast' or 'device'")
        o.mode = _lib.MODES[mode]
        o.seed, o.stream_id = int(seed) & (2**64 - 1), int(stream_id) & (2**64 - 1)
        o.rows_per_group = int(rows_per_group)
        o.no_sample = int(not sample)
        o.perm_stream_id = int(perm_stream_id) & (2**64 - 1)
        o.generic_kernel = int(generic_kernel)
        if mode == "device":
            if perm is not None or eps is not None or members is not None:
                raise ValueError("mode='device' draws its permutation and eps in-kernel")
        elif mode == "exact":
            if members is not None:
                if perm is not None or tuple(members.shape) != (B,):
                    raise ValueError("members= must be int64 [B], exclusive with perm=")
                perm, o.rows_per_member = member_slots(members.reshape(1, B), len(self.spec.members), dev)
                o.perms = _ptr(perm)
            elif perm is not None:
                _check_dev(perm, torch.int64, dev, "perm", (B,))
                o.perms = _ptr(perm)
            if sample and not self.spec.deterministic:
                if eps is None:
                    raise ValueError("EXACT step with sample=True needs eps [B, out_dim]")
                _check_dev(eps, torch.float32, dev, "eps", numel=B * self.spec.out_dim)
                o.eps = _ptr(eps)
        else:
            if eps is not None:
                _check_dev(eps, torch.float32, dev, "eps", numel=B * self.spec.out_dim)
                o.fast_eps = _ptr(eps)
            if member_schedule is not None:
                _check_dev(member_schedule, torch.int32, dev, "member_schedule")
                o.member_schedule, o.member_schedule_len = _ptr(member_schedule), int(member_schedule.numel())
        next_obs = torch.empty_like(obs)
        rewards = torch.empty(B, dtype=torch.float32, device=dev)
        dones = torch.empty(B, dtype=torch.uint8, device=dev)
        with torch.cuda.device(dev):
            _lib.check(self._lib.hipets_step(self._h, _ptr(obs), _ptr(actions), B, C.byref(o), _ptr(next_obs), _ptr(rewards),
                                             _ptr(dones), _stream(dev)))
        return next_obs, rewards.view(B, 1), dones.view(B, 1).bool()

    def fast_geometry(self, pop: int, num_particles: int, horizon: int, rows_per_group: int = 0):
        nwg, r = C.c_int32(), C.c_int32()
        _lib.check(self._lib.hipets_fast_geometry(self._h, pop, num_particles, horizon, rows_per_group, C.byref(nwg),
                                                  C.byref(r)))
        return nwg.value, r.value

    def kernel_class(self, pop: int, num_particles: int, horizon: int, mode: str = "device", rows_per_group: int = 0):
        cls, r = C.c_int32(), C.c_int32()
        _lib.check(self._lib.hipets_kernel_class(self._h, pop, num_particles, horizon, _lib.MODES[mode], int(rows_per_group), C.byref(cls),
                                                 C.byref(r)))
        return _lib.KERNEL_CLASSES[cls.value], r.value

    def fast_schedule(self, horizon: int, n_workgroups: int, seed: int = 0, stream_id: int = 0) -> torch.Tensor:
        out = torch.empty(horizon, n_workgroups, dtype=torch.int32, device=self.device)
        with torch.cuda.device(self.device):
            _lib.check(self._lib.hipets_fast_schedule(self._h, horizon, n_workgroups, int(seed) & (2**64 - 1),
                                                      int(stream_id) & (2**64 - 1), _ptr(out), _stream(self.device)))
        return out

    def fast_normals(self, horizon: int, batch: int, seed: int = 0, stream_id: int = 0) -> torch.Tensor:
        out = torch.empty(horizon, batch, self.spec.out_dim, dtype=torch.float32, device=self.device)
        with torch.cuda.device(self.device):
            _lib.check(self._lib.hipets_fast_normals(self._h, horizon, batch, int(seed) & (2**64 - 1),
                                                     int(stream_id) & (2**64 - 1), _ptr(out), _stream(self.device)))
        return out

    def device_perms(self, horizon: int, batch: int, seed: int = 0, stream_id: int = 0) -> torch.Tensor:
        fixed = self.spec.propagation == "fixed_model"
        out = torch.empty(1 if fixed else horizon, batch, dtype=torch.int64, device=self.device)
        with torch.cuda.device(self.device):
            _lib.check(self._lib.hipets_device_perms(self._h, horizon, batch, int(seed) & (2**64 - 1), int(stream_id) & (2**64 - 1),
                                                     _ptr(out), _stream(self.device)))
        return out[0] if fixed else out

    def set_plan_mode(self, mode: str):
        if mode not in ("fast", "device"):
            raise ValueError("plan mode must be 'fast' or 'device'")
        _lib.check(self._lib.hipets_set_plan_mode(self._h, _lib.MODES[mode]))
        self.plan_mode = mode

    def set_persistent(self, on: bool = True):
        _lib.check(self._lib.hipets_set_persistent(self._h, int(bool(on))))

    def synchronize(self):
        torch.cuda.synchronize(self.device)

    def set_handover_timeout(self, seconds: float = 0.2):
        _lib.check(self._lib.hipets_set_handover_timeout(self._h, float(seconds)))

    def check_async_error(self) -> bool:
        flag = C.c_int32(0)
        _lib.check(self._lib.hipets_check_async_error(self._h, C.byref(flag)))
        return bool(flag.value)

    def set_plan_trace(self, iters: int = 0, max_rows: int = 0, horizon: int = 0, act_dim: int = 0, elite_num: int = 0, n_env: int = 1):
        if iters <= 0:
            _lib.check(self._lib.hipets_set_plan_trace(self._h, None))
            self._trace = None
            return None
        dev = self.device
        tr = {"populations": torch.zeros(iters, max_rows, horizon, act_dim, device=dev),
              "values": torch.zeros(iters, max_rows, device=dev),
              "mus": torch.zeros((iters, horizon, act_dim) if n_env == 1 else (iters, n_env, horizon, act_dim), device=dev),
              "dispersions": torch.zeros((iters, horizon, act_dim) if n_env == 1 else (iters, n_env, horizon, act_dim), device=dev),
              "elite_idx": torch.zeros((iters, max(1, elite_num)) if n_env == 1 else (iters, n_env, max(1, elite_num)), dtype=torch.int32,
                                       device=dev)}
        t = PlanTrace()
        t.populations, t.values, t.mus = tr["populations"].data_ptr(), tr["values"].data_ptr(), tr["mus"].data_ptr()
        t.dispersions, t.elite_idx, t.max_rows = tr["dispersions"].data_ptr(), tr["elite_idx"].data_ptr(), int(max_rows)
        _lib.check(self._lib.hipets_set_plan_trace(self._h, C.byref(t)))
        self._trace = tr
        return tr

    @staticmethod
    def cem_params(population_size, horizon, act_dim, num_iterations, elite_num, alpha, return_mean_elites=False,
                   clipped_normal=False, unbiased_var=True) -> CemParams:
        p = CemParams()
        p.population_size, p.horizon, p.act_dim = int(population_size), int(horizon), int(act_dim)
        p.num_iterations, p.elite_num, p.alpha = int(num_iterations), int(elite_num), float(alpha)
        p.return_mean_elites, p.clipped_normal, p.unbiased_var = int(return_mean_elites), int(clipped_normal), int(unbiased_var)
        return p

    def cem_sample(self, p: CemParams, mu, dispersion, lower, upper, population, z=None, seed=0, stream_id=0):
        dev = self.device
        D = p.horizon * p.act_dim
        for n_, t in (("mu", mu), ("dispersion", dispersion), ("lower", lower), ("upper", upper)):
            _check_dev(t, torch.float32, dev, n_, numel=D)
        _check_dev(population, torch.float32, dev, "population", numel=p.population_size * D)
        if z is not None:
            _check_dev(z, torch.float32, dev, "z", numel=p.population_size * D)
        with torch.cuda.device(dev):
            _lib.check(self._lib.hipets_cem_sample(self._h, C.byref(p), _ptr(mu), _ptr(dispersion), _ptr(lower), _ptr(upper),
                                                   _ptr(z), int(seed) & (2**64 - 1), int(stream_id) & (2**64 - 1),
                                                   _ptr(population), _stream(dev)))
        return population

    def cem_refit(self, p: CemParams, values, population, mu, dispersion, best_value, best_solution, elite_idx=None, elites=None):
        dev = self.device
        D = p.horizon * p.act_dim
        _check_dev(values, torch.float32, dev, "values", (p.population_size,))
        _check_dev(population, torch.float32, dev, "population", numel=p.population_size * D)
        for n_, t in (("mu", mu), ("dispersion", dispersion), ("best_solution", best_solution)):
            _check_dev(t, torch.float32, dev, n_, numel=D)
        _check_dev(best_value, torch.float32, dev, "best_value", (1,))
        if elite_idx is not None:
            _check_dev(elite_idx, torch.int32, dev, "elite_idx", (p.elite_num,))
        if elites is not None:
            _check_dev(elites, torch.int32, dev, "elites", (p.elite_num,))
            lo, hi = int(elites.min()), int(elites.max())
            if lo < 0 or hi >= p.population_size:
                raise ValueError(f"elites must index the population [0, {p.population_size}): got {lo} .. {hi}")
            with torch.cuda.device(dev):
                _lib.check(self._lib.hipets_cem_refit_elites(self._h, C.byref(p), _ptr(values), _ptr(population), _ptr(elites), _ptr(mu),
                                                             _ptr(dispersion), _ptr(best_value), _ptr(best_solution), _stream(dev)))
            if elite_idx is not None:
                elite_idx.copy_(elites)
            return
        with torch.cuda.device(dev):
            _lib.check(self._lib.hipets_cem_refit(self._h, C.byref(p), _ptr(values), _ptr(population), _ptr(mu), _ptr(dispersion),
                                                  _ptr(best_value), _ptr(best_solution), _ptr(elite_idx), _stream(dev)))

    def gather_rows(self, src: torch.Tensor, index: torch.Tensor, out: torch.Tensor):
        dev = self.device
        rows, dim = int(index.numel()), int(out.numel() // max(1, index.numel()))
        _check_dev(src, torch.float32, dev, "src")
        _check_dev(index, torch.int32, dev, "index")
        _check_dev(out, torch.float32, dev, "out", numel=rows * dim)
        with torch.cuda.device(dev):
            _lib.check(self._lib.hipets_gather_rows(self._h, rows, dim, _ptr(src), _ptr(index), _ptr(out), _stream(dev)))
        return out

    def mppi_sample(self, pop, H, A, beta, mean, past_action, lower, upper, population, z=None, seed=0, stream_id=0):
        dev = self.device
        for n_, t in (("mean", mean), ("lower", lower), ("upper", upper)):
            _check_dev(t, torch.float32, dev, n_, numel=H * A)
        _check_dev(past_action, torch.float32, dev, "past_action", numel=A)
        _check_dev(population, torch.float32, dev, "population", numel=pop * H * A)
        if z is not None:
            _check_dev(z, torch.float32, dev, "z", numel=pop * H * A)
        with torch.cuda.device(dev):
            _lib.check(self._lib.hipets_mppi_sample(self._h, pop, H, A, float(beta), _ptr(mean), _ptr(past_action), _ptr(lower),
                                                    _ptr(upper), _ptr(z), int(seed) & (2**64 - 1), int(stream_id) & (2**64 - 1),
                                                    _ptr(population), _stream(dev)))
        return population

    def mppi_update(self, pop, H, A, gamma, values, population, mean):
        dev = self.device
        _check_dev(values, torch.float32, dev, "values", (pop,))
        _check_dev(population, torch.float32, dev, "population", numel=pop * H * A)
        _check_dev(mean, torch.float32, dev, "mean", numel=H * A)
        with torch.cuda.device(dev):
            _lib.check(self._lib.hipets_mppi_update(self._h, pop, H, A, float(gamma), _ptr(values), _ptr(population), _ptr(mean),
                                                    _stream(dev)))
        return mean

    def icem_sample(self, n, H, A, exponent, mu, var, lower, upper, population, normals=None, seed=0, stream_id=0):
        dev = self.device
        for n_, t in (("mu", mu), ("var", var), ("lower", lower), ("upper", upper)):
            _check_dev(t, torch.float32, dev, n_, numel=H * A)
        _check_dev(population, torch.float32, dev, "population")
        if population.numel() < n * H * A:
            raise ValueError("population buffer too small")
        if normals is not None:
            _check_dev(normals, torch.float32, dev, "normals", (2, n, A, H // 2 + 1))
        with torch.cuda.device(dev):
            _lib.check(self._lib.hipets_icem_sample(self._h, n, H, A, float(exponent), _ptr(mu), _ptr(var), _ptr(lower), _ptr(upper),
                                                    _ptr(normals), int(seed) & (2**64 - 1), int(stream_id) & (2**64 - 1),
                                                    _ptr(population), _stream(dev)))
        return population

    def icem_shift(self, keep, H, A, kept, mu, var, out, end_noise=None, seed=0, stream_id=0):
        dev = self.device
        _check_dev(kept, torch.float32, dev, "kept", numel=keep * H * A)
        _check_dev(out, torch.float32, dev, "out", numel=keep * H * A)
        for n_, t in (("mu", mu), ("var", var)):
            _check_dev(t, torch.float32, dev, n_, numel=H * A)
        if end_noise is not None:
            _check_dev(end_noise, torch.float32, dev, "end_noise", numel=keep * A)
        with torch.cuda.device(dev):
            _lib.check(self._lib.hipets_icem_shift(self._h, keep, H, A, _ptr(kept), _ptr(mu), _ptr(var), _ptr(end_noise),
                                                   int(seed) & (2**64 - 1), int(stream_id) & (2**64 - 1), _ptr(out), _stream(dev)))
        return out

    def _plan_args(self, tensors, n_env: int = 1, s0=None, latent0=None, belief0=None, sharded: bool = False, seed: int = 0, plan_id: int = 0):
        planet = s0 is None
        spec = self.planet_spec if planet else self.spec
        if spec is None:
            raise HipetsError("Engine.planet_set_model() has not been called" if planet else "Engine.set_model() has not been called")
        dev = self.device
        for name, t, size in tensors:
            if t is not None:
                dtype = torch.int32 if name == "keep_idx" else torch.float32
                _check_dev(t, dtype, dev, name, **({"shape": size} if isinstance(size, tuple) else {"numel": size}))
        if planet:
            _check_dev(latent0, torch.float32, dev, "latent0", numel=n_env * spec.latent_size)
            _check_dev(belief0, torch.float32, dev, "belief0", numel=n_env * spec.belief_size)
# ... 302 lines not shown
```

Baseline: 289.9 million.

## Add grid-stride tile loop for per-step rollout kernels capped at resident capacity

Per-step (non-persistent, single-step) rollout launches larger than the resident workgroup capacity now run a capped grid. Each workgroup loops over logical tiles with XCD-major remapping and an optional ragged last turn, and new _tl kernel instances are compiled for each R and kernel class. choose_R gains a cost model for the tile-loop schedule. The aim is to cut tail-wave imbalance and per-block launch overhead, at the price of many more compiled instances, larger binaries and more complex indexing.

```diff
diff --git a/__graft_entry__.py b/__graft_entry__.py
--- a/__graft_entry__.py
+++ b/__graft_entry__.py
@@ -10,9 +10,11 @@
 OBJDIR = os.path.join(PKG, "build")
 HIPCC = os.environ.get("HIPCC", "/opt/rocm/bin/hipcc")
 HOST_UNITS = ["train.hip", "plan.hip", "rollout.hip", "model.hip", "comm.hip", "engine.hip"]
-UNITS = ["rollout_r3.hip", "rollout_r4_gen.hip", "rollout_r4_gens.hip", "rollout_r3_gen.hip", "rollout_r3_gens.hip", "rollout_r2.hip", "rollout_r2_gen.hip",
-         "rollout_r2_gens.hip", "rollout_r1_gen.hip", "rollout_r1_gens.hip", "rollout_r1.hip", "rollout_r4.hip", "rollout_r2_fast.hip", "rollout_r3_fast.hip",
-         "rollout_r1_fast.hip", "planet.hip"] + HOST_UNITS + ["rollout_r4_fast.hip"]
+UNITS = ["rollout_r3.hip", "rollout_r3_tl.hip", "rollout_r4_gen.hip", "rollout_r4_gen_tl.hip", "rollout_r4_gens.hip", "rollout_r4_gens_tl.hip", "rollout_r3_gen.hip",
+         "rollout_r3_gen_tl.hip", "rollout_r3_gens.hip", "rollout_r3_gens_tl.hip", "rollout_r2.hip", "rollout_r2_tl.hip", "rollout_r2_gen.hip", "rollout_r2_gen_tl.hip",
+         "rollout_r2_gens.hip", "rollout_r2_gens_tl.hip", "rollout_r1_gen.hip", "rollout_r1_gen_tl.hip", "rollout_r1_gens.hip", "rollout_r1_gens_tl.hip", "rollout_r1.hip",
+         "rollout_r1_tl.hip", "rollout_r4.hip", "rollout_r4_tl.hip", "rollout_r2_fast.hip", "rollout_r3_fast.hip", "rollout_r1_fast.hip", "planet.hip"] + HOST_UNITS + [
+         "rollout_r4_fast.hip"]
 FLAGS = ["--offload-arch=gfx950", "-O3", "-std=c++17", "-ffp-contract=off", "-fPIC", "-Wno-pass-failed"]
 
 
diff --git a/include/hipets.h b/include/hipets.h
--- a/include/hipets.h
+++ b/include/hipets.h
@@ -162,6 +162,7 @@
                         void* stream);
 
 int hipets_set_persistent(hipets_engine* e, int32_t on);
+int hipets_set_tile_loop(hipets_engine* e, int32_t on, int32_t max_grid);
 int hipets_set_handover_timeout(hipets_engine* e, double seconds);
 int hipets_check_async_error(hipets_engine* e, int32_t* timed_out);
 
diff --git a/mbrl-lib_amd/csrc/engine.hip b/mbrl-lib_amd/csrc/engine.hip
--- a/mbrl-lib_amd/csrc/engine.hip
+++ b/mbrl-lib_amd/csrc/engine.hip
@@ -135,6 +135,14 @@
     return 0;
 }
 
+int hipets_set_tile_loop(hipets_engine* e, int32_t on, int32_t max_grid) {
+    if (!e) return fail("null engine");
+    if (max_grid < 0) return fail("tile loop: max_grid %d is negative (0: the resident capacity alone)", max_grid);
+    e->tile_loop = on != 0;
+    e->tile_loop_max_grid = max_grid;
+    return 0;
+}
+
 int hipets_set_handover_timeout(hipets_engine* e, double seconds) {
     if (!e) return fail("null engine");
     if (!(seconds >= 0.0) || seconds > 60.0) return fail("hand-over timeout %g s outside [0, 60]", seconds);
diff --git a/mbrl-lib_amd/csrc/engine.hpp b/mbrl-lib_amd/csrc/engine.hpp
--- a/mbrl-lib_amd/csrc/engine.hpp
+++ b/mbrl-lib_amd/csrc/engine.hpp
@@ -76,6 +76,8 @@
     int plan_keys_count = 0, plan_keys_H = 0;
     int* error_flag = nullptr;
     bool persistent_ok = true;
+    bool tile_loop = true;
+    int tile_loop_max_grid = 0;
     long long poll_ticks = 20000000ll;
     DevBuf census;
     hipStream_t last_stream = nullptr;
diff --git a/mbrl-lib_amd/csrc/kspec.hpp b/mbrl-lib_amd/csrc/kspec.hpp
--- a/mbrl-lib_amd/csrc/kspec.hpp
+++ b/mbrl-lib_amd/csrc/kspec.hpp
@@ -11,6 +11,10 @@
     int m = (hidc > outc ? hidc : outc) * 16;
     while (m % 64 != 8) m += 4;
     return m;
+}
+
+constexpr bool tile_loop_fits(const bool lean_plain, const int R, const int outc, const int obsp, const int rew) {
+    return !(lean_plain && R == 2 && (outc == 6 || (obsp == HIPETS_OBS_HALFCHEETAH && rew == HIPETS_REW_HALFCHEETAH)));
 }
 
 template <int ACT_, int HIDC_ = -1, int OUTC_ = -1, int NORM_ = -1, int OBSP_ = -1, int REW_ = -1, int TERM_ = -1, int KMODE_ = -1, int PREC_ = 0,
@@ -49,13 +53,13 @@
     else linear_op_b3<R, S::ACT, S::OUTC, S::PIECES>(W3, bias, lm.Kp32 / 32, md.ld * 4, true, inb, outb, wave, lane);
 }
 
-template <int R, class S>
+template <int R, class S, bool KS = true>
 __device__ __forceinline__ void mlp_layer(const ModelDev& md, const LayerMeta* lmeta, const int l, const int member,
                                           const float* in, float* out, const int wave, const int lane, Prof& prof, float* part = nullptr) {
     const LayerMeta lm = lmeta[l];
     const float* W = md.w + (size_t)member * md.wmember + lm.woff;
     const float* bias = md.b + (size_t)member * md.bmember + lm.boff;
-    if constexpr (S::KSPLIT && R == 1) {
+    if constexpr (S::KSPLIT && R == 1 && KS) {
         float* const po = part + (l & 1) * (kWaves * 64 * 4);
         const float* const pi = part + ((l & 1) ^ 1) * (kWaves * 64 * 4);
         if (l == 0) linear_op<R, S::ACT, S::HIDC, NoTail, S::LD, false, -1, 2>(W, bias, lm, md.ld, true, md.activation, md.slope, in, out, wave, lane, prof, nullptr, 0, nullptr, po);
@@ -79,13 +83,13 @@
     }
 }
 
-template <int R, class S, class TL>
+template <int R, class S, bool KS = true, class TL>
 __device__ __forceinline__ void mlp_output_layer_fused(const ModelDev& md, const LayerMeta* lmeta, const int member, const float* in,
                                                        const int wave, const int lane, Prof& prof, const TL& tl, const float* part = nullptr) {
     const LayerMeta lm = lmeta[md.n_layers - 1];
     const float* W = md.w + (size_t)member * md.wmember + lm.woff_pairs;
     const float* bias = md.b + (size_t)member * md.bmember + lm.boff_pairs;
-    if constexpr (S::KSPLIT && R == 1) {
+    if constexpr (S::KSPLIT && R == 1 && KS) {
         const float* const pi = part + ((md.n_layers - 2) & 1) * (kWaves * 64 * 4);
         linear_op<R, S::ACT, S::OUTC, TL, S::LD, S::SPL_OUT, S::HIDC, 1>(W, bias, lm, md.ld, false, md.activation, md.slope, in, nullptr, wave, lane, prof, &tl, 0, pi);
     } else {
diff --git a/mbrl-lib_amd/csrc/residency.hpp b/mbrl-lib_amd/csrc/residency.hpp
--- a/mbrl-lib_amd/csrc/residency.hpp
+++ b/mbrl-lib_amd/csrc/residency.hpp
@@ -90,10 +90,19 @@
 }
 
 inline hipError_t launch_rollout_kernel(KernelRec& k, int grid, const unsigned lds, const int lds_max, const ModelDev& md, const RolloutArgs& ra, hipStream_t st,
-                                        hipEvent_t start, hipEvent_t stop) {
+                                        hipEvent_t start, hipEvent_t stop, const int tile_cap = 0) {
     const hipError_t e = full_lds_once(k.lds, k.fn, lds_max);
     if (e != hipSuccess) return e;
-    if (!ra.exchange) return enqueue_rollout(k, grid, lds, md, ra, st, start, stop);
+    if (!ra.exchange && ra.n_logical <= 0) return enqueue_rollout(k, grid, lds, md, ra, st, start, stop);
+    if (!ra.exchange)
+        return with_residency(k, lds, lds_max, [&](Occ& oc) {
+            int g = oc.blocks * oc.n_cu;
+            if (max_workgroups()) g = std::min(g, max_workgroups());
+            if (tile_cap > 0) g = std::min(g, tile_cap);
+            RolloutArgs rl = ra;
+            if (grid <= g) rl.n_logical = 0;
+            return enqueue_rollout(k, std::min(grid, g), lds, md, rl, st, start, stop);
+        });
     return with_residency(k, lds, lds_max, [&](Occ& oc) {
         grid = std::min(grid, oc.blocks * oc.n_cu);
         if (max_workgroups()) grid = std::min(grid, max_workgroups());
diff --git a/mbrl-lib_amd/csrc/rollout.hip b/mbrl-lib_amd/csrc/rollout.hip
--- a/mbrl-lib_amd/csrc/rollout.hip
+++ b/mbrl-lib_amd/csrc/rollout.hip
@@ -25,9 +25,26 @@
     return k;
 }
 
+bool ragged_last_turn_on() {
+    static const bool on = [] { const char* v = std::getenv("HIPETS_RAGGED_LAST_TURN"); return !(v && v[0] == '0'); }();
+    return on;
+}
+
+bool tile_loop_call(const hipets_engine* e, const RolloutArgs& ra) {
+    return e->tile_loop && !ra.whole_horizon && !ra.exchange && ra.t_end - ra.t_begin == 1;
+}
+
 int launch_rollout(hipets_engine* e, int R, int grid, size_t lds, const RolloutArgs& ra, hipStream_t st) {
     RolloutArgs rl = ra;
     rl.lds_bytes = (unsigned)lds;
+    const bool lean_plain = pick_rollout_instance(e->md, rl, R) == RolloutInstance::lean;
+    int resident = ((R <= 2 && !rl.wide_lds) ? 2 : 1) * e->num_cu;
+    if (max_workgroups()) resident = std::min(resident, max_workgroups());
+    if (e->tile_loop_max_grid > 0) resident = std::min(resident, e->tile_loop_max_grid);
+    if (grid > resident && tile_loop_call(e, rl) && tile_loop_fits(lean_plain, R, e->md.outC, e->md.obs_process, e->md.reward_fn)) {
+        rl.n_logical = grid;
+        rl.ragged_last_turn = ragged_last_turn_on() ? 1 : 0;
+    }
     KernelRec* k = rollout_instance(e, R, rl);
     if (!k) return 1;
     hipEvent_t a = nullptr, b = nullptr;
@@ -42,7 +59,7 @@
             HCHECK(hipEventCreate(&b));
         }
     }
-    const hipError_t err = launch_rollout_kernel(*k, grid, (unsigned)lds, (int)e->lds_max, e->md, rl, st, a, b);
+    const hipError_t err = launch_rollout_kernel(*k, grid, (unsigned)lds, (int)e->lds_max, e->md, rl, st, a, b, e->tile_loop_max_grid);
     if (timed) e->events.emplace_back(a, b);
     if (err != hipSuccess) return fail_kind(HIPETS_ERR_RUNTIME, "rollout kernel launch failed: %s", hipGetErrorString(err));
     return 0;
@@ -73,7 +90,7 @@
     return std::max(std::max(simd[0], simd[1]), std::max(simd[2], simd[3]));
 }
 
-int choose_R(const hipets_engine* e, long long tiles_total_per_slice, int slices, int forced, int horizon, bool wide, bool drift) {
+int choose_R(const hipets_engine* e, long long tiles_total_per_slice, int slices, int forced, int horizon, bool wide, bool drift, bool tile_loop) {
     if (forced > 0) return forced;
     const int C = e->md.hidC;
     const double a = (wide ? (drift ? 6.45 : 2.67) : 1.77) * (double)C / 13.0;
@@ -94,6 +111,17 @@
         const double u_pair = (co == 2 && drift) ? (double)C * R / 4.0 : u;
         const long long full = n / co, rem = n % co;
         double cost = (double)full * (a + co * u_pair) + (rem ? a + (double)rem * u : 0.0);
+        const long long G = (long long)co * e->num_cu;
+        if (tile_loop && nwg > G && tile_loop_fits(lean_shape(e->md, R) == LeanShape::plain, R, e->md.outC, e->md.obs_process, e->md.reward_fn)) {
+            const double at = a + (co == 1 ? 1.5 : 0.0);
+            const long long full_turns = (nwg + G - 1) / G - 1, served = full_turns * G;
+            const long long dom = served / groups, tile = R * (served - dom * groups);
+            const long long rem_tiles = (tiles_total_per_slice - tile) + (slices - 1 - dom) * tiles_total_per_slice;
+            const long long rem_wg = nwg - served;
+            cost = (double)full_turns * (at + co * u);
+            if ((wide ? R == 2 : R >= 3) && lean_shape_exists(e->md, R) && rem_tiles <= G) cost += at + (double)((rem_tiles + e->num_cu - 1) / e->num_cu) * wave_units(C, 1);
+            else cost += at + (double)((rem_wg + e->num_cu - 1) / e->num_cu) * u;
+        }
         if (!lean_shape_exists(e->md, R)) cost *= 1.08;
         if (cost < best_cost - 1e-9) {
             best_cost = cost;
@@ -131,7 +159,8 @@
                     "the wide-output instance's: size member_schedule with hipets_fast_geometry(rows_per_group = -1) and pass its row-tile "
                     "count as opts->rows_per_group");
     const bool drift = g->whole_horizon && H > 1;
-    g->R = choose_R(e, g->tiles, g->domains, rows_per_group, H, g->wide, drift);
+    const bool tile_loop = e->tile_loop && !g->whole_horizon && (call == GeoCall::step || mode == HIPETS_MODE_EXACT);
+    g->R = choose_R(e, g->tiles, g->domains, rows_per_group, H, g->wide, drift, tile_loop);
     g->lds = lds_for(e, g->R, H, g->wide);
     if (g->lds > e->lds_max) return fail("rows_per_group %d does not fit LDS", g->R);
     g->groups = (int)((g->tiles + g->R - 1) / g->R);
@@ -314,8 +343,7 @@
             ra.t_begin = 0;
             ra.t_end = H;
             ra.n_logical = domains * groups;
-            static const bool ragged_ok = [] { const char* v = std::getenv("HIPETS_RAGGED_LAST_TURN"); return !(v && v[0] == '0'); }();
-            ra.ragged_last_turn = (g.wide && R == 2 && ragged_ok) ? 1 : 0;
+            ra.ragged_last_turn = ragged_last_turn_on() ? 1 : 0;
 
             if (launch_rollout(e, R, domains * groups, lds, ra, st)) return 1;
         } else if (per_step) {
diff --git a/mbrl-lib_amd/csrc/rollout.hpp b/mbrl-lib_amd/csrc/rollout.hpp
--- a/mbrl-lib_amd/csrc/rollout.hpp
+++ b/mbrl-lib_amd/csrc/rollout.hpp
@@ -36,7 +36,7 @@
 #define HIPETS_STAMP(k, step) do {} while (0)
 #endif
 
-template <int R, class S>
+template <int R, class S, bool TL = false>
 __global__ __launch_bounds__(kThreads, (MinWaves<R, S>::value)) void rollout_kernel(const ModelDev md, const RolloutArgs ra) {
     constexpr int ROWS = kTile * R;
     constexpr bool kLean = S::LEAN;
@@ -79,7 +79,7 @@
         }
 #endif
     }
-    const int tid = threadIdx.x;
+    int tid = threadIdx.x;
     if (ra.census) {
         if (tid == 0) {
             __hip_atomic_fetch_add(ra.census, 1, __ATOMIC_RELAXED, __HIP_MEMORY_SCOPE_AGENT);
@@ -97,11 +97,38 @@
     const int wave = __builtin_amdgcn_readfirstlane(tid >> 6);
     const bool fast = S::KMODE >= 0 ? S::KMODE == HIPETS_MODE_FAST : ra.whole_horizon != 0;
     const bool expectation = kLean ? false : md.propagation == HIPETS_PROP_EXPECTATION;
+    auto xcd_major = [&](const int i, const int n) __attribute__((always_inline)) {
+        const int x = i & 7, slot = i >> 3;
+        return x * (n >> 3) + min(x, n & 7) + slot;
+    };
+    constexpr bool kTileLoop = TL && tile_loop_fits(S::FUSE && !S::WIDE, R, S::OUTC, S::OBSP, S::REW);
+    const bool tloop = kTileLoop && !fast && ra.exchange == nullptr && ra.n_logical > 0;
+    constexpr bool kRagged = S::FUSE && (S::WIDE ? R == 2 : (TL && R >= 3));
+    int half_from = 0x7FFFFFFF;
+    int n_logical = ra.n_logical;
+    int hf_dom = 0, hf_tile = 0, hf_tpd = 1;
+    if constexpr (kRagged) {
+        if (!fast && ra.n_logical > 0 && ra.ragged_last_turn) {
+            const int G = (int)gridDim.x, nR = ra.n_logical;
+            const int turnsR = (nR + G - 1) / G, full = (turnsR - 1) * G;
+            if (turnsR >= 2) {
+                hf_tpd = (ra.rows_per_domain + kTile - 1) / kTile;
+                hf_dom = full / ra.groups;
+                hf_tile = R * (full - hf_dom * ra.groups);
+                const int rem = (hf_tpd - hf_tile) + (nR / ra.groups - 1 - hf_dom) * hf_tpd;
+                if (rem <= G) {
+                    half_from = full;
+                    n_logical = full + rem;
+                }
+            }
+        }
+    }
+    const int tl_xn = half_from != 0x7FFFFFFF ? half_from : n_logical;
+    auto tl_logical = [&](const int i) __attribute__((always_inline)) { return i < tl_xn ? xcd_major(i, tl_xn) : i; };
     int wg = blockIdx.x;
-    if (!fast) {
-        const int nwg = gridDim.x, x = wg & 7, slot = wg >> 3;
-        wg = x * (nwg >> 3) + min(x, nwg & 7) + slot;
-    }
+    if (tloop) wg = tl_logical(wg);
+    else if (!fast) wg = xcd_major(wg, (int)gridDim.x);
+    const int nwg_rule = tloop ? ra.n_logical : (int)gridDim.x;
 
     int domain = 0;
     if (fast) {
@@ -123,7 +150,7 @@
         domain = wg / ra.groups;
         const int j0 = (wg % ra.groups) * ROWS;
         const long long* perm = ra.perm ? ra.perm + (long long)ra.t_begin * ra.perm_step : nullptr;
-        if (perm && perm[(long long)domain * ra.rows_per_domain + j0] < 0) return;
+        if (!tloop && perm && perm[(long long)domain * ra.rows_per_domain + j0] < 0) return;
         const PermKeys keys0 = ra.exchange ? ra.step_keys[ra.t_begin] : ra.perm_keys;
         for (int s = tid; s < ROWS; s += kThreads) {
             const int j = j0 + s;
@@ -135,33 +162,16 @@
             sm.rowid[s] = rid;
         }
     }
-    int member_dom = domain;
-    if (!fast && ra.fast_members && !expectation)
-        member_dom = __builtin_amdgcn_readfirstlane(
-            ra.schedule ? ra.schedule[(size_t)ra.t_begin * gridDim.x + wg]
-                        : fast_member((unsigned)wg, gridDim.x, ra.fm_a, ra.fm_b, md.M, md.iid_members, ra.seed, ra.stream_id,
-                                      md.propagation == HIPETS_PROP_FIXED_MODEL ? 0xFFFFFFFFu : (unsigned)ra.t_begin));
+    auto member_of = [&](const int dom, const int v) __attribute__((always_inline)) {
+        if (!fast && ra.fast_members && !expectation)
+            return __builtin_amdgcn_readfirstlane(
+                ra.schedule ? ra.schedule[(size_t)ra.t_begin * nwg_rule + v]
+                            : fast_member((unsigned)v, nwg_rule, ra.fm_a, ra.fm_b, md.M, md.iid_members, ra.seed, ra.stream_id,
+                                          md.propagation == HIPETS_PROP_FIXED_MODEL ? 0xFFFFFFFFu : (unsigned)ra.t_begin));
+        return dom;
+    };
+    int member_dom = member_of(domain, wg);
     const bool persist = !fast && ra.exchange != nullptr;
-    constexpr bool kRagged = S::WIDE && R == 2;
-    int half_from = 0x7FFFFFFF;
-    int n_logical = ra.n_logical;
-    int hf_dom = 0, hf_tile = 0, hf_tpd = 1;
-    if constexpr (kRagged) {
-        if (persist && ra.ragged_last_turn) {
-            const int G = (int)gridDim.x, n2 = ra.n_logical;
-            const int turns2 = (n2 + G - 1) / G, full = (turns2 - 1) * G;
-            if (turns2 >= 2) {
-                hf_tpd = (ra.rows_per_domain + kTile - 1) / kTile;
-                hf_dom = full / ra.groups;
-                hf_tile = 2 * (full - hf_dom * ra.groups);
-                const int rem = (hf_tpd - hf_tile) + (n2 / ra.groups - 1 - hf_dom) * hf_tpd;
-                if (rem <= G) {
-                    half_from = full;
-                    n_logical = full + rem;
-                }
-            }
-        }
-    }
     auto logical_rows = [&](const int v, int& dom, int& j0, int& live) __attribute__((always_inline)) {
         if (!kRagged || v < half_from) {
             dom = v / ra.groups;
@@ -248,7 +258,7 @@
     };
     lds_barrier();
 
-    auto load_initial_state = [&]() __attribute__((always_inline)) {
+    auto load_initial_state = [&](auto with_constants) __attribute__((always_inline)) {
         constexpr int kStage = 4;
         constexpr int kRowStage = (ROWS + kThreads - 1) / kThreads;
         const int n_st = ROWS * md.obs_dim;
@@ -282,7 +292,7 @@
                 }
             }
             if (first) {
-                commit_constants();
+                if constexpr (decltype(with_constants)::value) commit_constants();
 #pragma unroll
                 for (int q = 0; q < kRowStage; ++q) {
                     const int s = tid + q * kThreads;
@@ -528,7 +538,7 @@
     {
         float av[kPrefetch];
         fetch_actions_issue(ra.t_begin, av);
-        load_initial_state();
+        load_initial_state(std::true_type{});
         fetch_actions_commit(ra.t_begin, av);
     }
     __syncthreads();
@@ -539,7 +549,8 @@
     prof.mark(0);
     float* step_in = sm.buf0;
 
-    const int n_serve = persist ? (n_logical - wg + (int)gridDim.x - 1) / (int)gridDim.x : 1;
+    const int n_serve = persist ? (n_logical - wg + (int)gridDim.x - 1) / (int)gridDim.x
+                                : (tloop ? (n_logical - (int)blockIdx.x + (int)gridDim.x - 1) / (int)gridDim.x : 1);
     const int n_seq = (ra.t_end - ra.t_begin) * n_serve;
     int stamp_seq = 0;
     (void)stamp_seq;
@@ -708,6 +719,30 @@
     };
     (void)dma_collect;
 
+    auto write_back = [&]() __attribute__((always_inline)) {
+        if constexpr (S::FUSE && S::TERM == HIPETS_TERM_HOPPER) {
+            if (ra.t_end > ra.t_begin && !persist)
+                for (int s = tid; s < ROWS; s += kThreads) sm.term[s] |= sm.pend[((ra.t_end - 1) & 1) * ROWS + s];
+        }
+        for (int s = tid; s < ROWS; s += kThreads) {
+            const int rid = sm.rowid[s];
+            if (rid < 0 || persist) continue;
+            ra.totals[rid] = sm.tot[s];
+            if (!fast && !persist) ra.term[rid] = (unsigned char)sm.term[s];
+        }
+        if (!fast && !persist) {
+            for (int i = tid; i < ROWS * md.obs_dim; i += kThreads) {
+                const int s = i / md.obs_dim, d = i % md.obs_dim;
+                const int rid = sm.rowid[s];
+                if (rid >= 0) ra.state[(size_t)rid * md.obs_dim + d] = sm.state[i];
+            }
+        }
+    };
+    auto tl_row = [&](const int jj) __attribute__((always_inline)) {
+        const long long* const pm = ra.perm ? ra.perm + (long long)ra.t_begin * ra.perm_step : nullptr;
+        return pm ? (int)pm[jj] : (ra.perm_n ? (int)perm_apply((unsigned)jj, ra.perm_n, ra.perm_a, ra.perm_b, ra.perm_keys) : jj);
+    };
+
     bool one_tile = false;
     for (int q_seq = 0; q_seq < n_seq; ++q_seq) {
         stamp_seq = q_seq;
@@ -715,7 +750,8 @@
         const bool more = t + 1 < ra.t_end;
         const bool has_next = q_seq + 1 < n_seq;
         const int t_next = ra.t_begin + (q_seq + 1) / n_serve;
-        const int v_next = wg + ((q_seq + 1) - ((q_seq + 1) / n_serve) * n_serve) * (int)gridDim.x;
+        const int v_next = tloop ? tl_logical((int)blockIdx.x + (q_seq + 1) * (int)gridDim.x)
+                                 : wg + ((q_seq + 1) - ((q_seq + 1) / n_serve) * n_serve) * (int)gridDim.x;
         float av[kPrefetch];
         if (more && !persist) fetch_actions_issue(t + 1, av);
         unsigned long long* const handover = (more && persist) ? ra.exchange : nullptr;
@@ -728,6 +764,13 @@
             const bool write_input = more && !persist && !kWide;
             const bool wide_fast_next = kWide && more && !persist;
             const bool prep_next = straight && more;
+            int wave1 = wave, lane1 = lane;
+            if constexpr (kRagged) {
+                if (one_tile) {
+                    asm volatile("" : "+s"(wave1));
+                    asm volatile("" : "+v"(lane1));
+                }
+            }
             int* const rows_nxt = sm.rowid == rows_a ? rows_b : rows_a;
             for (int l = 0; l + 1 < L; ++l) {
                 prof.mark(12);
@@ -745,7 +788,7 @@
                 }
                 if (l == L - 2 && (write_input || prep_next || wide_fast_next)) fetch_actions_commit(t + 1, av);
                 if constexpr (kRagged) {
-                    if (one_tile) mlp_layer<1, S>(md, sm.lmeta, l, member, cur, nxt, wave, lane, prof, sm.part);
+                    if (one_tile) mlp_layer<1, S, false>(md, sm.lmeta, l, member, cur, nxt, wave1, lane1, prof, sm.part);
                     else mlp_layer<R, S>(md, sm.lmeta, l, member, cur, nxt, wave, lane, prof, sm.part);
                 } else {
                     mlp_layer<R, S>(md, sm.lmeta, l, member, cur, nxt, wave, lane, prof, sm.part);
@@ -897,7 +940,7 @@
             const auto tail = make_tail(tail_prep, tail_draw, tail_unit, tail_finish);
             prof.mark(12);
             if constexpr (kRagged) {
-                if (one_tile) mlp_output_layer_fused<1, S>(md, sm.lmeta, member, cur, wave, lane, prof, tail, sm.part);
+                if (one_tile) mlp_output_layer_fused<1, S, false>(md, sm.lmeta, member, cur, wave1, lane1, prof, tail, sm.part);
                 else mlp_output_layer_fused<R, S>(md, sm.lmeta, member, cur, wave, lane, prof, tail, sm.part);
             } else {
                 mlp_output_layer_fused<R, S>(md, sm.lmeta, member, cur, wave, lane, prof, tail, sm.part);
@@ -1095,6 +1138,34 @@
 
         }
         HIPETS_STAMP(1, t);
+        if (tloop && has_next) {
+            const int tid_launch = tid;
+            asm volatile("" : "+v"(tid));
+            write_back();
+            lds_barrier();
+            int nj0, nlive;
+            logical_rows(v_next, domain, nj0, nlive);
+            if constexpr (kRagged) {
+                one_tile = nlive < ROWS;
+                in_rows = nlive;
+            }
+            member_dom = member_of(domain, domain * ra.groups + nj0 / ROWS);
+            for (int s = tid; s < ROWS; s += kThreads) {
+                const int j = nj0 + s;
+                sm.rowid[s] = (s < nlive && j < ra.rows_per_domain) ? tl_row(domain * ra.rows_per_domain + j) : -1;
+            }
+            lds_barrier();
+            compute_act_base();
+            float av2[kPrefetch];
+            fetch_actions_issue(t, av2);
+            load_initial_state(std::false_type{});
+            fetch_actions_commit(t, av2);
+            __syncthreads();
+            step_in = sm.buf0;
+            build_input(t, step_in);
+            __syncthreads();
+            tid = tid_launch;
+        }
         if (persist && has_next) {
             {
                 int nj0, nlive;
@@ -1188,27 +1259,11 @@
         }
     }
 
-    if constexpr (S::FUSE && S::TERM == HIPETS_TERM_HOPPER) {
-        if (ra.t_end > ra.t_begin && !persist)
-            for (int s = tid; s < ROWS; s += kThreads) sm.term[s] |= sm.pend[((ra.t_end - 1) & 1) * ROWS + s];
-    }
-    for (int s = tid; s < ROWS; s += kThreads) {
-        const int rid = sm.rowid[s];
-        if (rid < 0 || persist) continue;
-        ra.totals[rid] = sm.tot[s];
-        if (!fast && !persist) ra.term[rid] = (unsigned char)sm.term[s];
-    }
+    write_back();
     if (prof.on) {
 #pragma unroll
         for (int i = 0; i < 16; ++i) ra.phase_cycles[wave * 16 + i] += prof.slot[i];
     }
-    if (!fast && !persist) {
-        for (int i = tid; i < ROWS * md.obs_dim; i += kThreads) {
-            const int s = i / md.obs_dim, d = i % md.obs_dim;
-            const int rid = sm.rowid[s];
-            if (rid >= 0) ra.state[(size_t)rid * md.obs_dim + d] = sm.state[i];
-        }
-    }
 }
 
 }
diff --git a/mbrl-lib_amd/csrc/rollout_inst.inc b/mbrl-lib_amd/csrc/rollout_inst.inc
--- a/mbrl-lib_amd/csrc/rollout_inst.inc
+++ b/mbrl-lib_amd/csrc/rollout_inst.inc
@@ -13,28 +13,36 @@
 #define HIPETS_B3_SHAPES(X) HIPETS_CAT2(HIPETS_B3_SHAPES_R, HIPETS_R)(X)
 #define HIPETS_BF16_SHAPES(X) HIPETS_CAT2(HIPETS_BF16_SHAPES_R, HIPETS_R)(X)
 
+#if HIPETS_PART >= 5
+#define HIPETS_TL true
+#else
+#define HIPETS_TL false
+#endif
 #if HIPETS_PART == 2
 #define HIPETS_LEAN_MODE HIPETS_MODE_FAST
 #define HIPETS_SPEC_FN HIPETS_FN(_fast)
+#elif HIPETS_PART == 5
+#define HIPETS_LEAN_MODE HIPETS_MODE_EXACT
+#define HIPETS_SPEC_FN HIPETS_FN(_exact_tl)
 #else
 #define HIPETS_LEAN_MODE HIPETS_MODE_EXACT
 #define HIPETS_SPEC_FN HIPETS_FN(_exact)
 #endif
 #define HIPETS_TRY_SHAPE(HC, OC, RW, TM, OB) \
-    if (lean_shape_is(md, HC, OC, RW, TM, OB)) return &rec<LeanSpec<HC, OC, RW, TM, OB, HIPETS_LEAN_MODE>>();
+    if (lean_shape_is(md, HC, OC, RW, TM, OB)) return &rec<LeanSpec<HC, OC, RW, TM, OB, HIPETS_LEAN_MODE>, HIPETS_TL>();
 #define HIPETS_TRY_PREC(PREC, HC, OC, RW, TM) \
-    if (b3_shape_is(md, HC, OC, RW, TM)) return &rec<KSpec<HIPETS_ACT_SILU, HC, OC, HIPETS_NORM_F64, HIPETS_OBS_NONE, RW, TM, HIPETS_LEAN_MODE, PREC>>();
+    if (b3_shape_is(md, HC, OC, RW, TM)) return &rec<KSpec<HIPETS_ACT_SILU, HC, OC, HIPETS_NORM_F64, HIPETS_OBS_NONE, RW, TM, HIPETS_LEAN_MODE, PREC>, HIPETS_TL>();
 #define HIPETS_TRY_B3(HC, OC, RW, TM) HIPETS_TRY_PREC(HIPETS_PREC_BF16X3, HC, OC, RW, TM)
 #define HIPETS_TRY_BF16(HC, OC, RW, TM) HIPETS_TRY_PREC(HIPETS_PREC_BF16, HC, OC, RW, TM)
 #define HIPETS_TRY_HID(HC) \
-    if (hid_static_is(md, HC)) return &rec<KSpec<HIPETS_ACT_SILU, HC>>();
+    if (hid_static_is(md, HC)) return &rec<KSpec<HIPETS_ACT_SILU, HC>, HIPETS_TL>();
 
 namespace hipets {
 
 namespace {
-template <class S>
+template <class S, bool TL = false>
 KernelRec& rec() {
-    static KernelRec r{reinterpret_cast<const void*>(&rollout_kernel<HIPETS_R, S>)};
+    static KernelRec r{reinterpret_cast<const void*>(&rollout_kernel<HIPETS_R, S, TL>)};
     return r;
 }
 }
@@ -42,6 +50,10 @@
 KernelRec* HIPETS_FN(_fast)(RolloutInstance pick, const ModelDev& md);
 KernelRec* HIPETS_FN(_gen)();
 KernelRec* HIPETS_FN(_gens)();
+KernelRec* HIPETS_FN(_exact_tl)(RolloutInstance pick, const ModelDev& md);
+KernelRec* HIPETS_FN(_hid_tl)(const ModelDev& md);
+KernelRec* HIPETS_FN(_gen_tl)();
+KernelRec* HIPETS_FN(_gens_tl)();
 
 #if HIPETS_PART == 3
 KernelRec* HIPETS_FN(_gen)() { return &rec<KSpec<-1>>(); }
@@ -50,7 +62,20 @@
 KernelRec* HIPETS_FN(_gens)() { return &rec<KSpec<HIPETS_ACT_SILU>>(); }
 #endif
 
-#if HIPETS_PART <= 2
+#if HIPETS_PART == 6
+KernelRec* HIPETS_FN(_gen_tl)() { return &rec<KSpec<-1>, true>(); }
+#endif
+#if HIPETS_PART == 7
+KernelRec* HIPETS_FN(_gens_tl)() { return &rec<KSpec<HIPETS_ACT_SILU>, true>(); }
+#endif
+#if HIPETS_PART == 5
+KernelRec* HIPETS_FN(_hid_tl)(const ModelDev& md) {
+    HIPETS_HID_STATIC_SHAPES(HIPETS_TRY_HID)
+    return nullptr;
+}
+#endif
+
+#if HIPETS_PART <= 2 || HIPETS_PART == 5
 KernelRec* HIPETS_SPEC_FN(const RolloutInstance pick, const ModelDev& md) {
     if (pick == RolloutInstance::b3) {
         HIPETS_B3_SHAPES(HIPETS_TRY_B3)
@@ -66,15 +91,18 @@
 #if HIPETS_PART == 1
 KernelRec* HIPETS_FN()(const ModelDev& md, const RolloutArgs& ra, hipError_t* why) {
     const RolloutInstance pick = pick_rollout_instance(md, ra, HIPETS_R);
+    const bool tl = ra.n_logical > 0 && !ra.exchange && !ra.whole_horizon;
     *why = hipErrorNotSupported;
     switch (pick) {
         case RolloutInstance::lean:
         case RolloutInstance::lean_wide:
         case RolloutInstance::b3:
-        case RolloutInstance::bf16: return (ra.whole_horizon ? HIPETS_FN(_fast) : HIPETS_FN(_exact))(pick, md);
-        case RolloutInstance::hidden_static: HIPETS_HID_STATIC_SHAPES(HIPETS_TRY_HID) break;
-        case RolloutInstance::generic_silu: return HIPETS_FN(_gens)();
-        case RolloutInstance::generic: return HIPETS_FN(_gen)();
+        case RolloutInstance::bf16: return (ra.whole_horizon ? HIPETS_FN(_fast) : (tl ? HIPETS_FN(_exact_tl) : HIPETS_FN(_exact)))(pick, md);
+        case RolloutInstance::hidden_static:
+            if (tl) return HIPETS_FN(_hid_tl)(md);
+            HIPETS_HID_STATIC_SHAPES(HIPETS_TRY_HID) break;
+        case RolloutInstance::generic_silu: return tl ? HIPETS_FN(_gens_tl)() : HIPETS_FN(_gens)();
+        case RolloutInstance::generic: return tl ? HIPETS_FN(_gen_tl)() : HIPETS_FN(_gen)();
         case RolloutInstance::no_b3:
         case RolloutInstance::no_bf16: break;
         case RolloutInstance::no_wide: *why = hipErrorInvalidConfiguration; break;
diff --git a/mbrl-lib_amd/csrc/rollout_r1_gen_tl.hip b/mbrl-lib_amd/csrc/rollout_r1_gen_tl.hip
--- /dev/null
+++ b/mbrl-lib_amd/csrc/rollout_r1_gen_tl.hip
@@ -0,0 +1,3 @@
+#define HIPETS_R 1
+#define HIPETS_PART 6
+#include "rollout_inst.inc"
diff --git a/mbrl-lib_amd/csrc/rollout_r1_gens_tl.hip b/mbrl-lib_amd/csrc/rollout_r1_gens_tl.hip
--- /dev/null
+++ b/mbrl-lib_amd/csrc/rollout_r1_gens_tl.hip
@@ -0,0 +1,3 @@
+#define HIPETS_R 1
+#define HIPETS_PART 7
+#include "rollout_inst.inc"
diff --git a/mbrl-lib_amd/csrc/rollout_r1_tl.hip b/mbrl-lib_amd/csrc/rollout_r1_tl.hip
--- /dev/null
+++ b/mbrl-lib_amd/csrc/rollout_r1_tl.hip
@@ -0,0 +1,3 @@
+#define HIPETS_R 1
+#define HIPETS_PART 5
+#include "rollout_inst.inc"
diff --git a/mbrl-lib_amd/csrc/rollout_r2_gen_tl.hip b/mbrl-lib_amd/csrc/rollout_r2_gen_tl.hip
--- /dev/null
+++ b/mbrl-lib_amd/csrc/rollout_r2_gen_tl.hip
@@ -0,0 +1,3 @@
+#define HIPETS_R 2
+#define HIPETS_PART 6
+#include "rollout_inst.inc"
diff --git a/mbrl-lib_amd/csrc/rollout_r2_gens_tl.hip b/mbrl-lib_amd/csrc/rollout_r2_gens_tl.hip
--- /dev/null
+++ b/mbrl-lib_amd/csrc/rollout_r2_gens_tl.hip
@@ -0,0 +1,3 @@
+#define HIPETS_R 2
+#define HIPETS_PART 7
+#include "rollout_inst.inc"
diff --git a/mbrl-lib_amd/csrc/rollout_r2_tl.hip b/mbrl-lib_amd/csrc/rollout_r2_tl.hip
--- /dev/null
+++ b/mbrl-lib_amd/csrc/rollout_r2_tl.hip
@@ -0,0 +1,3 @@
+#define HIPETS_R 2
+#define HIPETS_PART 5
+#include "rollout_inst.inc"
diff --git a/mbrl-lib_amd/csrc/rollout_r3_gen_tl.hip b/mbrl-lib_amd/csrc/rollout_r3_gen_tl.hip
--- /dev/null
+++ b/mbrl-lib_amd/csrc/rollout_r3_gen_tl.hip
@@ -0,0 +1,3 @@
+#define HIPETS_R 3
+#define HIPETS_PART 6
+#include "rollout_inst.inc"
diff --git a/mbrl-lib_amd/csrc/rollout_r3_gens_tl.hip b/mbrl-lib_amd/csrc/rollout_r3_gens_tl.hip
--- /dev/null
+++ b/mbrl-lib_amd/csrc/rollout_r3_gens_tl.hip
@@ -0,0 +1,3 @@
+#define HIPETS_R 3
+#define HIPETS_PART 7
+#include "rollout_inst.inc"
diff --git a/mbrl-lib_amd/csrc/rollout_r3_tl.hip b/mbrl-lib_amd/csrc/rollout_r3_tl.hip
--- /dev/null
+++ b/mbrl-lib_amd/csrc/rollout_r3_tl.hip
@@ -0,0 +1,3 @@
+#define HIPETS_R 3
+#define HIPETS_PART 5
+#include "rollout_inst.inc"
diff --git a/mbrl-lib_amd/csrc/rollout_r4_gen_tl.hip b/mbrl-lib_amd/csrc/rollout_r4_gen_tl.hip
--- /dev/null
+++ b/mbrl-lib_amd/csrc/rollout_r4_gen_tl.hip
@@ -0,0 +1,3 @@
+#define HIPETS_R 4
+#define HIPETS_PART 6
+#include "rollout_inst.inc"
diff --git a/mbrl-lib_amd/csrc/rollout_r4_gens_tl.hip b/mbrl-lib_amd/csrc/rollout_r4_gens_tl.hip
--- /dev/null
+++ b/mbrl-lib_amd/csrc/rollout_r4_gens_tl.hip
@@ -0,0 +1,3 @@
+#define HIPETS_R 4
+#define HIPETS_PART 7
+#include "rollout_inst.inc"
diff --git a/mbrl-lib_amd/csrc/rollout_r4_tl.hip b/mbrl-lib_amd/csrc/rollout_r4_tl.hip
--- /dev/null
+++ b/mbrl-lib_amd/csrc/rollout_r4_tl.hip
@@ -0,0 +1,3 @@
+#define HIPETS_R 4
+#define HIPETS_PART 5
+#include "rollout_inst.inc"
diff --git a/mbrl-lib_amd/hipets/_lib.py b/mbrl-lib_amd/hipets/_lib.py
--- a/mbrl-lib_amd/hipets/_lib.py
+++ b/mbrl-lib_amd/hipets/_lib.py
@@ -158,6 +158,7 @@
     "hipets_device_perms": (C.c_int, [_P, C.c_int32, C.c_int32, C.c_uint64, C.c_uint64, _P, _P]),
     "hipets_set_plan_mode": (C.c_int, [_P, C.c_int32]),
     "hipets_set_persistent": (C.c_int, [_P, C.c_int32]),
+    "hipets_set_tile_loop": (C.c_int, [_P, C.c_int32, C.c_int32]),
     "hipets_set_handover_timeout": (C.c_int, [_P, C.c_double]),
     "hipets_check_async_error": (C.c_int, [_P, C.POINTER(C.c_int32)]),
     "hipets_set_plan_trace": (C.c_int, [_P, C.POINTER(PlanTrace)]),
diff --git a/mbrl-lib_amd/hipets/engine.py b/mbrl-lib_amd/hipets/engine.py
--- a/mbrl-lib_amd/hipets/engine.py
+++ b/mbrl-lib_amd/hipets/engine.py
@@ -328,6 +328,9 @@
     def set_persistent(self, on: bool = True):
         _lib.check(self._lib.hipets_set_persistent(self._h, int(bool(on))))
 
+    def set_tile_loop(self, on: bool = True, max_grid: int = 0):
+        _lib.check(self._lib.hipets_set_tile_loop(self._h, int(bool(on)), int(max_grid)))
+
     def synchronize(self):
         torch.cuda.synchronize(self.device)
 
```

Measured after the change: 289.7 million. No clear change (-0.1%).
